# qiskit-community/aqc-research

Measured on AMD Instinct MI355X. Metric: objective+gradient evals/sec, higher is better.
Workload: dtype f64; 1 GPU; 16-qubit, 40-block cx spin ansatz, state-vector objective+gradient; n_qubits=16, num_thetas=208, gate_groups=56, batch_per_gpu=1024, columns=1, transport=none, records_gathered=1024, launcher=none

## Files before the change

### aqc_research_amd/csrc/aqc_api.cpp

```cpp
#include "aqc_ws.h"

using namespace aqc;

namespace {
thread_local std::string g_error;
}

namespace aqc {

int fail(const char* fmt, ...) {
    char buf[1024];
    va_list ap;
    va_start(ap, fmt);
    vsnprintf(buf, sizeof buf, fmt, ap);
    va_end(ap);
    g_error = buf;
    return 1;
}
int set_error(const std::string& msg) { g_error = msg; return 1; }

int check_buf(const aqc_ws* ws, int buf) {
    if (!ws) return fail("null workspace");
    if (buf < 0 || buf >= AQC_NUM_BUFS) return fail("invalid buffer id %d", buf);
    return 0;
}

int check_block_range(const aqc_ws* ws, int block_from, int block_to) {
    const int nb = ws->ctx->prog.num_blocks;
    if (block_from < 0 || nb == 0) return 0;
    if (!(block_from < block_to && block_to <= nb)) return fail("invalid block_range [%d, %d)", block_from, block_to);
    return 0;
}

int ensure_small(aqc_ws* ws, size_t n_cplx) {
    if (n_cplx <= ws->small_cap) return 0;
    if (ws->d_small) HIP_OK(hipFree(ws->d_small));
    ws->d_small = nullptr;
    HIP_OK(hipMalloc((void**)&ws->d_small, n_cplx * sizeof(double2)));
    ws->small_cap = n_cplx;
    return 0;
}

int ensure_tmp(aqc_ws* ws, size_t n_index, size_t n_cplx) {
    if (n_index > ws->tmp_index_cap) {
        if (ws->d_tmp_index) HIP_OK(hipFree(ws->d_tmp_index));
        ws->d_tmp_index = nullptr;
        HIP_OK(hipMalloc((void**)&ws->d_tmp_index, n_index * sizeof(long long)));
        ws->tmp_index_cap = n_index;
    }
    if (n_cplx > ws->tmp_small_cap) {
        if (ws->d_tmp_small) HIP_OK(hipFree(ws->d_tmp_small));
        ws->d_tmp_small = nullptr;
        HIP_OK(hipMalloc((void**)&ws->d_tmp_small, n_cplx * sizeof(double2)));
        ws->tmp_small_cap = n_cplx;
    }
    return 0;
}

int ensure_index(aqc_ws* ws, size_t n) {
    if (n <= ws->index_cap) return 0;
    if (ws->d_index) HIP_OK(hipFree(ws->d_index));
    ws->d_index = nullptr;
    HIP_OK(hipMalloc((void**)&ws->d_index, n * sizeof(long long)));
    ws->index_cap = n;
    return 0;
}

int ensure_coef(aqc_ws* ws) {
    if (ws->coef_valid) return 0;
    return fail("thetas have not been uploaded (aqc_ws_set_thetas)");
}

int copy_in(aqc_ws* ws, double2* dst, const double* src, size_t rows) {
    if (ws->pitch == ws->ncols) {
        HIP_OK(hipMemcpyAsync(dst, src, rows * ws->ncols * sizeof(double2), hipMemcpyHostToDevice, ws->stream));
    } else {
        HIP_OK(hipMemsetAsync(dst, 0, rows * ws->pitch * sizeof(double2), ws->stream));
        HIP_OK(hipMemcpy2DAsync(dst, (size_t)ws->pitch * sizeof(double2), src, (size_t)ws->ncols * sizeof(double2),
                                (size_t)ws->ncols * sizeof(double2), rows, hipMemcpyHostToDevice, ws->stream));
    }
    HIP_OK(hipStreamSynchronize(ws->stream));
    return 0;
}
int copy_out(aqc_ws* ws, double* dst, const double2* src, size_t rows) {
    if (ws->pitch == ws->ncols) {
        HIP_OK(hipMemcpyAsync(dst, src, rows * ws->ncols * sizeof(double2), hipMemcpyDeviceToHost, ws->stream));
    } else {
        HIP_OK(hipMemcpy2DAsync(dst, (size_t)ws->ncols * sizeof(double2), src, (size_t)ws->pitch * sizeof(double2),
                                (size_t)ws->ncols * sizeof(double2), rows, hipMemcpyDeviceToHost, ws->stream));
    }
    HIP_OK(hipStreamSynchronize(ws->stream));
    return 0;
}

int results_guard(aqc_ws* ws) {
    if (ws->copy_pending && !ws->capturing) {
        HIP_OK(hipStreamWaitEvent(ws->stream, ws->ev_copied, 0));
        ws->copy_pending = false;
    }
    return 0;
}


}

extern "C" {

const char* aqc_version(void) { return "aqc_hip 0.1.0 (gfx950)"; }
const char* aqc_last_error(void) { return g_error.c_str(); }

int aqc_device_count(void) {
    int ndev = 0;
    return hipGetDeviceCount(&ndev) == hipSuccess ? ndev : 0;
}

int aqc_create(int num_qubits, int entangler, const int32_t* blocks, int num_blocks, int trotter, int second_order,
               aqc_ctx** out) {
    if (!out) return fail("out pointer is null");
    *out = nullptr;
    aqc_ctx* ctx = new aqc_ctx();
    const std::string err = build_program(num_qubits, entangler, blocks, num_blocks, trotter != 0, second_order != 0, ctx->prog);
    if (!err.empty()) {
        delete ctx;
        return fail("%s", err.c_str());
    }
    *out = ctx;
    return 0;
}

int aqc_destroy(aqc_ctx* ctx) {
    if (!ctx) return 0;
    for (auto& kv : ctx->oneshot) aqc_ws_destroy(kv.second);
    delete ctx;
    return 0;
}

int aqc_num_thetas(const aqc_ctx* ctx) { return ctx ? ctx->prog.num_thetas() : -1; }
int aqc_num_gate_groups(const aqc_ctx* ctx) { return ctx ? (int)ctx->prog.groups.size() : -1; }

int aqc_plan_query(aqc_ctx* ctx, int ncols, int which, int tile_bits, int low_bits, int stage, int* num_stages,
                   int* bits_out, int* num_bits, int* ops_out, int* num_ops) {
    if (!ctx) return fail("null context");
    if (ncols < 1) return fail("ncols must be positive");
    const int col_bits = ceil_log2(ncols);
    if (tile_bits <= 0) tile_bits = which == 1 ? 12 : 13;
    if (low_bits < 0) low_bits = 3;
    Plan plan = make_plan(ctx->prog, col_bits, tile_bits, low_bits, which == 0);
    if (which == 3) {
        split_substages(ctx->prog, plan, 4, 1 << 20);
        plan = mirror_plan(plan);
    }
    const std::string err = check_plan(ctx->prog, plan);
    if (!err.empty()) return fail("planner produced an invalid plan: %s", err.c_str());
    if (num_stages) *num_stages = (int)plan.stages.size();
    if (stage >= 0) {
        if (stage >= (int)plan.stages.size()) return fail("stage index out of range");
        const Stage& st = plan.stages[stage];
        if (num_bits) *num_bits = (int)st.bits.size();
        if (num_ops) *num_ops = (int)st.ops.size();
        if (bits_out) for (size_t i = 0; i < st.bits.size(); ++i) bits_out[i] = st.bits[i];
        if (ops_out) for (size_t i = 0; i < st.ops.size(); ++i) ops_out[i] = st.ops[i];
    }
    return 0;
}

int aqc_plan_projected(aqc_ctx* ctx, int tile_bits, int low_bits, int32_t* info) {
    if (!ctx || !info) return fail("null argument");
    if (tile_bits <= 0) tile_bits = 12;
    if (low_bits < 0) low_bits = 3;
    const Program& prog = ctx->prog;
    tile_bits = std::min(std::max(tile_bits, 8), std::min(12, prog.n));
    aqc_ws tmp;
    tmp.ctx = ctx;
    tmp.ncols = 1; tmp.col_bits = 0; tmp.nbits = prog.n;
    Plan best = make_plan(prog, 0, tile_bits, low_bits, false);
    for (int lb = low_bits - 1; lb >= 2; --lb) {
        Plan cand = make_plan(prog, 0, tile_bits, lb, false);
        if (cand.stages.size() < best.stages.size()) best = cand;
    }
    lower_plan(prog, best, tmp.sweep, 4, true, true);
    tmp.sparse_enabled = true;
    tmp.inv_mirrored = tmp.sweep.v3 && tmp.sweep.plan.stages.size() >= 2;
    proj_plan(&tmp, low_bits);
    const int rc = aqc_ws_projected_info(&tmp, info);
    tmp.ctx = nullptr;
    return rc;
}

int aqc_plan_substages(aqc_ctx* ctx, int ncols, int which, int tile_bits, int low_bits, int stage, int* num_subs, int* subs_out, int max_subs) {
    if (!ctx || !num_subs) return fail("null argument");
    if (ncols < 1) return fail("ncols must be positive");
    const int col_bits = ceil_log2(ncols);
    if (tile_bits <= 0) tile_bits = 12;
    if (low_bits < 0) low_bits = 3;
    Plan plan = make_plan(ctx->prog, col_bits, tile_bits, low_bits, which == 0);
    split_substages(ctx->prog, plan, 4, 1 << 20);
    if (which == 3) plan = mirror_plan(plan);
    const std::string err = check_plan(ctx->prog, plan);
    if (!err.empty()) return fail("planner produced an invalid plan: %s", err.c_str());
    if (stage < 0 || stage >= (int)plan.stages.size()) return fail("stage index out of range");
    const Stage& st = plan.stages[stage];
    *num_subs = (int)st.subs.size();
    if (subs_out)
        for (int i = 0; i < (int)st.subs.size() && i < max_subs; ++i) {
            for (int j = 0; j < 4; ++j) subs_out[5 * i + j] = j < (int)st.subs[i].bits.size() ? st.subs[i].bits[j] : -1;
            subs_out[5 * i + 4] = (int)st.subs[i].ops.size();
        }
    return 0;
}

int aqc_ws_create(aqc_ctx* ctx, int device, int batch, int ncols, int tile_bits_apply, int tile_bits_sweep, aqc_ws** out) {
    if (!out) return fail("out pointer is null");
    *out = nullptr;
    if (!ctx) return fail("null context");
    if (batch < 1 || batch > 65535) return fail("batch must be in [1, 65535] (lanes are the y dimension of the launch grid)");
    if (ncols < 1) return fail("ncols must be >= 1");
    const Program& prog = ctx->prog;
    int ndev = 0;
    hipError_t e = hipGetDeviceCount(&ndev);
    if (e != hipSuccess || ndev <= 0)
        return fail("no HIP device available (%s): the aqc_hip path needs an AMD GPU and has no CPU fallback",
                    e == hipSuccess ? "device count is 0" : hipGetErrorString(e));
    if (device < 0 || device >= ndev) return fail("device %d out of range (%d visible)", device, ndev);
    HIP_OK(hipSetDevice(device));
    HIP_OK(init_kernels());
    HIP_OK(init_kernels2());
    HIP_OK(init_kernels3());

    aqc_ws* ws = new aqc_ws();
    ws->ctx = ctx;
    ws->device = device;
    ws->batch = batch;
    ws->ncols = ncols;
    ws->col_bits = ceil_log2(ncols);
    ws->pitch = 1 << ws->col_bits;
    ws->nbits = ws->col_bits + prog.n;
    if (ws->nbits > kMaxBits) { delete ws; return fail("2^%d elements per lane is beyond this build's limit", ws->nbits); }
    ws->lane_elems = (size_t)1 << ws->nbits;
    const int low_bits = env_int("AQC_LOW_BITS", 3);
    int ka = tile_bits_apply > 0 ? tile_bits_apply : env_int("AQC_TILE_BITS_APPLY", 0);
    int ks = tile_bits_sweep > 0 ? tile_bits_sweep : env_int("AQC_TILE_BITS_SWEEP", 0);
    const int family = env_int("AQC_KERNEL_FAMILY", env_int("AQC_KERNEL_V2", -1) >= 0 ? env_int("AQC_KERNEL_V2", -1) + 1 : 0);
    if (family < 0 || family > 3) { delete ws; return fail("AQC_KERNEL_FAMILY must be 1 (per-group), 2 (register-blocked) or 3 (matrix cores)"); }
    const bool want_v3 = (family == 3 || family == 0) && ws->nbits >= 8;
    const int force_v2 = family == 3 ? 0 : (family ? family - 1 : -1);
    const size_t big_tiles = (size_t)batch << std::max(0, ws->nbits - 12);
    const bool want_v2 = force_v2 >= 0 ? force_v2 != 0 : big_tiles >= 512;
    auto pick = [&](int kmax) {
        if (want_v3) {
            int k = std::min(12, ws->nbits);
            while (k > 10 && ((size_t)batch << (ws->nbits - k)) < 256) --k;
            const int kmin = std::max(8, prog.n + std::min(ws->col_bits, 3));
            while (ws->col_bits > 0 && k > kmin && ((size_t)batch << (ws->nbits - k)) < 256) --k;
            return k;
        }
        if (want_v2) return std::min(kmax, ws->nbits);
        int k = std::min(11, ws->nbits);
        while (k > 10 && ((size_t)batch << (ws->nbits - k)) < 512) --k;
        return k;
    };
    if (ka <= 0) ka = pick(13);
    if (ks <= 0) ks = pick(12);
    ka = std::min(std::min(ka, 13), ws->nbits);
    ks = std::min(std::min(ks, 12), ws->nbits);
    ws->threads = env_int("AQC_THREADS", 0);
    if (ws->threads <= 0) ws->threads = std::min(256, std::max(64, 1 << (std::min(ka, ks) - 2)));
    if (ws->threads < 64 || ws->threads > 512 || ws->threads % 64) { delete ws; return fail("AQC_THREADS must be a multiple of 64 in [64, 512]"); }

    auto best_plan = [&](int k, bool inverse) {
        Plan best = make_plan(prog, ws->col_bits, k, low_bits, inverse);
        for (int lb = low_bits - 1; lb >= 2; --lb) {
            Plan cand = make_plan(prog, ws->col_bits, k, lb, inverse);
            if (cand.stages.size() < best.stages.size()) best = cand;
        }
        return best;
    };
    if (want_v3) { ka = std::min(std::max(ka, 8), 12); ks = std::max(ks, 8); }
    auto cached_plan = [&](int which, int k, bool inverse, int reg_bits, bool dots, DevPlan& out) {
        const std::vector<int> key = {which, ws->col_bits, k, low_bits, reg_bits, (int)dots, (int)want_v3};
        std::lock_guard<std::mutex> lock(ctx->mu);
        auto it = ctx->plan_cache.find(key);
        if (it == ctx->plan_cache.end()) {
            DevPlan fresh;
            lower_plan(prog, best_plan(k, inverse), fresh, reg_bits, dots, want_v3);
            it = ctx->plan_cache.emplace(key, std::move(fresh)).first;
        }
        out = it->second;
    };
    cached_plan(2, ka, false, (want_v2 || want_v3) ? 4 : 0, false, ws->fwd);
    cached_plan(1, ks, false, want_v3 ? 4 : (want_v2 ? (env_int("AQC_SWEEP_REG_BITS", 4) == 3 ? 3 : 4) : 0), true, ws->sweep);
    ws->inv_mirrored = want_v3 && ka == ks && ws->sweep.v3 && ws->sweep.plan.stages.size() >= 2 && env_int("AQC_MIRROR_PLAN", 1) != 0;
    if (ws->inv_mirrored) {
        const std::vector<int> key = {3, ws->col_bits, ks, low_bits, 4, 0, 1};
        std::lock_guard<std::mutex> lock(ctx->mu);
        auto it = ctx->plan_cache.find(key);
        if (it == ctx->plan_cache.end()) {
            DevPlan fresh;
            lower_plan(prog, mirror_plan(ws->sweep.plan), fresh, 4, false, true, true);
            it = ctx->plan_cache.emplace(key, std::move(fresh)).first;
        }
        ws->inv = it->second;
    } else {
        cached_plan(0, ka, true, (want_v2 || want_v3) ? 4 : 0, false, ws->inv);
    }
    ws->sparse_enabled = env_int("AQC_SPARSE_SWEEP", 1) != 0;
    ws->sparse_min_items = env_int("AQC_SPARSE_MIN_ITEMS", 512);
    ws->lazy_z_enabled = env_int("AQC_LAZY_Z", 1) != 0;
    ws->r_only_enabled = env_int("AQC_R_ONLY_LAST", 1) != 0;
    ws->r_only_max_subs = env_int("AQC_R_ONLY_MAX_SUBS", 12);
    ws->proj_vdag_enabled = env_int("AQC_PROJECTED_VDAG", 1) != 0;
    ws->proj_fused_enabled = env_int("AQC_PROJECTED_FUSED", 1) != 0;
    ws->proj_vdag_min_elems = (long long)env_int("AQC_PROJECTED_VDAG_MIN_ELEMS", 1 << 24);
    ws->skipw_enabled = env_int("AQC_SKIP_ZERO_W", 0) != 0;
    for (DevPlan* p : {&ws->fwd, &ws->inv, &ws->sweep}) {
        const std::string err = check_plan(prog, p->plan);
        if (!err.empty()) { delete ws; return fail("planner produced an invalid plan: %s", err.c_str()); }
    }
    proj_plan(ws, low_bits);

    const int T = prog.num_thetas();
    const int G = (int)prog.groups.size();
    ws->nslots = G * kSlotsPerGroup;
    const int partial_tiles = ws->sweep.v3 ? 1 : ws->sweep.ntiles;
    std::vector<int> theta_slots(2 * (size_t)std::max(T, 1), -1), slot_ntiles((size_t)std::max(ws->nslots, 1), partial_tiles);
    auto feed = [&](int theta, int slot) {
        if (theta_slots[2 * theta] < 0) theta_slots[2 * theta] = slot; else theta_slots[2 * theta + 1] = slot;
    };
    for (int gi = 0; gi < G; ++gi) {
        const GateGroup& g = prog.groups[gi];
        if (g.type == GROUP_FRONT) {
            feed(g.theta0 + 2, gi * kSlotsPerGroup + 0);
            feed(g.theta0 + 1, gi * kSlotsPerGroup + 1);
            feed(g.theta0 + 0, gi * kSlotsPerGroup + 2);
        } else {
            for (int d = 0; d < prog.tpb; ++d) feed(g.theta0 + d, gi * kSlotsPerGroup + d);
        }
    }

    std::vector<int> slot_theta((size_t)std::max(ws->nslots, 1), -1);
    ws->grads_direct = ws->sweep.v3 && T > 0 && env_int("AQC_GRADS_DIRECT", 1) != 0;
    for (int t = 0; t < T; ++t) {
        if (theta_slots[2 * t] < 0 || theta_slots[2 * t + 1] >= 0) { ws->grads_direct = false; break; }
        slot_theta[theta_slots[2 * t]] = t;
    }
    if (env_int("AQC_VERBOSE", 0) && want_v3)
        fprintf(stderr, "aqc_hip: matrix-core kernels, tiles 2^%d (V / V^H, %d workgroups per CU) / 2^%d (sweep, %d per CU), sub-stages %zu / %zu / %zu\n",
                ws->inv.k, mfma_occupancy(ws->inv.k, false), ws->sweep.k, mfma_occupancy(ws->sweep.k, true), ws->fwd.h_subs3.size(),
                ws->inv.h_subs3.size(), ws->sweep.h_subs3.size());
#define WS_TRY(x) do { if ((x) != 0) { aqc_ws_destroy(ws); return 1; } } while (0)
#define WS_HIP(x) do { hipError_t e_ = (x); if (e_ != hipSuccess) { fail("%s failed: %s", #x, hipGetErrorString(e_)); aqc_ws_destroy(ws); return 1; } } while (0)
    WS_HIP(hipStreamCreateWithFlags(&ws->stream, hipStreamNonBlocking));
    WS_HIP(hipEventCreate(&ws->ev0)); WS_HIP(hipEventCreate(&ws->ev1));
    WS_HIP(hipEventCreate(&ws->pev0)); WS_HIP(hipEventCreate(&ws->pev1));
    WS_TRY(upload_plan(ws->fwd)); WS_TRY(upload_plan(ws->inv)); WS_TRY(upload_plan(ws->sweep));
    WS_TRY(proj_alloc(ws));
    WS_HIP(hipMalloc((void**)&ws->d_thetas_own, sizeof(double) * (size_t)batch * std::max(T, 1)));
    ws->d_thetas = ws->d_thetas_own;
    WS_HIP(hipMalloc((void**)&ws->d_coef, sizeof(double) * (size_t)batch * (prog.n + prog.num_blocks + 1) * kCoefStride));
    for (int b = 0; b < AQC_NUM_BUFS; ++b) {
        WS_HIP(hipMalloc((void**)&ws->bufs[b], sizeof(double2) * (size_t)batch * ws->lane_elems));
        WS_HIP(hipMemsetAsync(ws->bufs[b], 0, sizeof(double2) * (size_t)batch * ws->lane_elems, ws->stream));
    }
    WS_HIP(hipMalloc((void**)&ws->d_partial, sizeof(double2) * (size_t)batch * std::max(ws->nslots, 1) * partial_tiles));
    for (DevPlan* p : {&ws->fwd, &ws->inv, &ws->sweep})
        if (p->v3) WS_HIP(hipMalloc((void**)&p->d_umat, sizeof(double) * (size_t)batch * std::max<size_t>(p->h_subs3.size(), 1) * 12 * 64));
    {
        std::vector<UJob> jobs;
        DevPlan* vsw = ws->proj.ok ? &ws->proj.vsw : nullptr;
        const int nsw = ws->sweep.v3 ? (int)ws->sweep.h_subs3.size() : 0;
        ws->ujobs_mirror = ws->inv_mirrored && ws->inv.v3 && (int)ws->inv.h_subs3.size() == nsw && env_int("AQC_UBUILD_MIRROR", 1) != 0;
        for (DevPlan* p : {&ws->inv, &ws->sweep, vsw, &ws->fwd})
            if (p && p->v3)
                for (size_t i = 0; i < p->h_subs3.size(); ++i) {
                    if (p == &ws->inv && ws->ujobs_mirror) continue;
                    UJob j{p->d_subs3 + i, p->d_grps, p->d_umat, (int)i, (int)p->h_subs3.size(), p->plan.inverse ? 1 : 0, prog.entangler, nullptr, 0, 0};
                    if (p == &ws->sweep && ws->ujobs_mirror) { j.umat_mirror = ws->inv.d_umat; j.mirror_index = nsw - 1 - (int)i; j.mirror_nsubs = nsw; }
                    if (p == vsw) {
                        const int nvs = (int)vsw->h_subs3.size();
                        j.umat_mirror = ws->proj.vinv.d_umat; j.mirror_index = nvs - 1 - (int)i; j.mirror_nsubs = nvs;
                    }
                    jobs.push_back(j);
                }
        if (!jobs.empty()) {
            WS_HIP(hipMalloc((void**)&ws->d_ujobs, sizeof(UJob) * jobs.size()));
            WS_HIP(hipMemcpy(ws->d_ujobs, jobs.data(), sizeof(UJob) * jobs.size(), hipMemcpyHostToDevice));
        }
    }
    if (ws->sweep.v3)
        WS_HIP(hipMalloc((void**)&ws->sweep.d_rpart, sizeof(double2) * (size_t)batch * std::max<size_t>(ws->sweep.h_subs3.size(), 1) *
                                                        sweep3_nparts(ws->sweep.ntiles, batch, ws->sweep.k) * 256));
    WS_HIP(hipMalloc((void**)&ws->d_grads, sizeof(double2) * (size_t)batch * std::max(T, 1)));
    WS_HIP(hipMalloc((void**)&ws->d_theta_slots, sizeof(int) * theta_slots.size()));
    WS_HIP(hipMalloc((void**)&ws->d_slot_ntiles, sizeof(int) * slot_ntiles.size()));
    WS_HIP(hipMemcpy(ws->d_theta_slots, theta_slots.data(), sizeof(int) * theta_slots.size(), hipMemcpyHostToDevice));
    WS_HIP(hipMalloc((void**)&ws->d_slot_theta, sizeof(int) * slot_theta.size()));
    WS_HIP(hipMemcpy(ws->d_slot_theta, slot_theta.data(), sizeof(int) * slot_theta.size(), hipMemcpyHostToDevice));
    WS_HIP(hipMemcpy(ws->d_slot_ntiles, slot_ntiles.data(), sizeof(int) * slot_ntiles.size(), hipMemcpyHostToDevice));
    ws->pin_thetas = (size_t)batch * std::max(T, 1);
    ws->pin_grads = 2 * (size_t)batch * std::max(T, 1);
    ws->pin_small = 2 * (size_t)batch * 64;
    WS_HIP(hipHostMalloc((void**)&ws->h_pin, sizeof(double) * (ws->pin_thetas + ws->pin_grads + ws->pin_small), hipHostMallocDefault));
    ws->vdot_parts = (int)std::min<size_t>(1024, std::max<size_t>(1, ws->lane_elems / 1024));
    WS_HIP(hipMalloc((void**)&ws->d_vdot_part, sizeof(double2) * (size_t)batch * ws->vdot_parts));
    WS_HIP(hipStreamSynchronize(ws->stream));
#undef WS_TRY
#undef WS_HIP
    *out = ws;
    return 0;
}


int aqc_ws_destroy(aqc_ws* ws) {
    if (!ws) return 0;
    (void)hipSetDevice(ws->device);
    if (ws->stream) (void)hipStreamSynchronize(ws->stream);
    drop_graphs(ws);
    proj_free(ws);
    for (DevPlan* p : {&ws->fwd, &ws->inv, &ws->sweep}) {
        if (p->d_stages) (void)hipFree(p->d_stages);
        if (p->d_ops) (void)hipFree(p->d_ops);
        if (p->d_subs) (void)hipFree(p->d_subs);
        if (p->d_mops) (void)hipFree(p->d_mops);
        if (p->d_subs3) (void)hipFree(p->d_subs3);
        if (p->d_grps) (void)hipFree(p->d_grps);
        if (p->d_umat) (void)hipFree(p->d_umat);
        if (p->d_rpart) (void)hipFree(p->d_rpart);
    }
    void* ptrs[] = {ws->d_thetas_own, ws->d_theta_bank, ws->d_coef, ws->d_partial, ws->d_grads, ws->d_small, ws->d_vdot_part, ws->d_index, ws->d_tmp_index, ws->d_tmp_small,
                    ws->d_theta_slots, ws->d_slot_theta, ws->d_slot_ntiles, ws->d_basis_index, ws->d_vdot_out, ws->d_ujobs};
    for (void* p : ptrs) if (p) (void)hipFree(p);
    for (int b = 0; b < AQC_NUM_BUFS; ++b) if (ws->bufs[b]) (void)hipFree(ws->bufs[b]);
    for (int b = 0; b < AQC_NUM_BUFS; ++b) if (ws->d_combo_prev[b]) (void)hipFree(ws->d_combo_prev[b]);
    for (void* q : {(void*)ws->d_sw_items, (void*)ws->d_sw_clear, (void*)ws->d_sw_counts, (void*)ws->d_sw_lane_parts, (void*)ws->d_sw_prev_tiles,
                    (void*)ws->w2, (void*)ws->zw2, (void*)ws->d_vd_items})
        if (q) (void)hipFree(q);
    if (ws->d_sur) (void)hipFree(ws->d_sur);
    if (ws->d_sur_real) (void)hipFree(ws->d_sur_real);
    if (ws->h_sur) (void)hipHostFree(ws->h_sur);
    if (ws->d_combo_index) (void)hipFree(ws->d_combo_index);
    if (ws->d_combo_coef) (void)hipFree(ws->d_combo_coef);
    if (ws->h_pin) (void)hipHostFree(ws->h_pin);
    for (auto& m : ws->mps) if (m.d_t) (void)hipFree(m.d_t);
    if (ws->d_mps_scratch) (void)hipFree(ws->d_mps_scratch);
    for (auto& t : ws->mps_tabs) if (t.dev) (void)hipFree(t.dev);
    if (ws->d_cd_prog) (void)hipFree(ws->d_cd_prog);
    if (ws->d_cd_thetas) (void)hipFree(ws->d_cd_thetas);
    if (ws->d_cd_fobj) (void)hipFree(ws->d_cd_fobj);
    if (ws->d_mps_lam) (void)hipFree(ws->d_mps_lam);
    for (hipEvent_t ev : {ws->ev0, ws->ev1, ws->pev0, ws->pev1, ws->ev_ready, ws->ev_copied}) if (ev) (void)hipEventDestroy(ev);
    if (ws->copy_stream) { (void)hipStreamSynchronize(ws->copy_stream); (void)hipStreamDestroy(ws->copy_stream); }
    if (ws->mps_stream) { (void)hipStreamSynchronize(ws->mps_stream); (void)hipStreamDestroy(ws->mps_stream); }
    for (hipEvent_t ev : {ws->ev_mps_fork, ws->ev_mps_join}) if (ev) (void)hipEventDestroy(ev);
    if (ws->stream) (void)hipStreamDestroy(ws->stream);
    delete ws;
    return 0;
}

int aqc_ws_set_thetas(aqc_ws* ws, const double* thetas) {
    if (!ws || !thetas) return fail("null argument");
    HIP_OK(hipSetDevice(ws->device));
    const Program& prog = ws->ctx->prog;
    const int T = prog.num_thetas();
    HIP_OK(hipMemcpyAsync(ws->d_thetas_own, thetas, sizeof(double) * (size_t)ws->batch * T, hipMemcpyHostToDevice, ws->stream));
    HIP_OK(hipStreamSynchronize(ws->stream));
    return run_coef(ws, ws->d_thetas_own);
}

int aqc_ws_upload(aqc_ws* ws, int buf, const double* src) {
    if (check_buf(ws, buf) || before_write(ws, buf)) return 1;
    if (!src) return fail("null source");
    HIP_OK(hipSetDevice(ws->device));
    return copy_in(ws, ws->bufs[buf], src, (size_t)ws->batch << ws->ctx->prog.n);
}

int aqc_ws_upload_lane(aqc_ws* ws, int buf, int lane, const double* src) {
    if (check_buf(ws, buf)) return 1;
    if (!src) return fail("null source");
    if (lane < 0 || lane >= ws->batch) return fail("lane out of range");
    HIP_OK(hipSetDevice(ws->device));
    if (before_write(ws, buf, true)) return 1;
    return copy_in(ws, ws->bufs[buf] + (size_t)lane * ws->lane_elems, src, (size_t)1 << ws->ctx->prog.n);
}

int aqc_ws_broadcast(aqc_ws* ws, int buf, const double* src) {
    if (check_buf(ws, buf) || before_write(ws, buf)) return 1;
    if (!src) return fail("null source");
    HIP_OK(hipSetDevice(ws->device));
    if (copy_in(ws, ws->bufs[buf], src, (size_t)1 << ws->ctx->prog.n)) return 1;
    for (int b = 1; b < ws->batch; ++b)
        HIP_OK(hipMemcpyAsync(ws->bufs[buf] + (size_t)b * ws->lane_elems, ws->bufs[buf], ws->lane_elems * sizeof(double2),
                              hipMemcpyDeviceToDevice, ws->stream));
    return 0;
}

int aqc_ws_copy_lane(aqc_ws* dst_ws, int dst_buf, int dst_lane, aqc_ws* src_ws, int src_buf, int src_lane) {
    if (check_buf(dst_ws, dst_buf) || check_buf(src_ws, src_buf)) return 1;
    if (dst_ws->device != src_ws->device) return fail("copy_lane: the two workspaces live on different devices");
    if (dst_ws->lane_elems != src_ws->lane_elems) return fail("copy_lane: lane sizes differ");
    if (dst_lane < 0 || dst_lane >= dst_ws->batch || src_lane < 0 || src_lane >= src_ws->batch) return fail("lane out of range");
    if (before_read(src_ws, src_buf) || before_write(dst_ws, dst_buf, true)) return 1;
    HIP_OK(hipSetDevice(dst_ws->device));
    if (src_ws->stream != dst_ws->stream) HIP_OK(hipStreamSynchronize(src_ws->stream));
    HIP_OK(hipMemcpyAsync(dst_ws->bufs[dst_buf] + (size_t)dst_lane * dst_ws->lane_elems, src_ws->bufs[src_buf] + (size_t)src_lane * src_ws->lane_elems,
                          sizeof(double2) * dst_ws->lane_elems, hipMemcpyDeviceToDevice, dst_ws->stream));
    return 0;
}

int aqc_ws_download(aqc_ws* ws, int buf, double* dst) {
    if (check_buf(ws, buf)) return 1;
    if (!dst) return fail("null destination");
    HIP_OK(hipSetDevice(ws->device));
    if (before_read(ws, buf)) return 1;
    return copy_out(ws, dst, ws->bufs[buf], (size_t)ws->batch << ws->ctx->prog.n);
}

int aqc_ws_download_lane(aqc_ws* ws, int buf, int lane, double* dst) {
    if (check_buf(ws, buf)) return 1;
    if (!dst) return fail("null destination");
    if (lane < 0 || lane >= ws->batch) return fail("lane out of range");
    HIP_OK(hipSetDevice(ws->device));
    if (before_read(ws, buf)) return 1;
    return copy_out(ws, dst, ws->bufs[buf] + (size_t)lane * ws->lane_elems, (size_t)1 << ws->ctx->prog.n);
}

int aqc_ws_set_basis(aqc_ws* ws, int buf, const int64_t* index) {
    if (check_buf(ws, buf) || before_write(ws, buf)) return 1;
    if (!index) return fail("null index");
    HIP_OK(hipSetDevice(ws->device));
    const int64_t dim = (int64_t)1 << ws->ctx->prog.n;
    std::vector<long long> elem(ws->batch);
    for (int b = 0; b < ws->batch; ++b) {
        if (index[b] < 0 || index[b] >= dim) return fail("basis index out of range");
        elem[b] = (long long)index[b] << ws->col_bits;
    }
    if (!ws->d_basis_index) HIP_OK(hipMalloc((void**)&ws->d_basis_index, sizeof(long long) * ws->batch));
    HIP_OK(hipMemcpyAsync(ws->d_basis_index, elem.data(), sizeof(long long) * ws->batch, hipMemcpyHostToDevice, ws->stream));
    HIP_OK(hipStreamSynchronize(ws->stream));
    HIP_OK(hipMemsetAsync(ws->bufs[buf], 0, sizeof(double2) * (size_t)ws->batch * ws->lane_elems, ws->stream));
    {
        ProfScope ps(ws, AQC_K_MISC);
        HIP_OK(launch_scatter_one(ws->bufs[buf], ws->lane_elems, ws->batch, ws->d_basis_index, ws->stream));
    }
    std::vector<long long> supp(2 * (size_t)ws->batch, -1);
    for (int b = 0; b < ws->batch; ++b) supp[2 * (size_t)b] = elem[b];
    if (!ws->d_combo_prev[buf]) HIP_OK(hipMalloc((void**)&ws->d_combo_prev[buf], sizeof(long long) * 2 * ws->batch));
    HIP_OK(hipMemcpyAsync(ws->d_combo_prev[buf], supp.data(), sizeof(long long) * supp.size(), hipMemcpyHostToDevice, ws->stream));
    HIP_OK(hipStreamSynchronize(ws->stream));
    std::vector<double> coef(4 * (size_t)ws->batch, 0.0);
    for (int b = 0; b < ws->batch; ++b) coef[4 * (size_t)b] = 1.0;
    lhs_support_changed(ws, buf, std::move(supp), std::move(coef));
    return 0;
}

int aqc_ws_set_identity(aqc_ws* ws, int buf) {
    if (check_buf(ws, buf) || before_write(ws, buf)) return 1;
    const int dim = 1 << ws->ctx->prog.n;
    if (ws->ncols != dim) return fail("identity needs a square workspace (ncols == 2^n)");
    HIP_OK(hipSetDevice(ws->device));
    HIP_OK(hipMemsetAsync(ws->bufs[buf], 0, sizeof(double2) * (size_t)ws->batch * ws->lane_elems, ws->stream));
    ProfScope ps(ws, AQC_K_MISC);
    HIP_OK(launch_set_identity(ws->bufs[buf], ws->lane_elems, dim, ws->pitch, ws->batch, ws->stream));
    return 0;
}

int aqc_ws_set_combo(aqc_ws* ws, int buf, const int64_t* index, const double* coef) {
    if (check_buf(ws, buf)) return 1;
    if (!index || !coef) return fail("null argument");
    if (buf == AQC_BUF_W || buf == AQC_BUF_ZW || buf == AQC_BUF_Z) return fail("set_combo targets an lhs buffer (X, X2) or Y");
    HIP_OK(hipSetDevice(ws->device));
    const int64_t dim = (int64_t)1 << ws->ctx->prog.n;
    const int B = ws->batch;
    std::vector<long long> elem(2 * (size_t)B);
    for (int b = 0; b < B; ++b) {
        const int64_t i0 = index[2 * b], i1 = index[2 * b + 1];
        if (i0 < 0 || i0 >= dim || i1 >= dim) return fail("basis index out of range");
        if (i1 == i0) return fail("the two basis states of a lane must differ");
        elem[2 * b] = (long long)i0 << ws->col_bits;
        elem[2 * b + 1] = i1 < 0 ? -1 : (long long)i1 << ws->col_bits;
    }
    std::vector<double> cf(coef, coef + 4 * (size_t)B);
    if (ws->combo_valid[buf] && ws->combo_last_elem[buf] == elem && ws->combo_last_coef[buf] == cf) return 0;
    if (!ws->d_combo_index) HIP_OK(hipMalloc((void**)&ws->d_combo_index, sizeof(long long) * 2 * B));
    if (!ws->d_combo_coef) HIP_OK(hipMalloc((void**)&ws->d_combo_coef, sizeof(double2) * 2 * B));
    if (!ws->d_combo_prev[buf]) HIP_OK(hipMalloc((void**)&ws->d_combo_prev[buf], sizeof(long long) * 2 * B));
    HIP_OK(hipMemcpyAsync(ws->d_combo_index, elem.data(), sizeof(long long) * 2 * B, hipMemcpyHostToDevice, ws->stream));
    HIP_OK(hipMemcpyAsync(ws->d_combo_coef, coef, sizeof(double2) * 2 * B, hipMemcpyHostToDevice, ws->stream));
    HIP_OK(hipStreamSynchronize(ws->stream));
    if (!ws->combo_valid[buf]) {
        HIP_OK(hipMemsetAsync(ws->bufs[buf], 0, sizeof(double2) * (size_t)B * ws->lane_elems, ws->stream));
        HIP_OK(hipMemsetAsync(ws->d_combo_prev[buf], 0xff, sizeof(long long) * 2 * B, ws->stream));
    }
    ProfScope ps(ws, AQC_K_MISC);
    HIP_OK(launch_scatter_two(ws->bufs[buf], ws->lane_elems, B, ws->d_combo_index, ws->d_combo_coef, ws->d_combo_prev[buf], ws->stream));
    lhs_support_changed(ws, buf, std::move(elem), std::move(cf));
    return 0;
}

int aqc_ws_get_grads(aqc_ws* ws, double* grads) {
    if (!ws || !grads) return fail("null argument");
    HIP_OK(hipSetDevice(ws->device));
    HIP_OK(hipMemcpyAsync(grads, ws->d_grads, sizeof(double2) * (size_t)ws->batch * ws->ctx->prog.num_thetas(),
                          hipMemcpyDeviceToHost, ws->stream));
    HIP_OK(hipStreamSynchronize(ws->stream));
    return 0;
}

int aqc_ws_gather(aqc_ws* ws, int buf, const int64_t* index, int count, double* out) {
    if (check_buf(ws, buf)) return 1;
    if (!index || !out || count < 1) return fail("invalid gather arguments");
    HIP_OK(hipSetDevice(ws->device));
    if (before_read(ws, buf)) return 1;
    const int64_t dim = (int64_t)1 << ws->ctx->prog.n;
    std::vector<long long> elem(count);
    for (int i = 0; i < count; ++i) {
// ... 352 lines not shown
```

### aqc_research_amd/csrc/aqc_kernels3.hip

```cpp
#include <hip/hip_runtime.h>

#include <cstring>

#include <type_traits>

#include "aqc_device.h"
#include "aqc_launch.h"
#include "aqc_math.h"

namespace aqc {

typedef double double4_t __attribute__((ext_vector_type(4)));

__host__ __device__ __forceinline__ unsigned swz3(unsigned l) { return l ^ ((l >> 4) & 15u) ^ ((l >> 8) & 15u); }

__device__ __forceinline__ double4_t mfma(double a, double b, double4_t c) {
    return __builtin_amdgcn_mfma_f64_16x16x4f64(a, b, c, 0, 0, 0);
}

struct Acc3 { double4_t k1, k2, k3; };
__device__ __forceinline__ void u_mfma(const cplx (&v)[4], const double (&u0)[4], const double (&u1)[4], const double (&u2)[4], Acc3& t) {
    t.k1 = double4_t{0.0, 0.0, 0.0, 0.0}; t.k2 = t.k1; t.k3 = t.k1;
#pragma unroll
    for (int s = 0; s < 4; ++s) {
        t.k1 = mfma(v[s].x + v[s].y, u0[s], t.k1);
        t.k2 = mfma(v[s].x, u1[s], t.k2);
        t.k3 = mfma(v[s].y, u2[s], t.k3);
    }
}
__device__ __forceinline__ void u_combine(const Acc3& t, cplx (&o)[4]) {
#pragma unroll
    for (int r = 0; r < 4; ++r) {
        o[r].x = t.k1[r] - t.k3[r];
        o[r].y = t.k1[r] + t.k2[r];
    }
}

#ifdef AQC_TUNING
#define AQC_STAMP(slot) do { if (a.stamps && threadIdx.x == 0 && (slot) < kStampSlots) \
    a.stamps[((size_t)blockIdx.y * gridDim.x + blockIdx.x) * kStampSlots + (slot)] = __builtin_amdgcn_s_memtime(); } while (0)
#ifdef AQC_TUNING_NODBG
#define AQC_DBG_AND(x)
#define AQC_DBG_TEST(x) false
#else
#define AQC_DBG_AND(x) && (x)
#define AQC_DBG_TEST(x) (x)
#endif
#else
#define AQC_STAMP(slot) do { } while (0)
#define AQC_DBG_AND(x)
#define AQC_DBG_TEST(x) false
#endif

__host__ __device__ constexpr bool sweep_scratch_double(int k) { return k >= 12 || k <= 9; }
#ifndef AQC_SWEEP_SPREAD
#define AQC_SWEEP_SPREAD 1
#endif
#ifndef AQC_APPLY_SPREAD
#define AQC_APPLY_SPREAD 1
#endif
#ifndef AQC_EXP_APPLY_SKIP
#define AQC_EXP_APPLY_SKIP 0
#endif
constexpr int kApplySkip = AQC_EXP_APPLY_SKIP;
#ifndef AQC_EXP_SWEEP_SKIP
#define AQC_EXP_SWEEP_SKIP 0
#endif
constexpr int kSweepSkip = AQC_EXP_SWEEP_SKIP;

constexpr int kSweepSpread = AQC_SWEEP_SPREAD, kApplySpread = AQC_APPLY_SPREAD;
template <int K, bool SWEEP = false> struct TileShape {
    static constexpr int kSweepWaves12 = 4;
    static constexpr int kWaves = (SWEEP && K == 12) ? kSweepWaves12 : (K >= 10 ? 4 : (1 << (K - 8)));
    static constexpr int kGroups = 1 << (K - 8);
    static constexpr int kGpw = kGroups / kWaves;
    static constexpr int kLoads = (1 << (K - 6)) / kWaves;
};

struct SubRegs {
    double u0[4], u1[4], u2[4];
    unsigned lane12;
};

template <int GPW>
__device__ __forceinline__ void fetch_sub(SubRegs& x, const DevSub3* subs, const double* umat, int sub_index, int lane, int wave,
                                          int nwaves) {
    const DevSub3* sub = subs + sub_index;
    const double* up = umat + (size_t)sub_index * 12 * 64;
#pragma unroll
    for (int s = 0; s < 4; ++s) {
        x.u0[s] = up[(0 * 4 + s) * 64 + lane];
        x.u1[s] = up[(1 * 4 + s) * 64 + lane];
        x.u2[s] = up[(2 * 4 + s) * 64 + lane];
    }
    x.lane12 = sub->lane12[lane];
}

template <int GPW>
struct SubAddr {
    unsigned a1, a2;
    unsigned k1[GPW][4], k2[GPW][4];
};
typedef unsigned uint8v_t __attribute__((ext_vector_type(8)));
template <int GPW>
__device__ __forceinline__ void fetch_k(SubAddr<GPW>& x, const DevSub3* subs, int sub_index, int wave, int nwaves) {
#pragma unroll
    for (int j = 0; j < GPW; ++j) {
        const uint8v_t kv = *reinterpret_cast<const __attribute__((address_space(4))) uint8v_t*>(
            (const __attribute__((address_space(4))) void*)(const void*)&subs[sub_index].kk[wave + j * nwaves][0]);
#pragma unroll
        for (int s = 0; s < 4; ++s) { x.k1[j][s] = kv[s]; x.k2[j][s] = kv[4 + s]; }
    }
}
template <int GPW>
__device__ __forceinline__ void sub_addr(SubAddr<GPW>& x, const SubRegs& c, unsigned lds_base) {
    x.a1 = ((c.lane12 & 0xffffu) << 4) + lds_base;
    x.a2 = ((c.lane12 >> 16) << 4) + lds_base;
}
typedef double dbl2_t __attribute__((ext_vector_type(2)));
typedef __attribute__((address_space(3))) dbl2_t* lds_cplx_ptr;
__device__ __forceinline__ cplx lds_get(unsigned addr) {
    const dbl2_t v = *reinterpret_cast<lds_cplx_ptr>(addr);
    return make_double2(v.x, v.y);
}
__device__ __forceinline__ void lds_put(unsigned addr, cplx v) { *reinterpret_cast<lds_cplx_ptr>(addr) = dbl2_t{v.x, v.y}; }
__device__ __forceinline__ unsigned lds_address(const void* p) {
    return (unsigned)reinterpret_cast<size_t>((__attribute__((address_space(3))) const char*)p);
}

__device__ __forceinline__ const void* uniform_ptr(const void* p) {
    const unsigned long long v = (unsigned long long)p;
    const unsigned lo = __builtin_amdgcn_readfirstlane((unsigned)v), hi = __builtin_amdgcn_readfirstlane((unsigned)(v >> 32));
    return (const void*)(((unsigned long long)hi << 32) | lo);
}

template <int K, int NV>
__device__ __forceinline__ void load_tiles3(cplx* t0, cplx* t1, const cplx* s0, const cplx* s1, const DevStage& st, unsigned lo, int wave) {
    constexpr int NL = TileShape<K, NV == 2>::kLoads, NW = TileShape<K, NV == 2>::kWaves;
    cplx v0[NL], v1[NL];
#pragma unroll
    for (int i = 0; i < NL; ++i) {
        const unsigned off = lo + st.dhi[wave + i * NW];
        v0[i] = s0[off];
        if (NV == 2) v1[i] = s1[off];
    }
#pragma unroll
    for (int i = 0; i < NL; ++i) {
        const unsigned slot = swz3((unsigned)((wave + i * NW) << 6) | (threadIdx.x & 63u));
        t0[slot] = v0[i];
        if (NV == 2) t1[slot] = v1[i];
    }
}
template <int K, bool SWEEP>
__device__ __forceinline__ void store_tile3(const cplx* tile, cplx* dst, const DevStage& st, unsigned lo, int wave) {
    constexpr int NL = TileShape<K, SWEEP>::kLoads, NW = TileShape<K, SWEEP>::kWaves;
#pragma unroll
    for (int i = 0; i < NL; ++i) {
        const unsigned slot = swz3((unsigned)((wave + i * NW) << 6) | (threadIdx.x & 63u));
        dst[lo + st.dhi[wave + i * NW]] = tile[slot];
    }
}
__device__ __forceinline__ size_t tile_base3(const DevStage& st, unsigned tile) {
    size_t base = 0;
    for (int i0 = 0; i0 < st.nub; i0 += 4) {
        int ub[4];
#pragma unroll
        for (int u = 0; u < 4; ++u) ub[u] = st.ubits[i0 + u];
#pragma unroll
        for (int u = 0; u < 4; ++u)
            if (i0 + u < st.nub) base |= (size_t)((tile >> (i0 + u)) & 1u) << ub[u];
    }
    return base;
}

__device__ __forceinline__ int uniform_load(const int* p) { return __builtin_amdgcn_readfirstlane(*p); }
struct ItemAt { int bl, tile, slot; };
template <bool LIST>
__device__ __forceinline__ ItemAt item_at(const Stage3Args& a, int wi) {
    if (LIST) {
        const TileItem* it = a.items + wi;
        return ItemAt{uniform_load(&it->lane), uniform_load(&it->tile), uniform_load(&it->slot)};
    }
    const int bl = wi / a.ntiles;
    return ItemAt{bl, wi - bl * a.ntiles, 0};
}
template <int K, bool LIST = false>
__global__ __launch_bounds__(TileShape<K>::kWaves * 64, 2) void apply_mfma_kernel(const Stage3Args a) {
    using TS = TileShape<K>;
    extern __shared__ __attribute__((aligned(16))) char smem[];
    const DevStage& st = a.stage;
    cplx* tw = reinterpret_cast<cplx*>(smem);
    const unsigned lds_base = lds_address(smem);
    if (lds_base & ((16u << K) - 1)) __builtin_trap();
    const int lane = threadIdx.x & 63;
    const int wave = __builtin_amdgcn_readfirstlane((int)(threadIdx.x >> 6));
    constexpr int NL = TS::kLoads, NW = TS::kWaves;
    constexpr bool kPersist = K >= 12;
    const int nwork = LIST ? uniform_load(a.nitems) : a.ntiles * a.batch;
    const unsigned lo = st.dlo[lane];
    const unsigned lo16 = lo << 4;
    SubRegs cur, nxt;
    SubAddr<TS::kGpw> ad;
    dbl2_t pw[NL];
    int wi = blockIdx.x + ((kPersist || LIST) ? 0 : (int)blockIdx.y * a.ntiles);
    if (LIST && wi >= nwork) return;
    ItemAt it = item_at<LIST>(a, wi);
    {
        const int bl = it.bl;
        if (st.nsubs > 0) {
            fetch_sub<TS::kGpw>(cur, a.subs, a.umat + (size_t)bl * a.nsubs_total * 12 * 64, st.sub_begin, lane, wave, NW);
            fetch_k<TS::kGpw>(ad, a.subs, st.sub_begin, wave, NW);
        }
        AQC_STAMP(0);
        if (!(kApplySkip & 64)) load_tiles3<K, 1>(tw, nullptr, a.in0 + (size_t)bl * a.lane_stride + tile_base3(st, it.tile), nullptr, st, lo, wave);
    }
    __builtin_amdgcn_s_waitcnt(0x0F70);
    AQC_STAMP(1);
    for (;;) {
    const int bl = it.bl;
    const size_t lane_off = (size_t)bl * a.lane_stride + tile_base3(st, it.tile);
    const double* umat = a.umat + (size_t)bl * a.nsubs_total * 12 * 64;
    const int nwi = wi + (int)gridDim.x;
    const bool more = kPersist && st.nsubs > 0 && nwi < nwork;
    const ItemAt nit = more ? item_at<LIST>(a, nwi) : ItemAt{0, 0, 0};
    const int nbl = nit.bl;
    const size_t next_off = more ? (size_t)nbl * a.lane_stride + tile_base3(st, nit.tile) : 0;
    for (int si = 0; si < st.nsubs; ++si) {
        AQC_STAMP(4 + si);
        if (!(kApplySkip & 512)) __syncthreads();
        if (si + 1 < st.nsubs) fetch_sub<TS::kGpw>(nxt, a.subs, umat, st.sub_begin + si + 1, lane, wave, NW);
        else if (more) fetch_sub<TS::kGpw>(nxt, a.subs, a.umat + (size_t)nbl * a.nsubs_total * 12 * 64, st.sub_begin, lane, wave, NW);
        if (kPersist && more && !(kApplySkip & 64)) {
#pragma unroll
            for (int c = 0; c < 4; ++c) {
                if (si == (c < st.nsubs ? c : st.nsubs - 1)) {
#pragma unroll
                    for (int i = c * (NL / 4); i < (c + 1) * (NL / 4); ++i) {
                        const size_t ub = next_off + st.dhi[wave + i * NW];
                        asm volatile("s_nop 4\n\tglobal_load_dwordx4 %0, %1, %2" : "=a"(pw[i]) : "v"(lo16), "s"(uniform_ptr(a.in0 + ub)) : "memory");
                    }
                }
            }
        }
        sub_addr(ad, cur, lds_base);
        cplx v[2][4];
        Acc3 acc;
#pragma unroll
        for (int s = 0; s < 4; ++s) v[0][s] = lds_get(ad.a1 ^ ad.k1[0][s]);
#pragma unroll
        for (int j = 0; j <= TS::kGpw; ++j) {
            if (j + 1 < TS::kGpw && !(kApplySkip & 2)) {
#pragma unroll
                for (int s = 0; s < 4; ++s) v[(j + 1) & 1][s] = lds_get((kApplySkip & 32) ? ad.a1 : (ad.a1 ^ ad.k1[j + 1][s]));
            }
            __builtin_amdgcn_sched_barrier(0);
            double sv[4];
            cplx o[4];
            if (j < TS::kGpw) {
#pragma unroll
                for (int s = 0; s < 4; ++s) sv[s] = (kApplySkip & (16 | 128)) ? v[j & 1][s].x : v[j & 1][s].x + v[j & 1][s].y;
            }
            if (j > 0) {
                if (kApplySkip & (16 | 256)) {
#pragma unroll
                    for (int r = 0; r < 4; ++r) o[r] = make_double2(acc.k1[r], acc.k2[r]);
                } else u_combine(acc, o);
            }
            unsigned wa[4];
            if (j < TS::kGpw) {
#pragma unroll
                for (int s = 0; s < 4; ++s) asm volatile("" : "+v"(sv[s]));
            }
            if (j > 0) {
#pragma unroll
                for (int r = 0; r < 4; ++r) { wa[r] = (kApplySkip & 32) ? ad.a2 : (ad.a2 ^ ad.k2[j - 1][r]); asm volatile("" : "+v"(wa[r])); }
            }
            __builtin_amdgcn_sched_barrier(0);
            if (j < TS::kGpw) {
                acc.k1 = double4_t{0.0, 0.0, 0.0, 0.0}; acc.k2 = acc.k1; acc.k3 = acc.k1;
#pragma unroll
                for (int s = 0; s < 4; ++s) {
                    if (kApplySkip & 8) continue;
                    acc.k1 = mfma(sv[s], cur.u0[s], acc.k1);
                    acc.k2 = mfma(v[j & 1][s].x, cur.u1[s], acc.k2);
                    acc.k3 = mfma(v[j & 1][s].y, cur.u2[s], acc.k3);
                }
            }
            if (j > 0 && !(kApplySkip & 1)) {
#pragma unroll
                for (int r = 0; r < 4; ++r) lds_put(wa[r], o[r]);
                if (j < TS::kGpw) {
#pragma unroll
                    for (int i = 0; i < 4; ++i) {
                        __builtin_amdgcn_sched_group_barrier(0x008, kApplySpread, 0);
                        __builtin_amdgcn_sched_group_barrier(0x200, 1, 0);
                    }
                }
            }
            __builtin_amdgcn_sched_barrier(0);
        }
        if (si + 1 < st.nsubs || more) {
            cur = nxt;
            fetch_k<TS::kGpw>(ad, a.subs, si + 1 < st.nsubs ? st.sub_begin + si + 1 : st.sub_begin, wave, NW);
        }
    }
    AQC_STAMP(4 + st.nsubs);
    __syncthreads();
    AQC_STAMP(2);
    if (!(kApplySkip & 64)) store_tile3<K, false>(tw, a.out0 + lane_off, st, lo, wave);
    AQC_STAMP(3);
    if (!more) break;
    __syncthreads();
    __builtin_amdgcn_s_waitcnt(0x0F70);
#pragma unroll
    for (int i = 0; i < NL; ++i) {
        const unsigned slot = swz3((unsigned)((wave + i * NW) << 6) | (threadIdx.x & 63u));
        asm volatile("ds_write_b128 %0, %1" : : "v"(lds_base + (slot << 4)), "a"(pw[i]) : "memory");
    }
    __builtin_amdgcn_s_waitcnt(0xC07F);
    wi = nwi;
    it = nit;
    }
}

template <int N>
__device__ __forceinline__ void wait_prefetched(dbl2_t (&pw)[N], dbl2_t (&pz)[N]) {
    asm volatile("s_waitcnt vmcnt(0)" : : : "memory");
#pragma unroll
    for (int i = 0; i < N; ++i) asm volatile("" : "+a"(pw[i]), "+a"(pz[i]));
}
__device__ __forceinline__ unsigned tile_offset3(const DevStage& st, unsigned local) { return st.dlo[local & 63u] | st.dhi[local >> 6]; }
template <int K> struct SweepShape : TileShape<K, true> {};
__device__ __forceinline__ unsigned elem_bit(const DevStage& st, long long e, unsigned local_pos) {
    const unsigned m = local_pos < 6 ? st.dlo[1u << local_pos] : st.dhi[1u << (local_pos - 6)];
    return ((unsigned long long)e & m) ? 1u : 0u;
}
template <int GPW, int NW>
__device__ __forceinline__ void skip_masks(const DevStage& st, unsigned info, long long e0, long long e1, int wave, unsigned& nzmask, unsigned& kneed) {
    nzmask = 0; kneed = 0;
    const unsigned gfresh = info & 15u, kfresh = (info >> 6) & 3u;
#pragma unroll
    for (int k = 0; k < 2; ++k) {
        const long long e = k ? e1 : e0;
        if (e < 0) continue;
        unsigned gb = 0;
#pragma unroll
        for (int i = 0; i < 4; ++i)
            if (gfresh >> i & 1) gb |= elem_bit(st, e, (info >> (8 + 4 * i)) & 15u) << i;
        unsigned kb = 0;
        if (kfresh & 1) kb |= elem_bit(st, e, (info >> 24) & 15u);
        if (kfresh & 2) kb |= elem_bit(st, e, (info >> 28) & 15u) << 1;
#pragma unroll
        for (int j = 0; j < GPW; ++j)
            if ((((unsigned)(wave + j * NW) ^ gb) & gfresh) == 0) nzmask |= 1u << j;
#pragma unroll
        for (unsigned s2 = 0; s2 < 4; ++s2)
            if (((s2 ^ kb) & kfresh) == 0) kneed |= 1u << s2;
    }
}
template <int K, bool LIST = false, bool SKIPW = false, bool RLAST = false>
__global__ __launch_bounds__(SweepShape<K>::kWaves * 64, K >= 12 ? 1 : 2) void sweep_mfma_kernel(const Stage3Args a) {
    using TS = TileShape<K, true>;
    constexpr int kSlots = TS::kWaves > 4 ? 4 : TS::kWaves;
    constexpr unsigned tsize = 1u << K;
    extern __shared__ __attribute__((aligned(16))) char smem[];
    const DevStage& st = a.stage;
    cplx* tw = reinterpret_cast<cplx*>(smem);
    cplx* tz = tw + tsize;
    cplx* scratch = tz + tsize;
    constexpr bool kDouble = sweep_scratch_double(K);
    const unsigned lds_base = lds_address(smem);
    if (lds_base & ((32u << K) - 1)) __builtin_trap();
    const int lane = threadIdx.x & 63;
    const int wave = __builtin_amdgcn_readfirstlane((int)(threadIdx.x >> 6));
    constexpr bool kPersist = K >= 12;
    constexpr int NL = TS::kLoads, NW = TS::kWaves;
    const int nwork = LIST ? uniform_load(a.nitems) : a.ntiles * a.batch;
    const unsigned lo = st.dlo[lane];
    SubRegs cur, nxt;
    SubAddr<TS::kGpw> ad;
    dbl2_t pw[NL], pz[NL];
    unsigned parity = 0;
    AQC_STAMP(0);
    const int chunk = kPersist ? (LIST ? (nwork + (int)gridDim.x - 1) / (int)gridDim.x : a.chunk) : 0;
    const int wi_first = kPersist ? (int)blockIdx.x * chunk : (int)blockIdx.x;
    const int wi_end = kPersist ? (wi_first + chunk < nwork ? wi_first + chunk : nwork) : wi_first + 1;
    int wi = wi_first;
    if (wi >= nwork) return;
    const unsigned e16 = threadIdx.x << 4;
    dbl2_t racc;
    static_assert(!kPersist || NL == 4 * TS::kGpw, "the prefetch registers are the first sub-stage's operands");
    const bool reg_first = kPersist && st.nsubs > 0;
    unsigned flo16 = 0;
    ItemAt it = item_at<LIST>(a, wi);
    size_t item_off = (size_t)it.bl * a.lane_stride + tile_base3(st, it.tile);
    {
        const size_t off0 = item_off;
        if (st.nsubs > 0) {
            fetch_sub<TS::kGpw>(cur, a.subs, a.umat + (size_t)it.bl * a.nsubs_total * 12 * 64, st.sub_begin, lane, wave, NW);
            fetch_k<TS::kGpw>(ad, a.subs, st.sub_begin, wave, NW);
        }
        if (reg_first) {
            flo16 = tile_offset3(st, swz3(cur.lane12 & 0xffffu)) << 4;
#pragma unroll
            for (int i = 0; i < ((kSweepSkip & 64) ? 0 : NL); ++i) {
                const size_t ub = off0 + a.first_hi[wave + (i / 4) * NW][i % 4];
                asm volatile("s_nop 4\n\tglobal_load_dwordx4 %0, %1, %2" : "=a"(pw[i]) : "v"(flo16), "s"(uniform_ptr(a.in0 + ub)) : "memory");
                asm volatile("s_nop 4\n\tglobal_load_dwordx4 %0, %1, %2" : "=a"(pz[i]) : "v"(flo16), "s"(uniform_ptr(a.in1 + ub)) : "memory");
            }
        } else {
            load_tiles3<K, 2>(tw, tz, a.in0 + off0, a.in1 + off0, st, lo, wave);
        }
    }
    __builtin_amdgcn_s_waitcnt(0x0F70);
    if (reg_first) wait_prefetched<NL>(pw, pz);
    __syncthreads();
    AQC_STAMP(1);
    for (;;) {
    const int bl = it.bl, tile = it.tile;
    const size_t lane_off = item_off;
    long long se0 = -1, se1 = -1;
    if (SKIPW) {
        const unsigned long long toff = (unsigned long long)tile_base3(st, tile);
        const long long c0 = a.supp[2 * (size_t)bl], c1 = a.supp[2 * (size_t)bl + 1];
        const unsigned lo0 = __builtin_amdgcn_readfirstlane((unsigned)c0), hi0 = __builtin_amdgcn_readfirstlane((unsigned)(c0 >> 32));
        const unsigned lo1 = __builtin_amdgcn_readfirstlane((unsigned)c1), hi1 = __builtin_amdgcn_readfirstlane((unsigned)(c1 >> 32));
        const long long u0 = (long long)(((unsigned long long)hi0 << 32) | lo0), u1 = (long long)(((unsigned long long)hi1 << 32) | lo1);
        if (u0 >= 0 && (((unsigned long long)u0 ^ toff) & st.fresh_nonlocal) == 0) se0 = u0;
        if (u1 >= 0 && (((unsigned long long)u1 ^ toff) & st.fresh_nonlocal) == 0) se1 = u1;
    }
    const double* umat = a.umat + (size_t)bl * a.nsubs_total * 12 * 64;
    const int part = LIST ? it.slot : (kPersist ? (int)blockIdx.x - (bl * a.ntiles) / chunk : tile);
    const bool seg_first = LIST || !kPersist || wi == wi_first || tile == 0;
    cplx* rpart = a.rpart + (((size_t)bl * a.nsubs_total + st.sub_begin) * a.nparts + part) * 256;
    const int nwi = wi + 1;
    const bool more = reg_first && nwi < wi_end;
    const ItemAt nit = more ? item_at<LIST>(a, nwi) : ItemAt{0, 0, 0};
    const int nbl = nit.bl;
    const size_t next_off = more ? (size_t)nbl * a.lane_stride + tile_base3(st, nit.tile) : 0;
    constexpr unsigned ZOFF = tsize * 16;
    cplx vw[2][4], vz[2][4];
    constexpr bool kEarly = K >= 11;
    if (reg_first) {
        sub_addr(ad, cur, lds_base);
#pragma unroll
        for (int s = 0; s < 4; ++s) { vw[0][s] = make_double2(pw[s].x, pw[s].y); vz[0][s] = make_double2(pz[s].x, pz[s].y); }
    } else if (kEarly && st.nsubs > 0) {
        sub_addr(ad, cur, lds_base);
#pragma unroll
        for (int s = 0; s < 4; ++s) { vw[0][s] = lds_get(ad.a1 ^ ad.k1[0][s]); vz[0][s] = lds_get((ad.a1 | ZOFF) ^ ad.k1[0][s]); }
    }
    auto prefetch = [&](int c) __attribute__((always_inline)) {
#pragma unroll
        for (int i = 0; i < ((kSweepSkip & 64) ? 0 : NL); ++i)
            if (i / (NL / 4) == c) {
                const size_t ub = next_off + a.first_hi[wave + (i / 4) * NW][i % 4];
                asm volatile("s_nop 4\n\tglobal_load_dwordx4 %0, %1, %2" : "=a"(pw[i]) : "v"(flo16), "s"(uniform_ptr(a.in0 + ub)) : "memory");
                asm volatile("s_nop 4\n\tglobal_load_dwordx4 %0, %1, %2" : "=a"(pz[i]) : "v"(flo16), "s"(uniform_ptr(a.in1 + ub)) : "memory");
            }
    };
    const int nmain = RLAST && a.r_only_last && st.nsubs >= 1 && !(kPersist && st.nsubs == 1) ? st.nsubs - 1 : st.nsubs;
    if (!RLAST) {
        for (int si = 0; si < st.nsubs; ++si) {
#define AQC_SS_FROM_REGS (reg_first && si == 0)
#define AQC_SS_RONLY false
#include "aqc_sweep_substage.inc"
#undef AQC_SS_FROM_REGS
#undef AQC_SS_RONLY
        }
    } else {
        if (nmain > 0) {
            const int si = 0;
#define AQC_SS_FROM_REGS reg_first
#define AQC_SS_RONLY false
#include "aqc_sweep_substage.inc"
#undef AQC_SS_FROM_REGS
#undef AQC_SS_RONLY
        }
        for (int si = 1; si < nmain; ++si) {
#define AQC_SS_FROM_REGS false
#define AQC_SS_RONLY false
#include "aqc_sweep_substage.inc"
#undef AQC_SS_FROM_REGS
#undef AQC_SS_RONLY
        }
        if (nmain < st.nsubs) {
            const int si = nmain;
#define AQC_SS_FROM_REGS false
#define AQC_SS_RONLY true
#include "aqc_sweep_substage.inc"
#undef AQC_SS_FROM_REGS
#undef AQC_SS_RONLY
        }
    }
    AQC_STAMP(kStampSlots - 2);
    if (more) wait_prefetched<NL>(pw, pz);
    if (!(kSweepSkip & 64)) {
        if (a.store_out & 1) store_tile3<K, true>(tw, a.out0 + lane_off, st, lo, wave);
        if (a.store_out & 2) store_tile3<K, true>(tz, a.out1 + lane_off, st, lo, wave);
    }
    AQC_STAMP(kStampSlots - 1);
    if (!more) break;
    AQC_STAMP(kStampSlots - 6);
    __syncthreads();
    AQC_STAMP(kStampSlots - 5);
    wi = nwi;
    it = nit;
    item_off = next_off;
    }
    AQC_STAMP(kStampSlots - 4);
}

constexpr int kGrpChunk = 16;
struct Gm {
    cplx c[4], t[4];
    double ec, es;
    double rc[4], rs[4];
    int type, pc, pt, flags, slot0, jblock, o0, o1;
};
__device__ __forceinline__ void m2_mul(const cplx (&a)[4], const cplx (&b)[4], cplx (&o)[4]) {
#pragma unroll
    for (int i = 0; i < 2; ++i)
#pragma unroll
        for (int j = 0; j < 2; ++j) {
            const cplx x = a[2 * i], y = b[j], u = a[2 * i + 1], v = b[2 + j];
            o[2 * i + j] = make_double2(x.x * y.x - x.y * y.y + u.x * v.x - u.y * v.y, x.x * y.y + x.y * y.x + u.x * v.y + u.y * v.x);
        }
}
__device__ __forceinline__ void m2_ry(double c, double s, cplx (&o)[4]) {
    o[0] = make_double2(c, 0.0); o[1] = make_double2(-s, 0.0); o[2] = make_double2(s, 0.0); o[3] = make_double2(c, 0.0);
}
__device__ __forceinline__ void m2_rz(double c, double s, cplx (&o)[4]) {
    o[0] = make_double2(c, -s); o[1] = make_double2(0.0, 0.0); o[2] = make_double2(0.0, 0.0); o[3] = make_double2(c, s);
}
__device__ __forceinline__ void m2_rx(double c, double s, cplx (&o)[4]) {
    o[0] = make_double2(c, 0.0); o[1] = make_double2(0.0, -s); o[2] = make_double2(0.0, -s); o[3] = make_double2(c, 0.0);
}
template <bool DAG, bool TR>
__device__ __forceinline__ void m2_apply(const cplx (&m)[4], cplx& a0, cplx& a1) {
    const cplx m00 = m[0], m01 = (DAG || TR) ? m[2] : m[1], m10 = (DAG || TR) ? m[1] : m[2], m11 = m[3];
    const double sg = DAG ? -1.0 : 1.0;
    const cplx x = a0, y = a1;
    a0 = make_double2(m00.x * x.x - sg * m00.y * x.y + m01.x * y.x - sg * m01.y * y.y, m00.x * x.y + sg * m00.y * x.x + m01.x * y.y + sg * m01.y * y.x);
    a1 = make_double2(m10.x * x.x - sg * m10.y * x.y + m11.x * y.x - sg * m11.y * y.y, m10.x * x.y + sg * m10.y * x.x + m11.x * y.y + sg * m11.y * y.x);
}
__device__ __forceinline__ void stage_groups(Gm* gm, const DevGrp* grps, int begin, int count, const double* th, int ent, int lane) {
    {
        const int gi = lane >> 2, k = lane & 3;
        if (gi < count) {
            const DevGrp d = grps[begin + gi];
            double c = 1.0, s = 0.0;
            if (k < (d.type == 0 ? 3 : 4)) sincos(0.5 * th[d.theta0 + k], &s, &c);
            gm[gi].rc[k] = c; gm[gi].rs[k] = s;
            if (k == 0) {
                double ec = 1.0, es = 0.0;
                if (ent == 2 && d.type != 0) sincos(th[d.theta0 + 4], &es, &ec);
                gm[gi].ec = ec; gm[gi].es = es;
            }
        }
    }
    __builtin_amdgcn_fence(__ATOMIC_SEQ_CST, "wavefront");
    __builtin_amdgcn_wave_barrier();
    if (lane >= count) return;
    const DevGrp d = grps[begin + lane];
    Gm g;
    g.type = d.type; g.pc = d.pc; g.pt = d.pt; g.flags = d.flags; g.slot0 = d.slot0; g.jblock = d.jblock;
    const int mask = 0xF & ~(1 << d.pc) & ~(1 << d.pt);
    g.o0 = __ffs(mask) - 1; g.o1 = __ffs(mask & (mask - 1)) - 1;
    g.ec = gm[lane].ec; g.es = gm[lane].es;
#pragma unroll
    for (int k = 0; k < 4; ++k) { g.rc[k] = gm[lane].rc[k]; g.rs[k] = gm[lane].rs[k]; }
    cplx a[4], b[4], m[4];
    if (d.type == 0) {
        m2_rz(g.rc[0], g.rs[0], a); m2_ry(g.rc[1], g.rs[1], b); m2_mul(a, b, m);
        m2_rz(g.rc[2], g.rs[2], b); m2_mul(m, b, g.c);
        g.t[0] = make_double2(1.0, 0.0); g.t[1] = make_double2(0.0, 0.0); g.t[2] = g.t[1]; g.t[3] = g.t[0];
    } else {
        m2_rz(g.rc[1], g.rs[1], a); m2_ry(g.rc[0], g.rs[0], b); m2_mul(a, b, g.c);
        if (d.flags & 1) { m2_rz(kR, -kR, b); m2_mul(g.c, b, m); g.c[0] = m[0]; g.c[1] = m[1]; g.c[2] = m[2]; g.c[3] = m[3]; }
        if (ent == 0) m2_rx(g.rc[3], g.rs[3], a); else m2_rz(g.rc[3], g.rs[3], a);
        m2_ry(g.rc[2], g.rs[2], b); m2_mul(a, b, g.t);
        if (d.flags & 2) { m2_rz(kR, kR, a); m2_mul(a, g.t, m); g.t[0] = m[0]; g.t[1] = m[1]; g.t[2] = m[2]; g.t[3] = m[3]; }
    }
    gm[lane] = g;
}
__device__ __forceinline__ int grp_index(const Gm& g, int l, int rest) {
    return ((l >> 1) << g.pc) | ((l & 1) << g.pt) | ((rest & 1) << g.o0) | ((rest >> 1) << g.o1);
}
template <int MODE>
__device__ __forceinline__ void grp_apply(const Gm& g, int ent, cplx (&x)[4]) {
    auto entangle = [&](double es) {
        if (g.type == 0) return;
        if (ent == 0) { const cplx t = x[2]; x[2] = x[3]; x[3] = t; }
        else if (ent == 1) x[3] = make_double2(-x[3].x, -x[3].y);
        else x[3] = cmul(x[3], g.ec, es);
    };
    if (MODE == 0) {
        entangle(g.es);
        m2_apply<false, false>(g.t, x[0], x[1]); m2_apply<false, false>(g.t, x[2], x[3]);
        m2_apply<false, false>(g.c, x[0], x[2]); m2_apply<false, false>(g.c, x[1], x[3]);
    } else {
        m2_apply<MODE == 1, MODE == 2>(g.c, x[0], x[2]); m2_apply<MODE == 1, MODE == 2>(g.c, x[1], x[3]);
        m2_apply<MODE == 1, MODE == 2>(g.t, x[0], x[1]); m2_apply<MODE == 1, MODE == 2>(g.t, x[2], x[3]);
        entangle(MODE == 1 ? -g.es : g.es);
    }
}

__global__ __launch_bounds__(64) void ubuild_kernel(const UJob* jobs, const double* thetas, int T, double* thetas_copy) {
    __shared__ cplx u[256];
    __shared__ Gm gm[kGrpChunk];
    const int lane = threadIdx.x, b = blockIdx.y;
    const UJob job = jobs[blockIdx.x];
    const DevSub3 sub = *job.sub;
    const double* th = thetas + (size_t)b * T;
    if (thetas_copy && blockIdx.x == 0)
        for (int i = lane; i < T; i += 64) thetas_copy[(size_t)b * T + i] = th[i];
#pragma unroll
    for (int m = 0; m < 4; ++m) {
        const int e = lane + 64 * m;
        u[e] = make_double2((e >> 4) == (e & 15) ? 1.0 : 0.0, 0.0);
    }
    const int col = lane & 15, rest = lane >> 4;
    for (int base = 0; base < sub.ngrp; base += kGrpChunk) {
        const int count = min(kGrpChunk, sub.ngrp - base);
        __syncthreads();
        stage_groups(gm, job.grps, sub.grp_begin + base, count, th, job.entangler, lane);
        __syncthreads();
        for (int i = 0; i < count; ++i) {
            const Gm& g = gm[i];
            cplx x[4];
            int idx[4];
#pragma unroll
            for (int l = 0; l < 4; ++l) { idx[l] = grp_index(g, l, rest) * 16 + col; x[l] = u[idx[l]]; }
            if (job.inverse) grp_apply<1>(g, job.entangler, x); else grp_apply<0>(g, job.entangler, x);
#pragma unroll
            for (int l = 0; l < 4; ++l) u[idx[l]] = x[l];
            __syncthreads();
        }
    }
    __syncthreads();
    double* out = job.umat + ((size_t)b * job.nsubs + job.index) * 12 * 64;
#pragma unroll
    for (int s = 0; s < 4; ++s) {
        const cplx v = u[(lane & 15) * 16 + 4 * s + (lane >> 4)];
        out[(0 * 4 + s) * 64 + lane] = v.x;
        out[(1 * 4 + s) * 64 + lane] = v.y - v.x;
        out[(2 * 4 + s) * 64 + lane] = v.x + v.y;
    }
    if (job.umat_mirror) {
        double* om = job.umat_mirror + ((size_t)b * job.mirror_nsubs + job.mirror_index) * 12 * 64;
#pragma unroll
        for (int s = 0; s < 4; ++s) {
            const cplx t = u[(4 * s + (lane >> 4)) * 16 + (lane & 15)];
            const double re = t.x, im = -t.y;
            om[(0 * 4 + s) * 64 + lane] = re;
            om[(1 * 4 + s) * 64 + lane] = im - re;
            om[(2 * 4 + s) * 64 + lane] = re + im;
        }
    }
}

template <int LB>
__device__ __forceinline__ void rho_unapply(cplx (&rho)[16], int kind, double c, double s) {
    constexpr int st = LB == 0 ? 1 : 2, other = LB == 0 ? 2 : 1;
#pragma unroll
    for (int q = 0; q < 2; ++q)
#pragma unroll
        for (int b = 0; b < 4; ++b) {
            const int a0 = q * other;
            if (kind == MOP_RY) ry2(rho[a0 * 4 + b], rho[(a0 + st) * 4 + b], c, -s);
            else if (kind == MOP_RZ) rz2(rho[a0 * 4 + b], rho[(a0 + st) * 4 + b], c, -s);
            else rx2(rho[a0 * 4 + b], rho[(a0 + st) * 4 + b], c, -s);
        }
#pragma unroll
    for (int q = 0; q < 2; ++q)
#pragma unroll
        for (int a = 0; a < 4; ++a) {
            const int b0 = q * other;
            if (kind == MOP_RY) ry2(rho[a * 4 + b0], rho[a * 4 + b0 + st], c, -s);
            else if (kind == MOP_RZ) rz2(rho[a * 4 + b0], rho[a * 4 + b0 + st], c, s);
            else rx2(rho[a * 4 + b0], rho[a * 4 + b0 + st], c, s);
        }
}
template <int LB>
__device__ __forceinline__ cplx rho_dot(const cplx (&rho)[16], int kind) {
    constexpr int st = LB == 0 ? 1 : 2, other = LB == 0 ? 2 : 1;
    double re = 0.0, im = 0.0;
#pragma unroll
    for (int q = 0; q < 2; ++q) {
        const int i0 = q * other, i1 = i0 + st;
        if (kind == MOP_RY) { re += rho[i1 * 4 + i0].x - rho[i0 * 4 + i1].x; im += rho[i1 * 4 + i0].y - rho[i0 * 4 + i1].y; }
        else if (kind == MOP_RZ) { re += rho[i0 * 4 + i0].x - rho[i1 * 4 + i1].x; im += rho[i0 * 4 + i0].y - rho[i1 * 4 + i1].y; }
        else { re += rho[i0 * 4 + i1].x + rho[i1 * 4 + i0].x; im += rho[i0 * 4 + i1].y + rho[i1 * 4 + i0].y; }
    }
    return kind == MOP_RY ? make_double2(0.5 * re, 0.5 * im) : make_double2(-0.5 * im, 0.5 * re);
}

#ifdef AQC_TUNING
__device__ unsigned long long g_rgrad_stamps[32 * 8];
#define RG_STAMP(slot) do { if (blockIdx.y == 0 && blockIdx.x < 32 && threadIdx.x == 0) g_rgrad_stamps[blockIdx.x * 8 + (slot)] = __builtin_amdgcn_s_memtime(); } while (0)
#else
#define RG_STAMP(slot) do { } while (0)
#endif
template <int WAVES>
__global__ __launch_bounds__(64 * WAVES) void rgrad_kernel(const DevSub3* subs, const DevGrp* grps, int ent, const double* thetas, int T,
                                                           const cplx* rpart, int ntiles, int nsubs_total, cplx* partial, int nslots,
                                                           int from, int to, int front, const int* slot_theta, cplx* grads, cplx* mirror,
                                                           const GatherJob gj, int tiles_per_lane, int chunk, int sparse_subs,
                                                           const int* lane_parts, int conj_sub, const double* umat, int nsubs_run,
                                                           const RgradSecond second) {
    if ((int)blockIdx.x == nsubs_run + second.count) {
        const cplx* src = static_cast<const cplx*>(gj.buf) + (size_t)blockIdx.y * gj.lane_stride;
        for (int i = threadIdx.x; i < gj.count; i += 64 * WAVES) {
            const cplx v = src[(size_t)gj.elem[i]];
            static_cast<cplx*>(gj.out)[(size_t)blockIdx.y * gj.count + i] = v;
            if (gj.mirror) static_cast<cplx*>(gj.mirror)[(size_t)blockIdx.y * gj.count + i] = v;
        }
        return;
    }
    __shared__ cplx R[16 * 17];
    __shared__ Gm gm[kGrpChunk];
    __shared__ cplx rho_s[kGrpChunk][16];
    __shared__ cplx psum[WAVES > 1 ? WAVES - 1 : 1][WAVES > 1 ? 256 : 1];
    const int lane = threadIdx.x & 63, wave = threadIdx.x >> 6, b = blockIdx.y;
    int si = blockIdx.x;
    if (si >= nsubs_run) {
        si -= nsubs_run;
        subs = second.subs; grps = second.grps; rpart = second.rpart; ntiles = second.nparts; nsubs_total = second.nsubs_total;
        tiles_per_lane = second.nparts; chunk = 0; sparse_subs = second.nsubs_total; lane_parts = second.lane_parts; conj_sub = -1; umat = second.umat;
    }
    RG_STAMP(0);
    const DevSub3 sub = subs[si];
    const double* th = thetas + (size_t)b * T;
    const int nparts_stride = ntiles;
    if (chunk > 0) ntiles = ((b + 1) * tiles_per_lane - 1) / chunk - (b * tiles_per_lane) / chunk + 1;
    if (si < sparse_subs) ntiles = lane_parts[b];
    const cplx* rp = rpart + ((size_t)b * nsubs_total + si) * nparts_stride * 256;
    {
        cplx acc[4] = {make_double2(0.0, 0.0), make_double2(0.0, 0.0), make_double2(0.0, 0.0), make_double2(0.0, 0.0)};
        constexpr int TB = 8;
        for (int t0 = wave; t0 < ntiles; t0 += TB * WAVES) {
            cplx v[TB][4];
#pragma unroll
            for (int u = 0; u < TB; ++u)
#pragma unroll
                for (int r = 0; r < 4; ++r)
                    v[u][r] = t0 + u * WAVES < ntiles ? rp[(size_t)(t0 + u * WAVES) * 256 + 64 * r + lane] : make_double2(0.0, 0.0);
            if (WAVES > 1 && t0 == wave && wave == 0 && sub.ngrp > 0)
                stage_groups(gm, grps, sub.grp_begin + max(0, sub.ngrp - kGrpChunk), min(sub.ngrp, kGrpChunk), th, ent, lane);
#pragma unroll
            for (int u = 0; u < TB; ++u)
#pragma unroll
                for (int r = 0; r < 4; ++r) { acc[r].x += v[u][r].x; acc[r].y += v[u][r].y; }
        }
        if (WAVES > 1) {
            if (wave > 0) {
#pragma unroll
                for (int r = 0; r < 4; ++r) psum[wave - 1][64 * r + lane] = acc[r];
            }
            __syncthreads();
            if (wave > 0) return;
#pragma unroll
            for (int w = 0; w < WAVES - 1; ++w)
#pragma unroll
                for (int r = 0; r < 4; ++r) { const cplx p = psum[w][64 * r + lane]; acc[r].x += p.x; acc[r].y += p.y; }
        }
#pragma unroll
        for (int r = 0; r < 4; ++r)
            R[(4 * r + (lane >> 4)) * 17 + (lane & 15)] = acc[r];
    }
    if (si == conj_sub) {
        cplx* const Us = &rho_s[0][0];
        const double* up = umat + ((size_t)b * nsubs_total + si) * 12 * 64;
        __syncthreads();
#pragma unroll
        for (int s2 = 0; s2 < 4; ++s2) {
            const double re = up[(0 * 4 + s2) * 64 + lane], im = up[(1 * 4 + s2) * 64 + lane] + re;
            Us[(lane & 15) * 16 + 4 * s2 + (lane >> 4)] = make_double2(re, im);
        }
        __syncthreads();
        const int i0 = lane & 15, j0 = lane >> 4;
        cplx acc[4];
#pragma unroll
        for (int m = 0; m < 4; ++m) {
            const int j = j0 + 4 * m;
            double re = 0.0, im = 0.0;
            for (int k = 0; k < 16; ++k) {
                const cplx u = Us[j * 16 + k], r = R[k * 17 + i0];
                re += u.x * r.x - u.y * r.y; im += u.x * r.y + u.y * r.x;
            }
            acc[m] = make_double2(re, im);
        }
        __syncthreads();
#pragma unroll
        for (int m = 0; m < 4; ++m) R[(j0 + 4 * m) * 17 + i0] = acc[m];
        __syncthreads();
#pragma unroll
        for (int m = 0; m < 4; ++m) {
            const int j = j0 + 4 * m;
            double re = 0.0, im = 0.0;
            for (int k = 0; k < 16; ++k) {
                const cplx t = R[j * 17 + k], u = Us[i0 * 16 + k];
                re += t.x * u.x + t.y * u.y; im += t.y * u.x - t.x * u.y;
            }
            acc[m] = make_double2(re, im);
        }
        __syncthreads();
#pragma unroll
        for (int m = 0; m < 4; ++m) R[(j0 + 4 * m) * 17 + i0] = acc[m];
        __syncthreads();
    }
    RG_STAMP(1);
    cplx* out = partial + (size_t)b * nslots;
    auto put = [&](int slot, cplx v) {
        out[slot] = v;
        if (slot_theta) {
            const int t = slot_theta[slot];
            if (t >= 0) {
                grads[(size_t)b * T + t] = v;
                if (mirror) mirror[(size_t)b * T + t] = v;
            }
        }
    };
    const int lo = lane & 15, hi = lane >> 4;
    for (int top = sub.ngrp; top > 0; top -= kGrpChunk) {
        const int base = max(0, top - kGrpChunk), count = top - base;
        __syncthreads();
        if (WAVES == 1 || top != sub.ngrp) stage_groups(gm, grps, sub.grp_begin + base, count, th, ent, lane);
        __syncthreads();
        RG_STAMP(2);
        for (int i = count - 1; i >= 0; --i) {
            const Gm& g = gm[i];
            {
                const int a = lane >> 4, bb = (lane >> 2) & 3, o = lane & 3;
                cplx v = R[grp_index(g, a, o) * 17 + grp_index(g, bb, o)];
                v.x += dpp_mov<0xB1, 0xf>(v.x); v.y += dpp_mov<0xB1, 0xf>(v.y);
                v.x += dpp_mov<0x4E, 0xf>(v.x); v.y += dpp_mov<0x4E, 0xf>(v.y);
                if (o == 0) rho_s[i][a * 4 + bb] = v;
            }
            cplx x[4];
            int idx[4];
#pragma unroll
            for (int l = 0; l < 4; ++l) { idx[l] = grp_index(g, l, hi) * 17 + lo; x[l] = R[idx[l]]; }
            grp_apply<1>(g, ent, x);
#pragma unroll
            for (int l = 0; l < 4; ++l) R[idx[l]] = x[l];
            __syncthreads();
#pragma unroll
            for (int l = 0; l < 4; ++l) { idx[l] = lo * 17 + grp_index(g, l, hi); x[l] = R[idx[l]]; }
            grp_apply<2>(g, ent, x);
#pragma unroll
            for (int l = 0; l < 4; ++l) R[idx[l]] = x[l];
            __syncthreads();
        }
        RG_STAMP(3);
        if (lane < count) {
            const Gm& g = gm[lane];
            const bool on = g.jblock < 0 ? (front != 0) : (g.jblock >= from && g.jblock < to);
            if (on && g.slot0 >= 0) {
                cplx rho[16];
#pragma unroll
                for (int e = 0; e < 16; ++e) rho[e] = rho_s[lane][e];
                if (g.type == 0) {
                    put(g.slot0 + 2, rho_dot<1>(rho, MOP_RZ));
                    rho_unapply<1>(rho, MOP_RZ, g.rc[0], g.rs[0]);
                    put(g.slot0 + 1, rho_dot<1>(rho, MOP_RY));
                    rho_unapply<1>(rho, MOP_RY, g.rc[1], g.rs[1]);
                    put(g.slot0 + 0, rho_dot<1>(rho, MOP_RZ));
                } else {
                    const int ks = ent == 0 ? MOP_RX : MOP_RZ;
                    if (g.flags & 2) rho_unapply<0>(rho, MOP_RZ, kR, kR);
                    put(g.slot0 + 3, rho_dot<0>(rho, ks));
                    rho_unapply<0>(rho, ks, g.rc[3], g.rs[3]);
                    put(g.slot0 + 2, rho_dot<0>(rho, MOP_RY));
                    put(g.slot0 + 1, rho_dot<1>(rho, MOP_RZ));
                    rho_unapply<1>(rho, MOP_RZ, g.rc[1], g.rs[1]);
                    put(g.slot0 + 0, rho_dot<1>(rho, MOP_RY));
                    if (ent == 2) {
                        rho_unapply<0>(rho, MOP_RY, g.rc[2], g.rs[2]);
                        rho_unapply<1>(rho, MOP_RY, g.rc[0], g.rs[0]);
                        put(g.slot0 + 4, make_double2(rho[15].y, -rho[15].x));
                    }
                }
            } else if (slot_theta && g.slot0 >= 0) {
                for (int k = 0; k < 5; ++k) put(g.slot0 + k, make_double2(0.0, 0.0));
            }
        }
        RG_STAMP(4);
    }
}
#ifdef AQC_TUNING
void rgrad_print_stamps(int nsubs) {
    unsigned long long h[32 * 8];
    if (hipMemcpyFromSymbol(h, HIP_SYMBOL(g_rgrad_stamps), sizeof h) != hipSuccess) return;
    double a = 0, b = 0, c = 0, d = 0;
    const int n = nsubs < 32 ? nsubs : 32;
    for (int i = 0; i < n; ++i) { a += h[i * 8 + 1] - h[i * 8]; b += h[i * 8 + 2] - h[i * 8 + 1]; c += h[i * 8 + 3] - h[i * 8 + 2]; d += h[i * 8 + 4] - h[i * 8 + 3]; }
    fprintf(stderr, "aqc_hip stamps: gradient walk (lane 0, %d sub-stages): tile sum %.0f + group decode %.0f + R walk %.0f + rho walk %.0f cycles\n", n, a / n, b / n, c / n, d / n);
}
#endif

void stage3_first_offsets(Stage3Args& a, const DevSub3& first_sub) {
    for (int g = 0; g < 16; ++g)
        for (int s = 0; s < 4; ++s) {
            const unsigned local = swz3(first_sub.kk[g][s] >> 4);
            a.first_hi[g][s] = a.stage.dlo[local & 63u] | a.stage.dhi[local >> 6];
        }
}

int mfma_threads(int k, bool sweep) { return (sweep && k == 12) ? 64 * SweepShape<12>::kWaves : 64 * std::min(4, 1 << std::max(0, k - 8)); }
size_t apply3_lds_bytes(int k) { return (size_t)16 << k; }
size_t sweep3_lds_bytes(int k) {
    return ((size_t)32 << k) + (size_t)(sweep_scratch_double(k) ? 2 : 1) * std::min(4, mfma_threads(k, true) / 64) * 256 * sizeof(cplx);
}

template <typename F>
static hipError_t big_lds(F kernel) {
    return hipFuncSetAttribute(reinterpret_cast<const void*>(kernel), hipFuncAttributeMaxDynamicSharedMemorySize, 160 * 1024);
}
hipError_t init_kernels3() {
    hipError_t e;
#define AQC_TRY(x) if ((e = (x)) != hipSuccess) return e
    AQC_TRY(big_lds(apply_mfma_kernel<8>)); AQC_TRY(big_lds(apply_mfma_kernel<9>)); AQC_TRY(big_lds(apply_mfma_kernel<10>));
    AQC_TRY(big_lds(apply_mfma_kernel<11>)); AQC_TRY(big_lds(apply_mfma_kernel<12>));
    AQC_TRY(big_lds(sweep_mfma_kernel<8>)); AQC_TRY(big_lds(sweep_mfma_kernel<9>)); AQC_TRY(big_lds(sweep_mfma_kernel<10>));
    AQC_TRY(big_lds(sweep_mfma_kernel<11>)); AQC_TRY(big_lds(sweep_mfma_kernel<12>));
    AQC_TRY(big_lds((apply_mfma_kernel<8, true>))); AQC_TRY(big_lds((apply_mfma_kernel<9, true>))); AQC_TRY(big_lds((apply_mfma_kernel<10, true>)));
    AQC_TRY(big_lds((apply_mfma_kernel<11, true>))); AQC_TRY(big_lds((apply_mfma_kernel<12, true>)));
    AQC_TRY(big_lds((sweep_mfma_kernel<8, true>))); AQC_TRY(big_lds((sweep_mfma_kernel<9, true>))); AQC_TRY(big_lds((sweep_mfma_kernel<10, true>)));
    AQC_TRY(big_lds((sweep_mfma_kernel<11, true>))); AQC_TRY(big_lds((sweep_mfma_kernel<12, true>)));
    AQC_TRY(big_lds((sweep_mfma_kernel<8, false, true>))); AQC_TRY(big_lds((sweep_mfma_kernel<9, false, true>)));
    AQC_TRY(big_lds((sweep_mfma_kernel<10, false, true>))); AQC_TRY(big_lds((sweep_mfma_kernel<11, false, true>)));
    AQC_TRY(big_lds((sweep_mfma_kernel<12, false, true>)));
    AQC_TRY(big_lds((sweep_mfma_kernel<8, false, false, true>))); AQC_TRY(big_lds((sweep_mfma_kernel<9, false, false, true>)));
    AQC_TRY(big_lds((sweep_mfma_kernel<10, false, false, true>))); AQC_TRY(big_lds((sweep_mfma_kernel<11, false, false, true>)));
    AQC_TRY(big_lds((sweep_mfma_kernel<12, false, false, true>)));
    AQC_TRY(big_lds((sweep_mfma_kernel<8, true, false, true>))); AQC_TRY(big_lds((sweep_mfma_kernel<9, true, false, true>)));
    AQC_TRY(big_lds((sweep_mfma_kernel<10, true, false, true>))); AQC_TRY(big_lds((sweep_mfma_kernel<11, true, false, true>)));
    AQC_TRY(big_lds((sweep_mfma_kernel<12, true, false, true>)));
#undef AQC_TRY
    return hipSuccess;
}
int mfma_occupancy(int k, bool sweep) {
    int n = 0;
    hipError_t e = hipErrorInvalidValue;
    const int t = mfma_threads(k, sweep);
    const size_t l = sweep ? sweep3_lds_bytes(k) : apply3_lds_bytes(k);
#define AQC_OCC(KK) case KK: e = sweep ? hipOccupancyMaxActiveBlocksPerMultiprocessor(&n, sweep_mfma_kernel<KK>, t, l) \
                                      : hipOccupancyMaxActiveBlocksPerMultiprocessor(&n, apply_mfma_kernel<KK>, t, l); break
    switch (k) { AQC_OCC(8); AQC_OCC(9); AQC_OCC(10); AQC_OCC(11); AQC_OCC(12); default: break; }
#undef AQC_OCC
    return e == hipSuccess ? n : -1;
}
static long persistent_sweep_grid() {
    static int cus[64] = {0};
    int dev = 0;
    if (hipGetDevice(&dev) != hipSuccess || dev < 0 || dev >= 64) return 256;
    if (cus[dev] == 0) {
        int n = 0;
        cus[dev] = (hipDeviceGetAttribute(&n, hipDeviceAttributeMultiprocessorCount, dev) == hipSuccess && n > 0) ? n : 256;
    }
    if (const char* e = getenv("AQC_SWEEP_GRID")) { const long v = atol(e); if (v > 0) return v; }
    return cus[dev];
}
hipError_t launch_apply3(int ntiles, int batch, int k, hipStream_t s, const Stage3Args& a) {
    if (a.ntiles != ntiles || a.batch != batch) return hipErrorInvalidValue;
    for (int l = 0; l < 64; ++l)
        if (k >= 12 && a.stage.dlo[l] >= (1u << 28)) return hipErrorInvalidValue;
    const bool list = a.items != nullptr;
    if (list && (!a.nitems || a.max_items < 1)) return hipErrorInvalidValue;
    const long nwork = list ? (long)a.max_items : (long)ntiles * batch;
    static const long persist = []() { const char* e = getenv("AQC_APPLY_PERSIST"); return e ? atol(e) : 2L; }();
    const dim3 grid = (k >= 12 && persist > 0 && a.stage.nsubs > 0) ? dim3((unsigned)std::min<long>(nwork, persist * persistent_sweep_grid()))
                                                                     : ((k >= 12 || list) ? dim3((unsigned)nwork) : dim3(ntiles, batch));
    if (list && k >= 12 && !(persist > 0 && a.stage.nsubs > 0)) return hipErrorInvalidValue;
    const int t = mfma_threads(k, false);
    const size_t l = apply3_lds_bytes(k);
#define AQC_LAUNCH(KK) case KK: if (list) apply_mfma_kernel<KK, true><<<grid, t, l, s>>>(a); else apply_mfma_kernel<KK, false><<<grid, t, l, s>>>(a); break
    switch (k) {
        AQC_LAUNCH(8); AQC_LAUNCH(9); AQC_LAUNCH(10); AQC_LAUNCH(11); AQC_LAUNCH(12);
        default: return hipErrorInvalidValue;
    }
#undef AQC_LAUNCH
    return hipGetLastError();
}
int sweep3_chunk(int ntiles, int batch, int k) {
    if (k < 12) return 0;
    const long nwork = (long)ntiles * batch, g = std::min<long>(nwork, persistent_sweep_grid());
    return (int)((nwork + g - 1) / g);
}
int sweep3_nparts(int ntiles, int batch, int k) {
    const int chunk = sweep3_chunk(ntiles, batch, k);
    return chunk > 0 ? std::min(ntiles, (ntiles + chunk - 1) / chunk + 1) : ntiles;
}
hipError_t launch_sweep3(int ntiles, int batch, int k, hipStream_t s, const Stage3Args& a) {
    if (a.ntiles != ntiles || a.batch != batch) return hipErrorInvalidValue;
    const bool list = a.items != nullptr;
    if (list && (!a.nitems || a.max_items < 1)) return hipErrorInvalidValue;
    if (a.nparts < 1 || (!list && (a.nparts != sweep3_nparts(ntiles, batch, k) || a.chunk != sweep3_chunk(ntiles, batch, k)))) return hipErrorInvalidValue;
    if (k >= 12 && a.stage.nsubs <= 0) return hipErrorInvalidValue;
    for (int l = 0; l < 64; ++l)
        if (k >= 12 && a.stage.dlo[l] >= (1u << 28)) return hipErrorInvalidValue;
    const long nwork = list ? (long)a.max_items : (long)ntiles * batch;
    const dim3 grid((unsigned)(k >= 12 ? (list ? std::min<long>(nwork, persistent_sweep_grid()) : (nwork + a.chunk - 1) / a.chunk) : nwork));
    const int t = mfma_threads(k, true);
    const size_t l = sweep3_lds_bytes(k);
    const bool skipw = !list && a.supp != nullptr;
    const bool rlast = !skipw && a.r_only_last != 0;
#define AQC_LAUNCH(KK) case KK: if (list && rlast) sweep_mfma_kernel<KK, true, false, true><<<grid, t, l, s>>>(a); \
                                else if (list) sweep_mfma_kernel<KK, true, false><<<grid, t, l, s>>>(a); \
                                else if (skipw) sweep_mfma_kernel<KK, false, true><<<grid, t, l, s>>>(a); \
                                else if (rlast) sweep_mfma_kernel<KK, false, false, true><<<grid, t, l, s>>>(a); \
                                else sweep_mfma_kernel<KK, false, false><<<grid, t, l, s>>>(a); break
    switch (k) {
        AQC_LAUNCH(8); AQC_LAUNCH(9); AQC_LAUNCH(10); AQC_LAUNCH(11); AQC_LAUNCH(12);
        default: return hipErrorInvalidValue;
    }
#undef AQC_LAUNCH
    return hipGetLastError();
}

__device__ __forceinline__ int tile_of_elem(const DevStage& st, long long e) {
    int t = 0;
    for (int i = 0; i < st.nub; ++i) t |= (int)((e >> st.ubits[i]) & 1) << i;
    return t;
}
__device__ __forceinline__ int lane_tiles(const DevStage& st, const long long* supp, int per_lane, const long long* extra, int nextra, int b,
                                          int (&tiles)[kMaxTileCands]) {
    int n = 0;
    auto add = [&](long long e) {
        if (e < 0) return;
        const int t = tile_of_elem(st, e);
        for (int i = 0; i < n; ++i)
            if (tiles[i] == t) return;
        tiles[n++] = t;
    };
    for (int k = 0; supp && k < per_lane; ++k) add(supp[(size_t)b * per_lane + k]);
    for (int k = 0; extra && k < nextra; ++k) add(extra[k]);
    return n;
}
__global__ __launch_bounds__(1024) void tile_items_kernel(const DevStage st, const long long* supp, int per_lane, const long long* extra, int nextra,
                                                          int batch, TileItem* items, int* nitems, int* lane_parts, int* prev_tiles,
                                                          TileItem* clear_items, int* nclear) {
    __shared__ int scan_a[1024], scan_b[1024];
    const int tid = threadIdx.x, per = (batch + 1023) / 1024;
    const int b0 = tid * per, b1 = min(batch, b0 + per);
    int tiles[kMaxTileCands];
    int mine = 0, mine_clear = 0;
    for (int b = b0; b < b1; ++b) {
        const int n = lane_tiles(st, supp, per_lane, extra, nextra, b, tiles);
        mine += n;
        if (prev_tiles)
            for (int k = 0; k < 2; ++k) {
                const int pt = prev_tiles[2 * b + k];
                bool stale = pt >= 0;
                for (int i = 0; i < n; ++i) stale = stale && tiles[i] != pt;
                mine_clear += stale ? 1 : 0;
            }
    }
    scan_a[tid] = mine; scan_b[tid] = mine_clear;
    __syncthreads();
    for (int d = 1; d < 1024; d <<= 1) {
        const int va = tid >= d ? scan_a[tid - d] : 0, vb = tid >= d ? scan_b[tid - d] : 0;
        __syncthreads();
        scan_a[tid] += va; scan_b[tid] += vb;
        __syncthreads();
    }
    int at = scan_a[tid] - mine, at_clear = scan_b[tid] - mine_clear;
    if (tid == 1023) { *nitems = scan_a[tid]; if (nclear) *nclear = scan_b[tid]; }
    for (int b = b0; b < b1; ++b) {
        const int n = lane_tiles(st, supp, per_lane, extra, nextra, b, tiles);
        if (lane_parts) lane_parts[b] = n;
        if (prev_tiles) {
            for (int k = 0; k < 2; ++k) {
                const int pt = prev_tiles[2 * b + k];
                bool stale = pt >= 0;
                for (int i = 0; i < n; ++i) stale = stale && tiles[i] != pt;
                if (stale) clear_items[at_clear++] = TileItem{b, pt, 0, 0};
            }
            prev_tiles[2 * b] = n > 0 ? tiles[0] : -1;
            prev_tiles[2 * b + 1] = n > 1 ? tiles[1] : -1;
        }
        for (int i = 0; i < n; ++i) items[at++] = TileItem{b, tiles[i], i, 0};
    }
}
hipError_t launch_tile_items(const DevStage& stage, const long long* supp, int per_lane, const long long* extra, int nextra, int batch,
                             TileItem* items, int* nitems, int* lane_parts, int* prev_tiles, TileItem* clear_items, int* nclear, hipStream_t s) {
    if ((supp ? per_lane : 0) + (extra ? nextra : 0) > kMaxTileCands || batch < 1) return hipErrorInvalidValue;
    if (prev_tiles && ((supp ? per_lane : 0) > 2 || (extra && nextra > 0) || !clear_items || !nclear)) return hipErrorInvalidValue;
    tile_items_kernel<<<1, 1024, 0, s>>>(stage, supp, per_lane, extra, nextra, batch, items, nitems, lane_parts, prev_tiles, clear_items, nclear);
    return hipGetLastError();
}
__global__ __launch_bounds__(256) void clear_tiles_kernel(const DevStage st, cplx* buf, size_t lane_stride, const TileItem* clear_items, const int* nclear) {
    if ((int)blockIdx.x >= *nclear) return;
    const TileItem it = clear_items[blockIdx.x];
    cplx* dst = buf + (size_t)it.lane * lane_stride + tile_base3(st, (unsigned)it.tile);
    for (unsigned l = threadIdx.x; l < (1u << st.k); l += 256) dst[tile_offset3(st, l)] = make_double2(0.0, 0.0);
}
hipError_t launch_clear_tiles(const DevStage& stage, void* buf, size_t lane_stride, const TileItem* clear_items, const int* nclear, int max_items,
                              hipStream_t s) {
    if (max_items < 1) return hipSuccess;
    clear_tiles_kernel<<<max_items, 256, 0, s>>>(stage, static_cast<cplx*>(buf), lane_stride, clear_items, nclear);
    return hipGetLastError();
}
hipError_t launch_ubuild(const UJob* jobs, int njobs, const double* thetas, int T, int batch, hipStream_t s, double* thetas_copy) {
    if (njobs < 1) return hipSuccess;
    ubuild_kernel<<<dim3(njobs, batch), 64, 0, s>>>(jobs, thetas, T, thetas_copy);
    return hipGetLastError();
}
hipError_t launch_rgrad(const DevSub3* subs, const DevGrp* grps, int entangler, const double* thetas, int T, const void* rpart,
                        int ntiles, int nsubs_total, void* partial, int nslots, int from, int to, int front, int batch, hipStream_t s,
                        const int* slot_theta, void* grads, void* mirror, GatherJob gather, int nparts, int chunk, int sparse_subs,
                        const int* lane_parts, int conj_sub, const double* umat, int nsubs_run, const RgradSecond* second_plan) {
    if (nsubs_total < 1) return hipSuccess;
    if (nsubs_run < 0 || nsubs_run > nsubs_total) nsubs_run = nsubs_total;
    RgradSecond second;
    memset(&second, 0, sizeof second);
    if (second_plan) second = *second_plan;
    const int extra = (gather.count > 0 && gather.buf ? 1 : 0) + second.count;
    if (nsubs_run + extra < 1) return hipSuccess;
    const int tiles_per_lane = ntiles;
    if (nparts <= 0) nparts = ntiles;
    ntiles = nparts;
    if (nparts >= 32 && second.count == 0)
        rgrad_kernel<4><<<dim3(nsubs_run + extra, batch), 256, 0, s>>>(subs, grps, entangler, thetas, T, static_cast<const cplx*>(rpart), ntiles,
                                                                  nsubs_total, static_cast<cplx*>(partial), nslots, from, to, front, slot_theta,
                                                                  static_cast<cplx*>(grads), static_cast<cplx*>(mirror), gather, tiles_per_lane, chunk, sparse_subs, lane_parts, conj_sub, umat, nsubs_run, second);
    else
        rgrad_kernel<1><<<dim3(nsubs_run + extra, batch), 64, 0, s>>>(subs, grps, entangler, thetas, T, static_cast<const cplx*>(rpart), ntiles,
                                                                 nsubs_total, static_cast<cplx*>(partial), nslots, from, to, front, slot_theta,
                                                                 static_cast<cplx*>(grads), static_cast<cplx*>(mirror), gather, tiles_per_lane, chunk, sparse_subs, lane_parts, conj_sub, umat, nsubs_run, second);
    return hipGetLastError();
}

}
```

### aqc_research_amd/csrc/aqc_launch.h

```cpp
#pragma once
#include <string>
#include <hip/hip_runtime.h>

#include <algorithm>
#include <cstddef>

#include "aqc_device.h"
#include "aqc_mps_walk.h"

namespace aqc {

struct StageArgs {
    const DevStage* stage;
    const DevOp* ops;
    const DevSub* subs;
    const DevMop* mops;
    const double* coef;
    int ncoef;
    const double2* in0;
    const double2* in1;
    double2* out0;
    double2* out1;
    size_t lane_stride;
    double2* partial;
    int nslots, ntiles_max;
    int from, to, front;
    int final_stage;
    int debug;
};

size_t apply_lds_bytes(int k);
size_t sweep_lds_bytes(int k, int threads);
hipError_t init_kernels();
hipError_t launch_apply(int ent, bool inverse, int ntiles, int batch, int threads, int k, hipStream_t s, const StageArgs& a);
hipError_t launch_sweep(int ent, int ntiles, int batch, int threads, int k, hipStream_t s, const StageArgs& a);
hipError_t launch_coef(const double* thetas, double* coef, int n, int nblocks, int tpb, int tail, int batch, hipStream_t s);
hipError_t launch_finalize(const void* partial, const int* theta_slots, const int* slot_ntiles, void* grads, int T,
                           int nslots, int ntiles_max, int n, int tpb, int from, int to, int front, int batch,
                           hipStream_t s, void* mirror = nullptr);
hipError_t launch_scatter_one(void* buf, size_t lane_stride, int batch, const long long* elem, hipStream_t s);
hipError_t launch_scatter_two(void* buf, size_t lane_stride, int batch, const long long* elem, const void* coef, long long* prev, hipStream_t s);
hipError_t launch_set_identity(void* buf, size_t lane_stride, int dim, int pitch, int batch, hipStream_t s);
hipError_t launch_gather(const void* buf, size_t lane_stride, const long long* elem, int count, int batch, void* out,
                         hipStream_t s, void* mirror = nullptr);
hipError_t launch_vdot(const void* a, const void* b, size_t lane_stride, size_t count, int batch, void* part, int nparts,
                       void* out, hipStream_t s);

hipError_t init_kernels2();
hipError_t launch_apply2(int ent, int ntiles, int batch, int k, hipStream_t s, const StageArgs& a);
hipError_t launch_sweep2(int ent, int ntiles, int batch, int k, int reg_bits, hipStream_t s, const StageArgs& a);

struct TileItem { int lane, tile, slot, pad; };
struct Stage3Args {
    DevStage stage;
    const DevSub3* subs;
    const double* umat;
    int nsubs_total;
    const double2* in0;
    const double2* in1;
    double2* out0;
    double2* out1;
    size_t lane_stride;
    double2* rpart;
    int ntiles;
    int batch;
    int chunk, nparts;
    int store_out;
    int r_only_last;
    const long long* supp;
    const TileItem* items;
    const int* nitems;
    int max_items;
    unsigned first_hi[16][4];
    int debug;
    unsigned long long* stamps;
};
constexpr int kStampSlots = 40;
void stage3_first_offsets(Stage3Args& a, const DevSub3& first_sub);
hipError_t init_kernels3();
int mfma_threads(int k, bool sweep);
int mfma_occupancy(int k, bool sweep);
hipError_t launch_apply3(int ntiles, int batch, int k, hipStream_t s, const Stage3Args& a);
hipError_t launch_sweep3(int ntiles, int batch, int k, hipStream_t s, const Stage3Args& a);
void rgrad_print_stamps(int nsubs);
int sweep3_chunk(int ntiles, int batch, int k);
int sweep3_nparts(int ntiles, int batch, int k);
struct ProjMap { const unsigned* tab; int shift; };
struct ProjArgs {
    const double2* y;
    const double2* s;
    double2* out;
    int s_virtual, out_virtual;
    int staged;
    int keep_bits, k_bits, cb;
    ProjMap y_keep, y_k, s_k, s_c, o_keep, o_c;
    size_t lane_stride;
    const TileItem* items;
    const int* nitems;
    const int* lane_parts;
    int nub0, ubits0[32];
    unsigned ff_mask, cb_mask, tf_mask;
    int nvp;
    const unsigned* off_t;
    const unsigned* off_cb;
    const unsigned* it_of_c;
    const unsigned* off_us;
    int us_bits;
    size_t part_stride;
    double2* cpart;
    int cpart_shares;
    int t, ntiles_v;
    double2* vm;
    TileItem* vitems;
    int* vcount;
    int* vlane_parts;
    int batch;
};
hipError_t launch_project_init(const ProjArgs& a, hipStream_t s);
hipError_t launch_project_fused(const ProjArgs& a, const void* mend, void* ctile, void* yout, hipStream_t s);
hipError_t launch_project_amps(const ProjArgs& a, const long long* gather, int ngather, const long long* supp, void* small, const void* vy, const void* z,
                               hipStream_t s);
hipError_t launch_project(const ProjArgs& a, hipStream_t s);
struct UJob {
    const DevSub3* sub;
    const DevGrp* grps;
    double* umat;
    int index, nsubs;
    int inverse, entangler;
    double* umat_mirror;
    int mirror_index, mirror_nsubs;
};
hipError_t launch_ubuild(const UJob* jobs, int njobs, const double* thetas, int T, int batch, hipStream_t s, double* thetas_copy = nullptr);
struct GatherJob {
    const void* buf; size_t lane_stride; const long long* elem; int count; void* out; void* mirror;
};
struct RgradSecond {
    const DevSub3* subs;
    const DevGrp* grps;
    const double2* rpart;
    const int* lane_parts;
    const double* umat;
    int nparts, nsubs_total, count;
};
hipError_t launch_rgrad(const DevSub3* subs, const DevGrp* grps, int entangler, const double* thetas, int T, const void* rpart,
                        int ntiles, int nsubs_total, void* partial, int nslots, int from, int to, int front, int batch, hipStream_t s,
                        const int* slot_theta = nullptr, void* grads = nullptr, void* mirror = nullptr,
                        GatherJob gather = GatherJob{nullptr, 0, nullptr, 0, nullptr, nullptr},
                        int nparts = 0, int chunk = 0,
                        int sparse_subs = 0, const int* lane_parts = nullptr,
                        int conj_sub = -1, const double* umat = nullptr,
                        int nsubs_run = -1,
                        const RgradSecond* second_plan = nullptr);
constexpr int kMaxTileCands = 72;
hipError_t launch_tile_items(const DevStage& stage, const long long* supp, int per_lane, const long long* extra, int nextra, int batch,
                             TileItem* items, int* nitems, int* lane_parts, int* prev_tiles, TileItem* clear_items, int* nclear, hipStream_t s);
hipError_t launch_clear_tiles(const DevStage& stage, void* buf, size_t lane_stride, const TileItem* clear_items, const int* nclear, int max_items,
                              hipStream_t s);

struct LbState {
    int B, T, S, memory;
    double *x, *g, *f;
    double *d, *slope, *step;
    double *x_new;
    double *Smem, *Ymem, *rho;
    int *active, *done;
    long long* nit;
    double *weight, *fidelity;
    int* max_no;
    double2 *cur_hs, *cur_g0;
    double2 *acc_hs, *acc_g0;
};
hipError_t lb_prepare(const LbState& st, const void* hs, int update, double* f_out, void* raw_hs, void* x2, size_t lane_stride,
                      const long long* index, long long* prev, hipStream_t s);
hipError_t lb_take(const LbState& st, const void* grads, double* g_out, void* raw_g, hipStream_t s);
hipError_t lb_probe(const LbState& st, const void* hs, int* flags, hipStream_t s);
hipError_t lb_commit0(const LbState& st, const void* hs, const void* raw_g, double* f_out, double* g_out, hipStream_t s);
hipError_t lb_active(const LbState& st, double gtol, double fid_thr, int* flags, hipStream_t s);
hipError_t lb_direction(const LbState& st, int count, hipStream_t s);
hipError_t lb_trial(const LbState& st, double* thetas, hipStream_t s);
hipError_t lb_armijo(const LbState& st, double c1, const double* thetas, const double* ft, const void* raw_hs_t, const void* raw_g0_t,
                     int* flags, hipStream_t s);
hipError_t lb_copy_raw(const LbState& st, hipStream_t s);
hipError_t lb_history(const LbState& st, int count, double ftol, const double* f_acc, const double* g_acc, hipStream_t s);

hipError_t launch_mps_scale(void* g, const double* lam, int rows, int cols, hipStream_t s);
hipError_t launch_zgemm(bool conj_t, bool accum, int M, int N, int K, const void* A, int lda, const void* B, int ldb,
                        void* C, int ldc, hipStream_t s);
hipError_t launch_zgemm_bh(bool conj_t, bool accum, int M, int N, int K, const void* A, int lda, const void* B, int ldb,
                           void* C, int ldc, hipStream_t s);
hipError_t launch_mps_env_dot(const void* e, const void* rc, size_t count, void* out, hipStream_t s);
hipError_t launch_zgemm_batched(bool conj_t, bool accum, int M, int N, int K, const void* A, int lda, const void* B, int ldb,
                                void* C, int ldc, size_t stride_a, size_t stride_b, size_t stride_c, int nbatch, hipStream_t s);
hipError_t launch_zgemm_tables(int M, int N, int K, const void* const* a_tab, int lda, const void* const* b_tab, int ldb, void* const* c_tab, int ldc,
                               size_t stride_a, size_t stride_b, size_t stride_c, int outer, int inner, hipStream_t s, int b_transposed = 0);
hipError_t launch_mps_product(const void* const* t_tab, void* const* out_tab, int n, int count, hipStream_t s);
struct MpsSites {
    int n;
    size_t total;
    size_t offset[65];
    int lam_offset[64];
    int cols[64];
};
hipError_t launch_mps_scale_all(void* t, const double* lam, const MpsSites& sites, hipStream_t s);

int cd_num_parts(size_t npairs);
hipError_t launch_cd_dot(const void* w, const void* z, size_t npairs, int hbit, int kind, void* part, hipStream_t s);
hipError_t launch_cd_update(void* w, void* z, size_t npairs, int hbit, int kind, const void* part, int nparts,
                            const double* theta_in, double* theta_out, int tindex, double dim, hipStream_t s);
hipError_t launch_cd_entangle(void* w, void* z, size_t ngroups, int cbit, int tbit, int ent, hipStream_t s);
struct CdSegHost { int32_t ha, hb, ent, nrot, kind[4], on_b[4], tindex[4]; };
size_t cd_persistent_lds_bytes(int nbits, int T);
hipError_t launch_cd_persistent(const void* prog, int nsegs, int nbits, int col_bits, const void* target, size_t lane_stride, double* thetas,
                                int T, double* fobj, int nsweeps, int max_steps, int batch, hipStream_t s);


hipError_t launch_gate1q(const void* src, void* dst, int n, size_t ncols, int q, const double* g, hipStream_t s);
hipError_t launch_gate2q(const void* src, void* dst, int n, size_t ncols, int qc, int qt, const double* g, hipStream_t s);
int gate_dot_parts(int n, size_t ncols, int kind);
hipError_t launch_gate_dot(const void* w, const void* z, int n, size_t ncols, int kind, int q0, int q1, void* partial, void* out,
                           hipStream_t s);


int set_error(const std::string& msg);

hipError_t launch_svd_identity(void* V, int cols, hipStream_t s);
hipError_t launch_jacobi_round(void* W, int rows, void* V, int cols, const void* pairs, int npairs, double tol, const double* fro2, int* rotations,
                               hipStream_t s);
hipError_t launch_svd_fro2(const void* W, size_t n, double* out, hipStream_t s);
hipError_t launch_svd_load(const void* a, int m, int n, int mode, void* work, hipStream_t s);
hipError_t launch_svd_assemble(const void* W, const void* V, const int* ord, const double* sigma, int m, int n, int k, int mode, void* u, void* vh,
                               double* s_sorted, hipStream_t s);
bool svd_fits_small(int rows, int cols);
hipError_t launch_jacobi_small(void* W, int rows, void* V, int cols, double tol, int max_sweeps, int* sweeps_out, double* sigma_out,
                               hipStream_t s);
bool svd_fits_block(int rows, int cols);
int svd_block_size();
hipError_t launch_jacobi_block(void* W, int rows, void* V, int cols, const void* bpairs, int rounds, int per_round, double tol, int max_sweeps,
                               const double* fro2, int* rot, unsigned* bar, int* status, hipStream_t s);
hipError_t launch_svd_norms(const void* W, int rows, int cols, double* sigma, hipStream_t s);
hipError_t launch_mps_theta(const void* theta0, const double* lam_left, int chil, int chir, const double* g16, int mode, void* work, hipStream_t s);
constexpr int kLaneCap = 32;
constexpr int kLaneSite = 2 * kLaneCap * kLaneCap;
constexpr int kLaneEnv = kLaneCap * kLaneCap;
constexpr int kLaneNoConv = 1, kLaneOverflow = 2, kLaneZero = 4, kLaneLdsShort = 8;
struct LaneMps { void* T; double* lam; int* dims; double* discarded; int n, pad; };
hipError_t launch_lanes_gate1(const LaneMps& a, const LaneMps* b, const LaneOp1* ops, int nops, const LaneOp1& one, const double* thetas, int T, int lanes,
                              int bond_hint, hipStream_t s);
hipError_t launch_lanes_gate2(const LaneMps& m, const LaneMps* m2, const LaneOp2* ops, int nops, const LaneOp2& one, const double* thetas, int T,
                              double trunc_thr, int max_bond, int* status, int* peak, int lanes, int bond_hint, hipStream_t s,
                              unsigned long long* jstats = nullptr);
hipError_t launch_lanes_env_left(const LaneMps& w, const LaneMps& z, int p, const void* in, size_t in_stride, void* out, size_t out_stride,
                                 const double* gh8, int lanes, hipStream_t s);
hipError_t launch_lanes_env_right(const LaneMps& w, const LaneMps& z, int p, const void* in, size_t in_stride, void* out, size_t out_stride, int lanes,
                                  hipStream_t s);
hipError_t launch_lanes_env_dot(const LaneMps& w, const LaneMps& z, int hi, const void* e, size_t e_stride, const void* rc, size_t rc_stride, void* vals,
                                int nvals, int slot, int lanes, hipStream_t s);
struct LaneSteps { LaneGate1 g[3]; double gh[3][8]; int count, pad; };
hipError_t launch_lanes_grad_step(const LaneMps& w, const LaneMps& z, int q, const LaneSteps& steps, const double* thetas, int T, const void* env_l,
                                  size_t l_stride, const void* env_r, size_t r_stride, void* scratch, void* vals, int nvals, int slot, int lanes, hipStream_t s);
hipError_t launch_lanes_basis(const LaneMps& m, const unsigned char* bits , int lanes, hipStream_t s);
hipError_t launch_lanes_bank_dot(const LaneMps& bank, int count, const LaneMps& vh, int lanes, void* vals, int nvals, int slot0, int* status,
                                 int bond_hint, hipStream_t s);
hipError_t launch_lanes_env_init(void* env_l, size_t l_stride, void* env_r_last, size_t r_stride, int lanes, hipStream_t s);
bool mps_env_fits_small(int xa, int ua, int yb, int vb);
hipError_t launch_mps_env_left(const void* in, const void* A, const void* B, int xa, int ua, int yb, int vb, const double* gh8, void* out, hipStream_t s);
hipError_t launch_mps_env_right(const void* rc, const void* A, const void* B, int xa, int ua, int yb, int vb, void* out, hipStream_t s);
hipError_t launch_mps_theta_fused(const void* tq, const void* tq1, const double* lam_left, int chil, int chim, int chir, const double* g16, int mode,
                                  void* work, hipStream_t s);
hipError_t launch_mps_split(const void* W, const void* V, const int* ord, const double* sigma, const double* lam_left, int chil, int chir,
                            int k, int mode, double rescale, void* tq, void* tq1, const double* lam_new, double* lam_dst, hipStream_t s);
hipError_t launch_mps_colscale(void* t, const double* lam, size_t rows, int cols, int mul, hipStream_t s);

}
```

### aqc_research_amd/csrc/aqc_ws.h

```cpp
#pragma once
#include <hip/hip_runtime_api.h>

#include <cmath>
#include <cstdarg>
#include <cstdio>
#include <cstdlib>
#include <cstring>
#include <functional>
#include <map>
#include <mutex>
#include <string>
#include <vector>

#include "../../include/aqc_hip.h"
#include "aqc_device.h"
#include "aqc_launch.h"
#include "aqc_plan.h"

namespace aqc {

int fail(const char* fmt, ...) __attribute__((format(printf, 1, 2)));

#define HIP_OK(expr)                                                                              \
    do {                                                                                          \
        hipError_t e_ = (expr);                                                                   \
        if (e_ != hipSuccess) return ::aqc::fail("%s failed: %s (%s:%d)", #expr, hipGetErrorString(e_), __FILE__, __LINE__); \
    } while (0)

inline int env_int(const char* name, int dflt) {
    const char* v = getenv(name);
    return (v && *v) ? atoi(v) : dflt;
}

inline int ceil_log2(int v) {
    int b = 0;
    while ((1 << b) < v) ++b;
    return b;
}

struct DevPlan {
    Plan plan;
    std::vector<DevStage> h_stages;
    std::vector<DevOp> h_ops;
    std::vector<DevSub> h_subs;
    std::vector<DevMop> h_mops;
    DevStage* d_stages = nullptr;
    DevOp* d_ops = nullptr;
    DevSub* d_subs = nullptr;
    DevMop* d_mops = nullptr;
    int k = 0, ntiles = 0, reg_bits = 0;
    bool v2 = false;
    bool v3 = false;
    std::vector<DevSub3> h_subs3;
    std::vector<DevGrp> h_grps;
    DevSub3* d_subs3 = nullptr;
    DevGrp* d_grps = nullptr;
    double* d_umat = nullptr;
    double2* d_rpart = nullptr;
    bool u_valid = false;
    int family() const { return v3 ? 3 : (v2 ? 2 : 1); }
};

struct ListKey {
    static constexpr int kUnknown = -2, kGatherOnly = -1;
    int buf = kUnknown;
    unsigned long long supp = 0, gather = 0;
    bool operator==(const ListKey& o) const { return buf != kUnknown && buf == o.buf && supp == o.supp && gather == o.gather; }
};

struct ProjRoute {
    bool ok = false;
    int t = 0, cb = 0, us = 0, nv = 0, nvp = 0, kv = 0, ntiles_v = 0;
    int first_subs = 0;
    Program vprog;
    std::vector<int> rest;
    DevPlan vsw;
    DevPlan vinv;
    double2* vm = nullptr;
    double2* vy = nullptr;
    double2* vme = nullptr;
    double2* cpart = nullptr;
    int cpart_shares = 0;
    int vy_copies = 1;
    unsigned l0_mask = 0;
    unsigned* d_tab = nullptr;
    std::vector<unsigned> h_tab;
    unsigned ff_mask = 0, cb_mask = 0, tf_mask = 0;
    TileItem* d_items = nullptr;
    int* d_count = nullptr;
    int* d_lane_parts = nullptr;
    ListKey init_key;
};

void lower_plan(const Program& prog, const Plan& plan, DevPlan& out, int reg_bits, bool with_dots, bool mfma = false, bool presplit = false, int beam_width = 64);
int upload_plan(DevPlan& p);
Plan mirror_plan(const Plan& plan);

}

using aqc::DevPlan; using aqc::Program; using aqc::UJob;

struct aqc_ctx {
    Program prog;
    std::mutex mu;
    std::map<std::vector<int>, DevPlan> plan_cache;
    std::map<int, aqc_ws*> oneshot;
};

struct aqc_ws {
    aqc_ctx* ctx = nullptr;
    int device = 0, batch = 1, ncols = 1, pitch = 1, col_bits = 0, nbits = 0, threads = 256;
    size_t lane_elems = 0;
    hipStream_t stream = nullptr;
    DevPlan fwd, inv, sweep;
    double* d_thetas = nullptr;
    double* d_thetas_own = nullptr;
    double* d_theta_bank = nullptr;
    int bank_sets = 0, gather_count = 0;
    double* d_coef = nullptr;
    double2* bufs[AQC_NUM_BUFS] = {nullptr, nullptr, nullptr, nullptr, nullptr, nullptr};
    double* h_pin = nullptr;
    size_t pin_thetas = 0, pin_grads = 0, pin_small = 0;
    double2* d_partial = nullptr;
    double2* d_grads = nullptr;
    double* mirror_grads = nullptr;
    double* mirror_small = nullptr;
    double2* d_small = nullptr;
    double2* d_vdot_part = nullptr;
    double2* d_vdot_out = nullptr;
    long long* d_index = nullptr;
    long long* d_tmp_index = nullptr;
    double2* d_tmp_small = nullptr;
    size_t tmp_index_cap = 0, tmp_small_cap = 0;
    long long* d_basis_index = nullptr;
    long long* d_combo_prev[AQC_NUM_BUFS] = {nullptr, nullptr, nullptr, nullptr, nullptr, nullptr};
    bool combo_valid[AQC_NUM_BUFS] = {false, false, false, false, false, false};
    std::vector<long long> combo_last_elem[AQC_NUM_BUFS];
    std::vector<double> combo_last_coef[AQC_NUM_BUFS];
    void* d_sur = nullptr;
    void* h_sur = nullptr;
    int sur_states = 0;
    double* d_sur_real = nullptr;
    size_t sur_real_cap = 0;
    long long* d_combo_index = nullptr;
    double2* d_combo_coef = nullptr;
    size_t small_cap = 0, index_cap = 0;
    int* d_theta_slots = nullptr;
    int* d_slot_theta = nullptr;
    bool grads_direct = false;
    int* d_slot_ntiles = nullptr;
    int nslots = 0, vdot_parts = 0;
    bool coef_valid = false;
    bool need_coef = false;
    std::map<std::vector<long long>, hipGraphExec_t> graphs;
    bool capturing = false;
    UJob* d_ujobs = nullptr;
    bool ujobs_mirror = false;
    struct MpsSlot {
        std::vector<int> dims;
        std::vector<size_t> offset;
        double2* d_t = nullptr;
        size_t cap = 0;
    } mps[AQC_MPS_SLOTS];
    double* d_mps_lam = nullptr;
    size_t mps_lam_cap = 0;
    double2* d_mps_scratch = nullptr;
    size_t mps_scratch_cap = 0;
    struct MpsTabs { std::vector<const void*> host; const void** dev = nullptr; size_t cap = 0; unsigned long long tick = 0; };
    void* d_cd_prog = nullptr;
    int cd_nsteps = 0;
    double* d_cd_thetas = nullptr;
    double* d_cd_fobj = nullptr;
    size_t cd_fobj_cap = 0;
    MpsTabs mps_tabs[32];
    unsigned long long mps_tabs_tick = 0;
    hipEvent_t ev0 = nullptr, ev1 = nullptr, pev0 = nullptr, pev1 = nullptr;
    hipStream_t copy_stream = nullptr;
    hipEvent_t ev_ready = nullptr, ev_copied = nullptr;
    hipStream_t mps_stream = nullptr;
    hipEvent_t ev_mps_fork = nullptr, ev_mps_join = nullptr;
    bool copy_pending = false;
    const double* theta_host = nullptr;
    bool gather_rides = false;
    bool inv_mirrored = false;
    bool ckpt_valid = false;
    bool w_clean = true;
    bool sparse_enabled = true;
    bool r_only_enabled = true;
    int r_only_max_subs = 12;
    bool skipw_enabled = false;
    long sparse_min_items = 512;
    unsigned long long supp_version[AQC_NUM_BUFS] = {0, 0, 0, 0, 0, 0};
    aqc::TileItem* d_sw_items = nullptr;
    aqc::TileItem* d_sw_clear = nullptr;
    int* d_sw_counts = nullptr;
    int* d_sw_lane_parts = nullptr;
    int* d_sw_prev_tiles = nullptr;
    int sw_lists_built = 0;
    aqc::ListKey sw_items_key;
    double2* w2 = nullptr;
    double2* zw2 = nullptr;
    bool lazy_z_enabled = true;
    bool z_full = true;
    aqc::TileItem* d_vd_items = nullptr;
    size_t vd_items_cap = 0;
    unsigned long long gather_gen = 0;
    aqc::ListKey vd_key;
    aqc::ListKey z_key;
    aqc::ProjRoute proj;
    bool proj_vdag_enabled = true;
    long long proj_vdag_min_elems = 1ll << 24;
    bool proj_fused_enabled = true;
    bool proj_y0_ready = false;
    bool z_from_y = false;
    std::vector<long long> h_gather;
    aqc::ListKey projb_key;
    bool projb_ok = false;
    bool profile = false;
    int64_t prof_count[AQC_NUM_KINDS] = {};
    double prof_ms[AQC_NUM_KINDS] = {};
    std::vector<std::pair<int, float>> prof_log;
};

namespace aqc {

struct ProfScope {
    aqc_ws* ws;
    int kind;
    ProfScope(aqc_ws* w, int k) : ws(w), kind(k) {
        if (ws->profile) (void)hipEventRecord(ws->pev0, ws->stream);
    }
    ~ProfScope() {
        if (!ws->profile) return;
        float ms = 0.f;
        if (hipEventRecord(ws->pev1, ws->stream) == hipSuccess && hipEventSynchronize(ws->pev1) == hipSuccess &&
            hipEventElapsedTime(&ms, ws->pev0, ws->pev1) == hipSuccess) {
            ws->prof_count[kind] += 1;
            ws->prof_ms[kind] += ms;
            if (ws->prof_log.size() < 100000) ws->prof_log.emplace_back(kind, ms);
        }
    }
};

int check_buf(const aqc_ws* ws, int buf);
int check_block_range(const aqc_ws* ws, int block_from, int block_to);
int ensure_small(aqc_ws* ws, size_t n_cplx);
int ensure_tmp(aqc_ws* ws, size_t n_index, size_t n_cplx);
int ensure_index(aqc_ws* ws, size_t n);
int ensure_coef(aqc_ws* ws);
int copy_in(aqc_ws* ws, double2* dst, const double* src, size_t rows);
int copy_out(aqc_ws* ws, double* dst, const double2* src, size_t rows);
int results_guard(aqc_ws* ws);
int before_read(aqc_ws* ws, int buf);
int before_gather(aqc_ws* ws, int buf);
int before_write(aqc_ws* ws, int buf, bool some_lanes = false);
void lhs_support_changed(aqc_ws* ws, int buf, std::vector<long long> elem = {}, std::vector<double> coef = {});
int run_coef(aqc_ws* ws, double* d_thetas);
void thetas_changed(aqc_ws* ws, double* d_thetas);
ListKey key_of(const aqc_ws* ws, int lhs_buf, bool gather);
bool built_for(const aqc_ws* ws, const ListKey& slot, const ListKey& key);
void record_key(const aqc_ws* ws, ListKey& slot, const ListKey& key);
void replay_state_after(aqc_ws* ws);
int run_graph(aqc_ws* ws, const std::vector<long long>& key, const std::function<int()>& enqueue, const std::function<void()>& state_after);
bool vdag_route_restricted(const aqc_ws* ws, int x_buf);
int run_vdag_restricted(aqc_ws* ws, int x_buf, bool support_in_gather_set = false);
void vdag_restricted_state_after(aqc_ws* ws, int x_buf);
void vdag_projected_state_after(aqc_ws* ws, int x_buf);
int grad_from_impl(aqc_ws* ws, int x_buf, int block_from, int block_to, int front_layer, bool support_in_gather_set);
bool sweep_route_sparse(const aqc_ws* ws, int x_buf, bool will_vdag);
bool sweep_skips_zero_w(const aqc_ws* ws, int x_buf);
int sweep_r_only_sub(const aqc_ws* ws);
int sweep_sparse_prepare(aqc_ws* ws);
void apply_state_after(aqc_ws* ws, bool inverse, int src_buf, int dst_buf);
void sweep_state_after(aqc_ws* ws, bool sparse);
int ensure_umat(aqc_ws* ws, DevPlan& p);
int run_apply(aqc_ws* ws, bool inverse, int src_buf, int dst_buf);
void drop_graphs(aqc_ws* ws);
void proj_plan(aqc_ws* ws, int low_bits);
int proj_alloc(aqc_ws* ws);
void proj_free(aqc_ws* ws);
bool sweep_route_projected(const aqc_ws* ws, bool sparse);
int run_projected_stages(aqc_ws* ws);
aqc::RgradSecond projected_rgrad_plan(aqc_ws* ws);
bool vdag_route_projected(aqc_ws* ws, int x_buf);
int run_vdag_projected(aqc_ws* ws, int x_buf);
int proj_fix_amplitudes(aqc_ws* ws, int x_buf);
int ensure_sweep_items(aqc_ws* ws, int x_buf);

}
```

### aqc_research_amd/csrc/aqc_ws_project.cpp

```cpp
#include "aqc_ws.h"

#include <algorithm>

using namespace aqc;

namespace aqc {

namespace {
int popc(uint64_t v) { return __builtin_popcountll(v); }
unsigned deposit_bits(unsigned v, const std::vector<int>& bits) {
    unsigned o = 0;
    for (size_t j = 0; j < bits.size(); ++j)
        if (v >> j & 1) o |= 1u << bits[j];
    return o;
}
}

void proj_plan(aqc_ws* ws, int low_bits) {
    ProjRoute& pr = ws->proj;
    pr.ok = false;
    const Program& prog = ws->ctx->prog;
    const DevPlan& p = ws->sweep;
    if (env_int("AQC_PROJECTED", 1) == 0 || !ws->sparse_enabled || !ws->inv_mirrored || !p.v3 || ws->col_bits != 0 || ws->ncols != 1 ||
        p.plan.stages.size() < 2 || prog.n > 30)
        return;
    const int n = prog.n;
    uint64_t L0 = 0, T = 0;
    for (int b : p.plan.stages[0].bits) L0 |= 1ull << b;
    pr.rest.clear();
    for (size_t s = 1; s < p.plan.stages.size(); ++s)
        for (int gi : p.plan.stages[s].ops) {
            const GateGroup& g = prog.groups[gi];
            pr.rest.push_back(gi);
            T |= 1ull << g.q0;
            if (g.q1 >= 0) T |= 1ull << g.q1;
        }
    if (pr.rest.empty()) return;
    const uint64_t all = (1ull << n) - 1, F = all & ~L0, Cb = T & L0, Us = L0 & ~T;
    pr.t = popc(T); pr.cb = popc(Cb); pr.us = popc(Us);
    pr.nv = pr.t + pr.cb;
    if ((Us & 15) != 15 || pr.t < 4 || pr.cb > 6 || pr.nv + 2 > n || pr.nv > 20) return;
    pr.nvp = std::max(pr.nv, 8);
    pr.kv = std::min(pr.nvp, p.k);
    pr.ntiles_v = 1 << (pr.nvp - pr.kv);
    pr.first_subs = p.h_stages[0].nsubs;
    std::vector<int> tbits, cbits, usbits;
    std::vector<int> vq(n, -1);
    for (int b = 0; b < n; ++b) {
        if (T >> b & 1) { vq[b] = (int)tbits.size(); tbits.push_back(b); }
        if (Cb >> b & 1) cbits.push_back(b);
        if (Us >> b & 1) usbits.push_back(b);
    }
    pr.vprog = prog;
    for (int gi : pr.rest) {
        GateGroup& g = pr.vprog.groups[gi];
        g.q0 = vq[g.q0];
        if (g.q1 >= 0) g.q1 = vq[g.q1];
    }
    Plan best;
    for (int lb = std::max(low_bits, 2); lb >= 2; --lb) {
        Plan cand = make_plan(pr.vprog, 0, pr.kv, lb, false, &pr.rest, pr.nvp);
        if (best.stages.empty() || cand.stages.size() < best.stages.size()) best = cand;
    }
    lower_plan(pr.vprog, best, pr.vsw, 4, true, true, false, env_int("AQC_PROJECTED_BEAM", 8));
    if (!pr.vsw.v3 || !check_plan(pr.vprog, pr.vsw.plan, &pr.rest).empty()) return;
    lower_plan(pr.vprog, mirror_plan(pr.vsw.plan), pr.vinv, 4, false, true, true);
    if (!pr.vinv.v3 || pr.vinv.h_subs3.size() != pr.vsw.h_subs3.size()) return;
    for (DevPlan* q : {&pr.vsw, &pr.vinv})
        for (DevStage& ds : q->h_stages) {
            if (ds.nub >= 32) return;
            ds.ubits[ds.nub++] = pr.nvp;
            ds.ntiles *= 2;
        }
    pr.l0_mask = (unsigned)L0;
    pr.ff_mask = (unsigned)(F & ~T);
    pr.cb_mask = (unsigned)Cb;
    pr.tf_mask = (unsigned)(T & F);
    pr.h_tab.clear();
    for (unsigned i = 0; i < (1u << pr.t); ++i) pr.h_tab.push_back(deposit_bits(i, tbits));
    for (unsigned k = 0; k < (1u << pr.us); ++k) pr.h_tab.push_back(deposit_bits(k, usbits));
    for (unsigned c = 0; c < (1u << pr.cb); ++c) pr.h_tab.push_back(deposit_bits(c, cbits));
    for (unsigned c = 0; c < (1u << pr.cb); ++c) {
        const unsigned addr = deposit_bits(c, cbits);
        unsigned it = 0;
        for (size_t j = 0; j < tbits.size(); ++j)
            if (addr >> tbits[j] & 1) it |= 1u << j;
        pr.h_tab.push_back(it);
    }
    pr.ok = true;
    if (env_int("AQC_VERBOSE", 0))
        fprintf(stderr, "aqc_hip: projected route: the sweep's stages after the first run on %d virtual qubits (%d touched, %d shared with the first "
                "stage) instead of %d: %zu stage(s) of 2^%d tiles, %zu sub-stages\n", pr.nv, pr.t, pr.cb, n, pr.vsw.h_stages.size(), pr.kv,
                pr.vsw.h_subs3.size());
}

int proj_alloc(aqc_ws* ws) {
    ProjRoute& pr = ws->proj;
    if (!pr.ok) return 0;
    const size_t B = (size_t)ws->batch;
    if (upload_plan(pr.vsw) || upload_plan(pr.vinv)) return 1;
    const size_t nsubs = std::max<size_t>(pr.vsw.h_subs3.size(), 1);
    HIP_OK(hipMalloc((void**)&pr.vsw.d_umat, sizeof(double) * B * nsubs * 12 * 64));
    HIP_OK(hipMalloc((void**)&pr.vinv.d_umat, sizeof(double) * B * nsubs * 12 * 64));
    HIP_OK(hipMalloc((void**)&pr.vsw.d_rpart, sizeof(double2) * B * nsubs * (2 * (size_t)pr.ntiles_v) * 256));
    const size_t vbytes = sizeof(double2) * B * (2ull << pr.nvp);
    HIP_OK(hipMalloc((void**)&pr.vm, vbytes));
    pr.vy_copies = pr.us > 8 && pr.us <= 10 && pr.cb <= 4 ? 1 << (pr.us - 8) : 1;
    HIP_OK(hipMalloc((void**)&pr.vy, vbytes * pr.vy_copies));
    HIP_OK(hipMemsetAsync(pr.vm, 0, vbytes, ws->stream));
    HIP_OK(hipMemsetAsync(pr.vy, 0, vbytes * pr.vy_copies, ws->stream));
    pr.cpart_shares = 0;
    const long want_wgs = env_int("AQC_PROJECTED_FUSED_WGS", 512);
    if (pr.us <= 10 && pr.cb <= 4 && (long)B < want_wgs) {
        int shares = 1;
        const int cap = env_int("AQC_PROJECTED_FUSED_MAX_SHARES", 64);
        while ((long)B * pr.vy_copies * shares < want_wgs && 2 * shares <= (1 << (pr.t - 4)) && 2 * shares <= cap) shares *= 2;
        if (shares > 1) {
            HIP_OK(hipMalloc((void**)&pr.cpart, sizeof(double2) * (size_t)shares * 2 * B * (16ull << pr.us)));
            pr.cpart_shares = shares;
        }
    }
    HIP_OK(hipMalloc((void**)&pr.vme, vbytes));
    HIP_OK(hipMemsetAsync(pr.vme, 0, vbytes, ws->stream));
    HIP_OK(hipMalloc((void**)&pr.d_tab, sizeof(unsigned) * pr.h_tab.size()));
    HIP_OK(hipMemcpy(pr.d_tab, pr.h_tab.data(), sizeof(unsigned) * pr.h_tab.size(), hipMemcpyHostToDevice));
    HIP_OK(hipMalloc((void**)&pr.d_items, sizeof(TileItem) * 2 * B * pr.ntiles_v));
    HIP_OK(hipMalloc((void**)&pr.d_count, sizeof(int)));
    HIP_OK(hipMemsetAsync(pr.d_count, 0, sizeof(int), ws->stream));
    HIP_OK(hipMalloc((void**)&pr.d_lane_parts, sizeof(int) * B));
    HIP_OK(hipMemsetAsync(pr.d_lane_parts, 0, sizeof(int) * B, ws->stream));
    return 0;
}

void proj_free(aqc_ws* ws) {
    ProjRoute& pr = ws->proj;
    for (DevPlan* vp : {&pr.vsw, &pr.vinv}) {
        DevPlan& v = *vp;
        for (void* q : {(void*)v.d_stages, (void*)v.d_ops, (void*)v.d_subs, (void*)v.d_mops, (void*)v.d_subs3, (void*)v.d_grps, (void*)v.d_umat, (void*)v.d_rpart})
            if (q) (void)hipFree(q);
        v.d_stages = nullptr; v.d_ops = nullptr; v.d_subs = nullptr; v.d_mops = nullptr; v.d_subs3 = nullptr; v.d_grps = nullptr;
        v.d_umat = nullptr; v.d_rpart = nullptr;
    }
    for (void* q : {(void*)pr.vm, (void*)pr.vy, (void*)pr.vme, (void*)pr.cpart, (void*)pr.d_tab, (void*)pr.d_items, (void*)pr.d_count, (void*)pr.d_lane_parts})
        if (q) (void)hipFree(q);
    pr.vm = pr.vy = pr.vme = nullptr; pr.cpart = nullptr; pr.d_tab = nullptr; pr.d_items = nullptr; pr.d_count = nullptr; pr.d_lane_parts = nullptr;
    pr.ok = false;
}

bool sweep_route_projected(const aqc_ws* ws, bool sparse) { return sparse && ws->proj.ok; }

static ProjArgs proj_args(aqc_ws* ws);
static int ensure_pattern(aqc_ws* ws, const ProjArgs& a) {
    ProjRoute& pr = ws->proj;
    if (pr.vsw.h_stages.size() == 1 && built_for(ws, pr.init_key, ws->sw_items_key)) return 0;
    ProfScope ps(ws, AQC_K_MISC);
    HIP_OK(launch_project_init(a, ws->stream));
    record_key(ws, pr.init_key, ws->sw_items_key);
    return 0;
}

static ProjArgs proj_args(aqc_ws* ws) {
    ProjRoute& pr = ws->proj;
    ProjArgs a;
    memset(&a, 0, sizeof a);
    a.lane_stride = ws->lane_elems;
    a.items = ws->d_sw_items;
    a.nitems = ws->d_sw_counts;
    a.lane_parts = ws->d_sw_lane_parts;
    const DevStage& s0 = ws->sweep.h_stages[0];
    a.nub0 = s0.nub;
    for (int i = 0; i < s0.nub; ++i) a.ubits0[i] = s0.ubits[i];
    a.ff_mask = pr.ff_mask; a.cb_mask = pr.cb_mask; a.tf_mask = pr.tf_mask;
    a.nvp = pr.nvp;
    a.off_t = pr.d_tab;
    a.off_cb = pr.d_tab + (1u << pr.t) + (1u << pr.us);
    a.it_of_c = a.off_cb + (1u << pr.cb);
    a.off_us = pr.d_tab + (1u << pr.t);
    a.us_bits = pr.us;
    a.t = pr.t; a.cb = pr.cb; a.ntiles_v = pr.ntiles_v;
    a.vm = pr.vm;
    a.vitems = pr.d_items; a.vcount = pr.d_count; a.vlane_parts = pr.d_lane_parts;
    a.batch = ws->batch;
    return a;
}

int run_projected_stages(aqc_ws* ws) {
    ProjRoute& pr = ws->proj;
    DevPlan& v = pr.vsw;
    if (!ws->proj_y0_ready) {
        ProjArgs a = proj_args(ws);
        if (ensure_pattern(ws, a)) return 1;
        a.y = ws->bufs[AQC_BUF_ZW];
        a.s = ws->bufs[AQC_BUF_W];
        a.out = pr.vy;
        a.s_virtual = 0; a.out_virtual = 1;
        a.staged = 1;
        a.keep_bits = pr.t; a.k_bits = pr.us;
        const unsigned* off_us = pr.d_tab + (1u << pr.t);
        a.y_keep = ProjMap{pr.d_tab, 0};
        a.y_k = ProjMap{off_us, 0};
        a.s_k = ProjMap{off_us, 0};
        a.s_c = ProjMap{a.off_cb, 0};
        a.o_keep = ProjMap{nullptr, 0};
        a.o_c = ProjMap{nullptr, pr.t};
        ProfScope ps(ws, AQC_K_PROJECT);
        HIP_OK(launch_project(a, ws->stream));
    }
    const size_t m = v.h_stages.size();
    const int ntiles = 2 * pr.ntiles_v;
    for (size_t s = 0; s < m; ++s) {
        Stage3Args a;
        memset(&a, 0, sizeof a);
        a.stage = v.h_stages[s];
        a.subs = v.d_subs3;
        a.umat = v.d_umat;
        a.nsubs_total = (int)v.h_subs3.size();
        a.lane_stride = 2ull << pr.nvp;
        a.ntiles = ntiles;
        a.batch = ws->batch;
        a.in0 = pr.vm; a.in1 = pr.vy; a.out0 = pr.vm; a.out1 = pr.vy;
        a.store_out = s + 1 < m ? 3 : 0;
        a.items = pr.d_items; a.nitems = pr.d_count; a.max_items = 2 * ws->batch * pr.ntiles_v;
        a.rpart = v.d_rpart;
        a.nparts = ntiles;
        a.chunk = 0;
        if (a.stage.nsubs > 0) stage3_first_offsets(a, v.h_subs3[a.stage.sub_begin]);
        ProfScope ps(ws, AQC_K_SWEEP_VIRTUAL);
        HIP_OK(launch_sweep3(ntiles, ws->batch, pr.kv, ws->stream, a));
    }
    return 0;
}

RgradSecond projected_rgrad_plan(aqc_ws* ws) {
    ProjRoute& pr = ws->proj;
    DevPlan& v = pr.vsw;
    RgradSecond r;
    memset(&r, 0, sizeof r);
    r.subs = v.d_subs3; r.grps = v.d_grps; r.rpart = v.d_rpart; r.lane_parts = pr.d_lane_parts; r.umat = v.d_umat;
    r.nparts = 2 * pr.ntiles_v;
    r.nsubs_total = r.count = (int)v.h_subs3.size();
    return r;
}

bool vdag_route_projected(aqc_ws* ws, int x_buf) {
    ProjRoute& pr = ws->proj;
    if (!pr.ok || !ws->proj_vdag_enabled || ws->capturing || (long long)ws->lane_elems * ws->batch < ws->proj_vdag_min_elems) return false;
    const ListKey key = key_of(ws, x_buf, true);
    if (ws->projb_key == key) return ws->projb_ok;
    ws->projb_key = key;
    ws->projb_ok = false;
    const std::vector<long long>& el = ws->combo_last_elem[x_buf];
    const std::vector<double>& cf = ws->combo_last_coef[x_buf];
    const size_t B = (size_t)ws->batch;
    if (el.size() != 2 * B || cf.size() != 4 * B || (ws->gather_count > 0 && ws->h_gather.size() != (size_t)ws->gather_count)) return false;
    const unsigned fmask = ~pr.l0_mask & (unsigned)((1ull << ws->ctx->prog.n) - 1);
    for (size_t b = 0; b < B; ++b) {
        if (el[2 * b] < 0 || el[2 * b + 1] >= 0 || cf[4 * b] != 1.0 || cf[4 * b + 1] != 0.0) return false;
        const unsigned e = (unsigned)el[2 * b];
        for (long long gl : ws->h_gather) {
            const unsigned d = e ^ (unsigned)gl;
            if ((d & fmask) == 0) continue;
            if ((d & pr.l0_mask) != 0 || (d & pr.ff_mask) != 0) return false;
        }
    }
    ws->projb_ok = true;
    return true;
}

static int virtual_apply(aqc_ws* ws, DevPlan& v, const double2* src, double2* dst) {
    ProjRoute& pr = ws->proj;
    const size_t m = v.h_stages.size();
    const int ntiles = 2 * pr.ntiles_v;
    for (size_t s = 0; s < m; ++s) {
        Stage3Args a;
        memset(&a, 0, sizeof a);
        a.stage = v.h_stages[s];
        a.subs = v.d_subs3;
        a.umat = v.d_umat;
        a.nsubs_total = (int)v.h_subs3.size();
        a.lane_stride = 2ull << pr.nvp;
        a.ntiles = ntiles;
        a.batch = ws->batch;
        a.in0 = s == 0 ? src : dst;
        a.out0 = dst;
        a.items = pr.d_items; a.nitems = pr.d_count; a.max_items = 2 * ws->batch * pr.ntiles_v;
        ProfScope ps(ws, AQC_K_APPLY_VIRTUAL);
        HIP_OK(launch_apply3(ntiles, ws->batch, pr.kv, ws->stream, a));
    }
    return 0;
}

int run_vdag_projected(aqc_ws* ws, int x_buf) {
    ProjRoute& pr = ws->proj;
    DevPlan& p = ws->sweep;
    if (ensure_umat(ws, ws->inv)) return 1;
    if (!ws->d_sw_items || !ws->w_clean) return fail("objective by projection without the sparse route's preparation");
    if (ensure_sweep_items(ws, x_buf)) return 1;
    {
        Stage3Args a;
        memset(&a, 0, sizeof a);
        a.stage = p.h_stages[0];
        a.subs = p.d_subs3;
        a.umat = p.d_umat;
        a.nsubs_total = (int)p.h_subs3.size();
        a.lane_stride = ws->lane_elems;
        a.ntiles = p.ntiles;
        a.batch = ws->batch;
        a.in0 = ws->bufs[x_buf];
        a.out0 = ws->bufs[AQC_BUF_W];
        a.items = ws->d_sw_items; a.nitems = ws->d_sw_counts; a.max_items = 2 * ws->batch;
        ProfScope ps(ws, AQC_K_APPLY_LIST);
        HIP_OK(launch_apply3(p.ntiles, ws->batch, p.k, ws->stream, a));
    }
    ProjArgs a = proj_args(ws);
    if (ensure_pattern(ws, a)) return 1;
    if (virtual_apply(ws, pr.vsw, pr.vm, pr.vme)) return 1;
    const unsigned* off_us = pr.d_tab + (1u << pr.t);
    if (ws->proj_fused_enabled && pr.us <= 10 && pr.cb <= 4 && (pr.us <= 8 || pr.vy_copies == 1 << (pr.us - 8))) {
        ProjArgs q = a;
        q.part_stride = (size_t)ws->batch * (2ull << pr.nvp);
        q.cpart = pr.cpart; q.cpart_shares = pr.cpart_shares;
        q.y = ws->bufs[AQC_BUF_Y]; q.s = ws->bufs[AQC_BUF_W];
        ProfScope ps(ws, AQC_K_PROJECT);
        HIP_OK(launch_project_fused(q, pr.vme, ws->bufs[AQC_BUF_ZW], pr.vy, ws->stream));
    } else {
    {
        ProjArgs q = a;
        q.y = ws->bufs[AQC_BUF_Y]; q.s = ws->bufs[AQC_BUF_W]; q.out = pr.vy;
        q.s_virtual = 0; q.out_virtual = 1; q.staged = 1;
        q.keep_bits = pr.t; q.k_bits = pr.us;
        q.y_keep = ProjMap{pr.d_tab, 0}; q.y_k = ProjMap{off_us, 0};
        q.s_k = ProjMap{off_us, 0}; q.s_c = ProjMap{a.off_cb, 0};
        q.o_keep = ProjMap{nullptr, 0}; q.o_c = ProjMap{nullptr, pr.t};
        ProfScope ps(ws, AQC_K_PROJECT);
        HIP_OK(launch_project(q, ws->stream));
    }
    {
        ProjArgs q = a;
        q.y = ws->bufs[AQC_BUF_Y]; q.s = pr.vme; q.out = ws->bufs[AQC_BUF_ZW];
        q.s_virtual = 1; q.out_virtual = 0; q.staged = 0;
        q.keep_bits = pr.us; q.k_bits = pr.t;
        q.y_keep = ProjMap{off_us, 0}; q.y_k = ProjMap{pr.d_tab, 0};
        q.s_k = ProjMap{nullptr, 0}; q.s_c = ProjMap{nullptr, pr.t};
        q.o_keep = ProjMap{off_us, 0}; q.o_c = ProjMap{a.off_cb, 0};
        ProfScope ps(ws, AQC_K_PROJECT);
        HIP_OK(launch_project(q, ws->stream));
    }
    }
    if (virtual_apply(ws, pr.vinv, pr.vy, pr.vy)) return 1;
    {
        DevPlan& iv = ws->inv;
        Stage3Args s3;
        memset(&s3, 0, sizeof s3);
        s3.stage = iv.h_stages.back();
        s3.subs = iv.d_subs3;
        s3.umat = iv.d_umat;
        s3.nsubs_total = (int)iv.h_subs3.size();
        s3.lane_stride = ws->lane_elems;
        s3.ntiles = iv.ntiles;
        s3.batch = ws->batch;
        s3.in0 = ws->bufs[AQC_BUF_ZW];
        s3.out0 = ws->bufs[AQC_BUF_Z];
        s3.items = ws->d_sw_items; s3.nitems = ws->d_sw_counts; s3.max_items = 2 * ws->batch;
        ProfScope ps(ws, AQC_K_APPLY_LIST);
        HIP_OK(launch_apply3(iv.ntiles, ws->batch, iv.k, ws->stream, s3));
    }
    vdag_projected_state_after(ws, x_buf);
    return 0;
}

int proj_fix_amplitudes(aqc_ws* ws, int x_buf) {
    ProjRoute& pr = ws->proj;
    if (results_guard(ws)) return 1;
    ProfScope ps(ws, AQC_K_MISC);
    ProjArgs a = proj_args(ws);
    HIP_OK(launch_project_amps(a, ws->d_index, ws->gather_count, ws->d_combo_prev[x_buf], ws->d_small, pr.vy, ws->bufs[AQC_BUF_Z], ws->stream));
    return 0;
}

}
```

### aqc_research_amd/csrc/aqc_ws_sweep.cpp

```cpp
#include "aqc_ws.h"

#include <algorithm>

using namespace aqc;

namespace aqc {


void thetas_changed(aqc_ws* ws, double* d_thetas) {
    ws->d_thetas = d_thetas;
    ws->coef_valid = true;
    ws->fwd.u_valid = ws->inv.u_valid = ws->sweep.u_valid = false;
    ws->ckpt_valid = false;
    ws->z_from_y = false;
    ws->proj_y0_ready = false;
}

static void umat_state_after(aqc_ws* ws, const DevPlan& p) {
    if (!p.v3) return;
    if (&p == &ws->fwd) ws->fwd.u_valid = true;
    else ws->inv.u_valid = ws->sweep.u_valid = true;
}

static int ensure_z_full(aqc_ws* ws, bool reader);
// ... 127 lines not shown
    fprintf(stderr, "aqc_hip stamps: stage %zu workgroup lifetimes (s_memtime ticks): min %llu max %llu; starts spread over %llu, ends over %llu; "
            "first start -> last end %llu\n", s, wg_min, wg_max, last_start - first_start, last_end - first_end, last_end - first_start);
    return 0;
}
#endif

Stage3Args stage3_args(aqc_ws* ws, const DevPlan& p, size_t s) {
    Stage3Args a;
    memset(&a, 0, sizeof a);
    a.stage = p.h_stages[s];
    a.subs = p.d_subs3;
    a.umat = p.d_umat;
    a.nsubs_total = (int)p.h_subs3.size();
    a.lane_stride = ws->lane_elems;
    a.ntiles = p.ntiles;
    a.batch = ws->batch;
    return a;
}

}

static bool keeps_checkpoint(const aqc_ws* ws, bool inverse, int src_buf, int dst_buf) {
    return inverse && ws->inv_mirrored && ws->inv.v3 && dst_buf == AQC_BUF_Z && src_buf != AQC_BUF_ZW && ws->inv.h_stages.size() >= 2;
}
void apply_state_after(aqc_ws* ws, bool inverse, int src_buf, int dst_buf) {
    umat_state_after(ws, inverse ? ws->inv : ws->fwd);
    touch_buf(ws, dst_buf);
    if (keeps_checkpoint(ws, inverse, src_buf, dst_buf)) { touch_buf(ws, AQC_BUF_ZW); ws->ckpt_valid = true; }
}

int run_apply(aqc_ws* ws, bool inverse, int src_buf, int dst_buf) {
    DevPlan& p = inverse ? ws->inv : ws->fwd;
    const Program& prog = ws->ctx->prog;
    if (before_read(ws, src_buf) || before_write(ws, dst_buf)) return 1;
    if (p.v3) {
        if (ensure_umat(ws, p)) return 1;
        const bool keep = keeps_checkpoint(ws, inverse, src_buf, dst_buf);
        const size_t m = p.h_stages.size();
        for (size_t s = 0; s < m; ++s) {
            Stage3Args a = stage3_args(ws, p, s);
            const int mid = keep ? AQC_BUF_ZW : dst_buf;
            a.in0 = s == 0 ? ws->bufs[src_buf] : ws->bufs[mid];
            a.out0 = s + 1 == m ? ws->bufs[dst_buf] : ws->bufs[mid];
#ifdef AQC_TUNING
            const size_t nwg = (size_t)p.ntiles * ws->batch;
            if (stamps_begin(ws, a, nwg)) return 1;
#endif
            {
                ProfScope ps(ws, AQC_K_APPLY);
                HIP_OK(launch_apply3(p.ntiles, ws->batch, p.k, ws->stream, a));
            }
#ifdef AQC_TUNING
            if (stamps_apply(ws, a, s, nwg)) return 1;
#endif
        }
        apply_state_after(ws, inverse, src_buf, dst_buf);
        return 0;
    }
    for (size_t s = 0; s < p.h_stages.size(); ++s) {
        StageArgs a;
        memset(&a, 0, sizeof a);
        a.stage = p.d_stages + s;
        a.ops = p.d_ops;
        a.subs = p.d_subs;
        a.mops = p.d_mops;
        a.coef = ws->d_coef;
        a.ncoef = prog.n + prog.num_blocks + 1;
        a.in0 = s == 0 ? ws->bufs[src_buf] : ws->bufs[dst_buf];
        a.out0 = ws->bufs[dst_buf];
        a.lane_stride = ws->lane_elems;
        a.final_stage = (s + 1 == p.h_stages.size()) ? 1 : 0;
        ProfScope ps(ws, AQC_K_APPLY);
        if (p.v2) HIP_OK(launch_apply2(prog.entangler, p.ntiles, ws->batch, p.k, ws->stream, a));
        else HIP_OK(launch_apply(prog.entangler, inverse, p.ntiles, ws->batch, ws->threads, p.k, ws->stream, a));
    }
    apply_state_after(ws, inverse, src_buf, dst_buf);
    return 0;
}

bool vdag_route_restricted(const aqc_ws* ws, int x_buf) {
    return ws->lazy_z_enabled && sweep_route_sparse(ws, x_buf, true) && 2 + ws->gather_count <= kMaxTileCands;
}
static Stage3Args last_vdag_stage(aqc_ws* ws) {
    DevPlan& p = ws->inv;
    Stage3Args a = stage3_args(ws, p, p.h_stages.size() - 1);
    a.in0 = ws->bufs[AQC_BUF_ZW];
    a.out0 = ws->bufs[AQC_BUF_Z];
    return a;
}
int run_vdag_restricted(aqc_ws* ws, int x_buf, bool support_in_gather_set) {
    DevPlan& p = ws->inv;
    if (ensure_umat(ws, p)) return 1;
    const size_t m = p.h_stages.size();
    const size_t per_lane = 2 + (size_t)ws->gather_count;
    if (!ws->d_vd_items || ws->vd_items_cap < per_lane * ws->batch) return fail("objective V^H inside a captured graph without its preparation");
    for (size_t s = 0; s + 1 < m; ++s) {
        Stage3Args a = stage3_args(ws, p, s);
        a.in0 = s == 0 ? ws->bufs[AQC_BUF_Y] : ws->bufs[AQC_BUF_ZW];
        a.out0 = ws->bufs[AQC_BUF_ZW];
        ProfScope ps(ws, AQC_K_APPLY);
        HIP_OK(launch_apply3(p.ntiles, ws->batch, p.k, ws->stream, a));
    }
    const bool gather_only = support_in_gather_set && ws->gather_count > 0;
    const ListKey key = key_of(ws, gather_only ? ListKey::kGatherOnly : x_buf, true);
    if (!built_for(ws, ws->vd_key, key)) {
        ProfScope ps(ws, AQC_K_MISC);
        HIP_OK(launch_tile_items(p.h_stages[m - 1], gather_only ? nullptr : ws->d_combo_prev[x_buf], 2, ws->gather_count > 0 ? ws->d_index : nullptr,
                                 ws->gather_count, ws->batch, ws->d_vd_items, ws->d_sw_counts + 2, nullptr, nullptr, nullptr, nullptr, ws->stream));
        record_key(ws, ws->vd_key, key);
    }
    Stage3Args a = last_vdag_stage(ws);
    a.items = ws->d_vd_items;
    a.nitems = ws->d_sw_counts + 2;
    a.max_items = (int)(per_lane * ws->batch);
    ws->sw_lists_built |= 2;
    {
        ProfScope ps(ws, AQC_K_APPLY_LIST);
        HIP_OK(launch_apply3(p.ntiles, ws->batch, p.k, ws->stream, a));
    }
    vdag_restricted_state_after(ws, x_buf);
    return 0;
}
void vdag_restricted_state_after(aqc_ws* ws, int x_buf) {
    apply_state_after(ws, true, AQC_BUF_Y, AQC_BUF_Z);
    ws->z_full = false;
    ws->z_key = key_of(ws, x_buf, true);
}
void vdag_projected_state_after(aqc_ws* ws, int x_buf) {
    vdag_restricted_state_after(ws, x_buf);
    ws->z_key.gather = 0;
    ws->ckpt_valid = false;
    ws->z_from_y = true;
    ws->proj_y0_ready = true;
}
static int ensure_z_full(aqc_ws* ws, bool reader) {
    if (ws->z_full) return 0;
    if (ws->capturing) return fail("BUF_Z is partial inside a captured graph");
    if (ws->ckpt_valid && ws->inv.u_valid) {
        Stage3Args a = last_vdag_stage(ws);
        ProfScope ps(ws, AQC_K_APPLY);
        HIP_OK(launch_apply3(ws->inv.ntiles, ws->batch, ws->inv.k, ws->stream, a));
        ws->z_full = true;
        return 0;
    }
    if (!reader) return 0;
    if (ws->z_from_y && ws->inv.u_valid) {
        ws->z_full = true;
        return run_apply(ws, true, AQC_BUF_Y, AQC_BUF_Z);
    }
    return fail("BUF_Z holds V^H y only on the tiles the last one-call evaluation read, and the thetas (or ZW) have changed since: "
                "run aqc_ws_apply(inverse) for the whole vector");
}

void drop_graphs(aqc_ws* ws) {
    for (auto& kv : ws->graphs) (void)hipGraphExecDestroy(kv.second);
    ws->graphs.clear();
}

int run_graph(aqc_ws* ws, const std::vector<long long>& key, const std::function<int()>& enqueue, const std::function<void()>& state_after) {
    auto it = ws->graphs.find(key);
    if (it == ws->graphs.end()) {
        hipGraph_t graph = nullptr;
        hipGraphExec_t exec = nullptr;
        HIP_OK(hipStreamSynchronize(ws->stream));
        HIP_OK(hipStreamBeginCapture(ws->stream, hipStreamCaptureModeThreadLocal));
        ws->capturing = true;
        const int rc = enqueue();
        ws->capturing = false;
        const hipError_t e = hipStreamEndCapture(ws->stream, &graph);
        if (rc != 0) { if (graph) (void)hipGraphDestroy(graph); return 1; }
        if (e != hipSuccess || !graph) return fail("hipStreamEndCapture failed: %s", hipGetErrorString(e));
        const hipError_t ei = hipGraphInstantiate(&exec, graph, nullptr, nullptr, 0);
        (void)hipGraphDestroy(graph);
        if (ei != hipSuccess) return fail("hipGraphInstantiate failed: %s", hipGetErrorString(ei));
        if (ws->graphs.size() >= 16) drop_graphs(ws);
        it = ws->graphs.emplace(key, exec).first;
    }
    state_after();
    replay_state_after(ws);
    HIP_OK(hipGraphLaunch(it->second, ws->stream));
    return 0;
}

bool sweep_route_sparse(const aqc_ws* ws, int x_buf, bool will_vdag) {
    const DevPlan& p = ws->sweep;
    if (!ws->sparse_enabled || !p.v3 || !ws->inv_mirrored || p.h_stages.size() < 2) return false;
    if (!ws->combo_valid[x_buf] || !ws->d_combo_prev[x_buf]) return false;
    if (!(will_vdag ? keeps_checkpoint(ws, true, AQC_BUF_Y, AQC_BUF_Z) : (ws->ckpt_valid || ws->proj_y0_ready))) return false;
    return (long)p.ntiles * ws->batch >= ws->sparse_min_items;
}
int sweep_r_only_sub(const aqc_ws* ws) {
    const DevPlan& p = ws->sweep;
    if (!p.v3 || !ws->r_only_enabled || p.h_stages.empty()) return -1;
    const DevStage& last = p.h_stages.back();
    if (last.nsubs < 1 || last.nsubs > ws->r_only_max_subs || (p.k >= 12 && last.nsubs == 1)) return -1;
    return last.sub_begin + last.nsubs - 1;
}
bool sweep_skips_zero_w(const aqc_ws* ws, int x_buf) {
    return ws->skipw_enabled && ws->sweep.v3 && ws->combo_valid[x_buf] && ws->d_combo_prev[x_buf] != nullptr;
}
int sweep_sparse_prepare(aqc_ws* ws) {
    const DevPlan& p = ws->sweep;
    const int B = ws->batch;
    if (!ws->d_sw_items) {
        HIP_OK(hipMalloc((void**)&ws->d_sw_items, sizeof(TileItem) * 2 * B));
        HIP_OK(hipMalloc((void**)&ws->d_sw_clear, sizeof(TileItem) * 2 * B));
        HIP_OK(hipMalloc((void**)&ws->d_sw_counts, sizeof(int) * 4));
        HIP_OK(hipMemsetAsync(ws->d_sw_counts, 0, sizeof(int) * 4, ws->stream));
        HIP_OK(hipMalloc((void**)&ws->d_sw_lane_parts, sizeof(int) * B));
        HIP_OK(hipMalloc((void**)&ws->d_sw_prev_tiles, sizeof(int) * 2 * B));
        ws->w_clean = false;
    }
    if (p.h_stages.size() >= 3 && !ws->w2 && !ws->proj.ok) {
        HIP_OK(hipMalloc((void**)&ws->w2, sizeof(double2) * (size_t)B * ws->lane_elems));
        HIP_OK(hipMalloc((void**)&ws->zw2, sizeof(double2) * (size_t)B * ws->lane_elems));
    }
    const size_t vd_need = (2 + (size_t)ws->gather_count) * B;
    if (ws->lazy_z_enabled && ws->vd_items_cap < vd_need) {
        HIP_OK(hipStreamSynchronize(ws->stream));
        if (ws->d_vd_items) HIP_OK(hipFree(ws->d_vd_items));
        ws->d_vd_items = nullptr; ws->vd_items_cap = 0;
        HIP_OK(hipMalloc((void**)&ws->d_vd_items, sizeof(TileItem) * vd_need));
        ws->vd_items_cap = vd_need;
        ws->vd_key = ListKey{};
    }
    if (!ws->w_clean) {
        HIP_OK(hipMemsetAsync(ws->bufs[AQC_BUF_W], 0, sizeof(double2) * (size_t)B * ws->lane_elems, ws->stream));
        HIP_OK(hipMemsetAsync(ws->d_sw_prev_tiles, 0xff, sizeof(int) * 2 * B, ws->stream));
        ws->w_clean = true;
        ws->sw_items_key = ListKey{};
    }
    return 0;
}
void sweep_state_after(aqc_ws* ws, bool sparse) {
    umat_state_after(ws, ws->sweep);
    ws->proj_y0_ready = false;
    if (!sparse) {
        ws->w_clean = false;
        ws->ckpt_valid = false;
    }
}

}

extern "C" {

int aqc_ws_apply(aqc_ws* ws, int inverse, int src_buf, int dst_buf) {
    if (check_buf(ws, src_buf) || check_buf(ws, dst_buf)) return 1;
    if (ensure_coef(ws)) return 1;
    HIP_OK(hipSetDevice(ws->device));
    return run_apply(ws, inverse != 0, src_buf, dst_buf);
}

int aqc_ws_sweep_r_only_sub(aqc_ws* ws) { return ws ? sweep_r_only_sub(ws) : -1; }

int aqc_ws_grad(aqc_ws* ws, int block_from, int block_to, int front_layer) {
    return aqc_ws_grad_from(ws, AQC_BUF_X, block_from, block_to, front_layer);
}

int aqc_ws_grad_from(aqc_ws* ws, int x_buf, int block_from, int block_to, int front_layer) {
    return grad_from_impl(ws, x_buf, block_from, block_to, front_layer, false);
}

}

namespace aqc {

int ensure_sweep_items(aqc_ws* ws, int x_buf) {
    const DevPlan& p = ws->sweep;
    const ListKey key = key_of(ws, x_buf, false);
    if (!built_for(ws, ws->sw_items_key, key)) {
        ProfScope ps(ws, AQC_K_MISC);
        HIP_OK(launch_tile_items(p.h_stages[0], ws->d_combo_prev[x_buf], 2, nullptr, 0, ws->batch, ws->d_sw_items, ws->d_sw_counts,
                                 ws->d_sw_lane_parts, ws->d_sw_prev_tiles, ws->d_sw_clear, ws->d_sw_counts + 1, ws->stream));
        HIP_OK(launch_clear_tiles(p.h_stages[0], ws->bufs[AQC_BUF_W], ws->lane_elems, ws->d_sw_clear, ws->d_sw_counts + 1, 2 * ws->batch, ws->stream));
        record_key(ws, ws->sw_items_key, key);
        ws->sw_lists_built |= 1;
    }
    return 0;
}

int grad_from_impl(aqc_ws* ws, int x_buf, int block_from, int block_to, int front_layer, bool support_in_gather_set) {
    if (check_buf(ws, x_buf)) return 1;
    if (results_guard(ws)) return 1;
    if (x_buf == AQC_BUF_W || x_buf == AQC_BUF_ZW || x_buf == AQC_BUF_Z) return fail("lhs buffer must not be Z, W or ZW");
    if (ensure_coef(ws)) return 1;
    const Program& prog = ws->ctx->prog;
    if (block_from < 0) { block_from = 0; block_to = prog.num_blocks; }
    if (prog.num_blocks > 0 && !(0 <= block_from && block_from < block_to && block_to <= prog.num_blocks))
        return fail("invalid block_range [%d, %d)", block_from, block_to);
    HIP_OK(hipSetDevice(ws->device));
    DevPlan& p = ws->sweep;
    if (p.v3) {
        if (ensure_umat(ws, p)) return 1;
        const int nsubs = (int)p.h_subs3.size();
        const size_t m = p.h_stages.size();
        const bool sparse = sweep_route_sparse(ws, x_buf, false);
        const bool skipw = sweep_skips_zero_w(ws, x_buf);
        const bool projected = sweep_route_projected(ws, sparse);
        int r_only_sub = skipw || projected ? -1 : sweep_r_only_sub(ws);
        const bool first_stage_r_only = projected && ws->proj_y0_ready && ws->r_only_enabled && p.h_stages[0].nsubs >= 2 &&
                                        p.h_stages[0].nsubs <= ws->r_only_max_subs;
        if (first_stage_r_only) r_only_sub = p.h_stages[0].sub_begin + p.h_stages[0].nsubs - 1;
        if (!ws->z_full && !(sparse && ((support_in_gather_set && ws->z_key.gather == ws->gather_gen) ||
                                        (ws->z_key.buf == x_buf && ws->z_key.supp == ws->supp_version[x_buf]))) && ensure_z_full(ws, true))
            return 1;
        if (sparse) {
            if (!ws->capturing && sweep_sparse_prepare(ws)) return 1;
            if (!ws->d_sw_items || !ws->w_clean || (m >= 3 && !ws->w2 && !projected)) return fail("sparse sweep inside a captured graph without its preparation");
            if (ensure_sweep_items(ws, x_buf)) return 1;
        }
        for (size_t s = 0; s < (projected ? 1 : m); ++s) {
            Stage3Args a = stage3_args(ws, p, s);
            if (sparse) {
                double2* w2 = m >= 3 ? ws->w2 : nullptr;
                double2* z2 = m >= 3 ? ws->zw2 : nullptr;
                a.in0 = s == 0 ? ws->bufs[x_buf] : (s == 1 ? ws->bufs[AQC_BUF_W] : w2);
                a.in1 = s == 0 ? ws->bufs[AQC_BUF_Z] : (s == 1 ? ws->bufs[AQC_BUF_ZW] : z2);
                a.out0 = s == 0 ? ws->bufs[AQC_BUF_W] : w2;
                a.out1 = s == 0 ? nullptr : z2;
                a.store_out = s + 1 < m ? (s == 0 ? 1 : 3) : 0;
                if (s == 0) { a.items = ws->d_sw_items; a.nitems = ws->d_sw_counts; a.max_items = 2 * ws->batch; }
                if (s == 0 && first_stage_r_only) { a.r_only_last = 1; a.store_out = 0; }
            } else {
                a.in0 = s == 0 ? ws->bufs[x_buf] : ws->bufs[AQC_BUF_W];
                a.in1 = s == 0 ? ws->bufs[AQC_BUF_Z] : ws->bufs[AQC_BUF_ZW];
                a.out0 = ws->bufs[AQC_BUF_W];
                a.out1 = ws->bufs[AQC_BUF_ZW];
                a.store_out = s + 1 < m ? 3 : 0;
            }
            if (skipw && !a.items) a.supp = ws->d_combo_prev[x_buf];
            if (s + 1 == m && r_only_sub >= 0) a.r_only_last = 1;
            a.rpart = p.d_rpart;
            a.chunk = sweep3_chunk(p.ntiles, ws->batch, p.k);
            a.nparts = sweep3_nparts(p.ntiles, ws->batch, p.k);
            if (a.stage.nsubs > 0) stage3_first_offsets(a, p.h_subs3[a.stage.sub_begin]);
#ifdef AQC_TUNING
            const size_t nwg = (size_t)p.ntiles * ws->batch;
            a.debug = env_int("AQC_DEBUG_SKIP", 0);
            if (stamps_begin(ws, a, nwg)) return 1;
#endif
            {
                ProfScope ps(ws, a.items ? AQC_K_SWEEP_LIST : AQC_K_SWEEP);
                HIP_OK(launch_sweep3(p.ntiles, ws->batch, p.k, ws->stream, a));
            }
#ifdef AQC_TUNING
            if (stamps_sweep(ws, a, s, nwg)) return 1;
#endif
        }
        if (projected && run_projected_stages(ws)) return 1;
        sweep_state_after(ws, sparse);
        ProfScope ps(ws, AQC_K_FINALIZE);
        RgradSecond vwalk;
        if (projected) vwalk = projected_rgrad_plan(ws);
        HIP_OK(launch_rgrad(p.d_subs3, p.d_grps, prog.entangler, ws->d_thetas, prog.num_thetas(), p.d_rpart, p.ntiles, nsubs, ws->d_partial,
                            ws->nslots, block_from, block_to, front_layer ? 1 : 0, ws->batch, ws->stream,
                            ws->grads_direct ? ws->d_slot_theta : nullptr, ws->d_grads, ws->mirror_grads,
                            ws->gather_rides ? GatherJob{ws->bufs[AQC_BUF_Z], ws->lane_elems, ws->d_index, ws->gather_count, ws->d_small, ws->mirror_small}
                                             : GatherJob{nullptr, 0, nullptr, 0, nullptr, nullptr},
                            sweep3_nparts(p.ntiles, ws->batch, p.k), sweep3_chunk(p.ntiles, ws->batch, p.k),
                            sparse ? p.h_stages[0].nsubs : 0, sparse ? ws->d_sw_lane_parts : nullptr, r_only_sub, p.d_umat,
                            projected ? p.h_stages[0].nsubs : -1, projected ? &vwalk : nullptr));
#ifdef AQC_TUNING
        if (env_int("AQC_STAMPS", 0) != 0) { HIP_OK(hipStreamSynchronize(ws->stream)); rgrad_print_stamps(nsubs); }
#endif
        if (!ws->grads_direct)
            HIP_OK(launch_finalize(ws->d_partial, ws->d_theta_slots, ws->d_slot_ntiles, ws->d_grads, prog.num_thetas(), ws->nslots,
                                   1, prog.n, prog.tpb, block_from, block_to, front_layer ? 1 : 0, ws->batch, ws->stream, ws->mirror_grads));
        return 0;
    }
    if (before_read(ws, AQC_BUF_Z)) return 1;
    for (size_t s = 0; s < p.h_stages.size(); ++s) {
        StageArgs a;
        memset(&a, 0, sizeof a);
        a.stage = p.d_stages + s;
        a.ops = p.d_ops;
        a.subs = p.d_subs;
        a.mops = p.d_mops;
        a.coef = ws->d_coef;
        a.ncoef = prog.n + prog.num_blocks + 1;
        a.in0 = s == 0 ? ws->bufs[x_buf] : ws->bufs[AQC_BUF_W];
        a.in1 = s == 0 ? ws->bufs[AQC_BUF_Z] : ws->bufs[AQC_BUF_ZW];
        a.out0 = ws->bufs[AQC_BUF_W];
        a.out1 = ws->bufs[AQC_BUF_ZW];
        a.lane_stride = ws->lane_elems;
        a.partial = ws->d_partial;
        a.nslots = ws->nslots;
        a.ntiles_max = p.ntiles;
#ifdef AQC_TUNING
        a.debug = env_int("AQC_DEBUG_SKIP", 0);
#endif
        a.from = block_from;
        a.to = block_to;
        a.front = front_layer ? 1 : 0;
        ProfScope ps(ws, AQC_K_SWEEP);
        if (p.v2) HIP_OK(launch_sweep2(prog.entangler, p.ntiles, ws->batch, p.k, p.reg_bits, ws->stream, a));
        else HIP_OK(launch_sweep(prog.entangler, p.ntiles, ws->batch, ws->threads, p.k, ws->stream, a));
    }
    sweep_state_after(ws, false);
    ProfScope ps(ws, AQC_K_FINALIZE);
    HIP_OK(launch_finalize(ws->d_partial, ws->d_theta_slots, ws->d_slot_ntiles, ws->d_grads, prog.num_thetas(), ws->nslots,
                           p.ntiles, prog.n, prog.tpb, block_from, block_to, front_layer ? 1 : 0, ws->batch, ws->stream, ws->mirror_grads));
    return 0;
}

}

extern "C" {

int aqc_ws_objective_launch(aqc_ws* ws, int x_buf, int block_from, int block_to, int front_layer) {
    if (check_buf(ws, x_buf)) return 1;
    if (x_buf == AQC_BUF_W || x_buf == AQC_BUF_ZW || x_buf == AQC_BUF_Z || x_buf == AQC_BUF_Y) return fail("lhs buffer must be X or X2");
    if (check_block_range(ws, block_from, block_to)) return 1;
    if (ensure_coef(ws)) return 1;
    HIP_OK(hipSetDevice(ws->device));
    const bool sparse = sweep_route_sparse(ws, x_buf, true);
    if (sparse && sweep_sparse_prepare(ws)) return 1;
    const bool lazy = sparse && vdag_route_restricted(ws, x_buf);
    const bool by_projection = lazy && vdag_route_projected(ws, x_buf);
    if (by_projection) { if (run_vdag_projected(ws, x_buf)) return 1; }
    else if (lazy) { if (run_vdag_restricted(ws, x_buf)) return 1; }
    else if (run_apply(ws, true, AQC_BUF_Y, AQC_BUF_Z)) return 1;
    if (ws->gather_count > 0 && (by_projection ? proj_fix_amplitudes(ws, x_buf) : aqc_ws_gather_launch(ws, AQC_BUF_Z))) return 1;
    return grad_from_impl(ws, x_buf, block_from, block_to, front_layer, false);
}

int aqc_ws_eval(aqc_ws* ws, const double* thetas, int do_vdag, double* gathered, int x_buf, int block_from, int block_to,
                int front_layer, double* grads) {
    if (!ws) return fail("null workspace");
    HIP_OK(hipSetDevice(ws->device));
    if (ws->copy_pending) {
        HIP_OK(hipStreamSynchronize(ws->copy_stream));
        ws->copy_pending = false;
    }
    const Program& prog = ws->ctx->prog;
    const size_t nth = (size_t)ws->batch * prog.num_thetas();
    double* pin_th = ws->h_pin;
    double* pin_gr = ws->h_pin + ws->pin_thetas;
    double* pin_sm = pin_gr + ws->pin_grads;
    size_t nsm = 0;
    if (gathered) {
        if (ws->gather_count < 1) return fail("aqc_ws_gather_setup has not been called");
        nsm = (size_t)ws->batch * ws->gather_count;
        if (2 * nsm > ws->pin_small) return fail("too many gathered amplitudes for the staging buffer");
    }
    if (check_buf(ws, x_buf)) return 1;
    if (grads && check_block_range(ws, block_from, block_to)) return 1;
    if (!thetas && (do_vdag || grads) && ensure_coef(ws)) return 1;
    const bool zero_copy = sizeof(double2) * (nth + nsm) <= 65536;
    struct MirrorScope {
        aqc_ws* w;
        MirrorScope(aqc_ws* w_, double* g, double* s) : w(w_) { w->mirror_grads = g; w->mirror_small = s; }
        ~MirrorScope() {
            w->mirror_grads = nullptr; w->mirror_small = nullptr; w->theta_host = nullptr; w->gather_rides = false;
        }
    } mirror_scope(ws, zero_copy ? pin_gr : nullptr, zero_copy ? pin_sm : nullptr);
    const bool sparse = grads && (do_vdag ? sweep_route_sparse(ws, x_buf, true) : (!thetas && sweep_route_sparse(ws, x_buf, false)));
    if (sparse && sweep_sparse_prepare(ws)) return 1;
    const bool lazy = sparse && do_vdag && vdag_route_restricted(ws, x_buf);
    const bool by_projection = lazy && grads && !(gathered && zero_copy && ws->sweep.v3) && vdag_route_projected(ws, x_buf);
    if (!do_vdag && (gathered || grads) && before_read(ws, AQC_BUF_Z)) return 1;
    auto enqueue = [&]() -> int {
        if (thetas) {
            const bool direct_thetas = zero_copy && (do_vdag || grads) && ws->fwd.v3 && ws->inv.v3 && ws->sweep.v3 && !ws->need_coef &&
                                       (do_vdag ? ws->inv.v3 : true);
            if (!direct_thetas) HIP_OK(hipMemcpyAsync(ws->d_thetas_own, pin_th, sizeof(double) * nth, hipMemcpyHostToDevice, ws->stream));
            if (run_coef(ws, ws->d_thetas_own)) return 1;
            ws->theta_host = direct_thetas ? pin_th : nullptr;
        }
        if (do_vdag && (by_projection ? run_vdag_projected(ws, x_buf) : (lazy ? run_vdag_restricted(ws, x_buf) : run_apply(ws, true, AQC_BUF_Y, AQC_BUF_Z)))) return 1;
        const bool ride = gathered && grads && zero_copy && ws->sweep.v3;
        if (gathered && !ride) {
            if (by_projection ? proj_fix_amplitudes(ws, x_buf) : aqc_ws_gather_launch(ws, AQC_BUF_Z)) return 1;
            if (!zero_copy) HIP_OK(hipMemcpyAsync(pin_sm, ws->d_small, sizeof(double2) * nsm, hipMemcpyDeviceToHost, ws->stream));
        }
        ws->gather_rides = ride;
        if (grads) {
            if (aqc_ws_grad_from(ws, x_buf, block_from, block_to, front_layer)) return 1;
            if (!zero_copy) HIP_OK(hipMemcpyAsync(pin_gr, ws->d_grads, sizeof(double2) * nth, hipMemcpyDeviceToHost, ws->stream));
        }
        ws->gather_rides = false;
        ws->theta_host = nullptr;
        return 0;
    };
    if (thetas) memcpy(pin_th, thetas, sizeof(double) * nth);
    static const bool graphs_on = env_int("AQC_GRAPH", 1) != 0;
    if (thetas && graphs_on && !ws->profile) {
        const std::vector<long long> key = {do_vdag, gathered ? 1 : 0, grads ? 1 : 0, x_buf, block_from, block_to, front_layer,
                                            (long long)ws->gather_count, (long long)(size_t)ws->d_small, (long long)(size_t)ws->h_pin,
                                            (sparse ? 1 : 0) + (lazy ? 2 : 0) + (grads && sweep_skips_zero_w(ws, x_buf) ? 4 : 0) + (by_projection ? 8 : 0),
                                            (long long)(size_t)ws->d_combo_prev[x_buf],
                                            (long long)(size_t)ws->d_vd_items};
        auto state_after = [&]() {
            thetas_changed(ws, ws->d_thetas_own);
            if (do_vdag) {
                if (by_projection) vdag_projected_state_after(ws, x_buf);
                else if (lazy) vdag_restricted_state_after(ws, x_buf);
                else apply_state_after(ws, true, AQC_BUF_Y, AQC_BUF_Z);
            }
            if (grads) sweep_state_after(ws, sparse);
        };
        if (run_graph(ws, key, enqueue, state_after)) return 1;
    } else if (enqueue()) {
        return 1;
    }
    HIP_OK(hipStreamSynchronize(ws->stream));
    if (gathered) memcpy(gathered, pin_sm, sizeof(double2) * nsm);
    if (grads) memcpy(grads, pin_gr, sizeof(double2) * nth);
    return 0;
}

}
```

Before: 1.103 million evals/s.

## Pair independent apply and sweep launches into single two-list persistent kernels

Adds pair kernels that run two independent tile-list stages, a real-space apply or sweep and the projected virtual-space one, in a single launch. For persistent (K>=12) workgroups each workgroup moves from the first list to the second and prefetches the second list's first item while finishing the first. It reads both argument blocks straight from the kernarg segment. This cuts launch count and the tail idle time between back-to-back small kernels on the projected objective path. It adds complexity, macro-redirected arguments and a layout assumption about kernel-argument packing.

```diff
diff --git a/aqc_research_amd/csrc/aqc_api.cpp b/aqc_research_amd/csrc/aqc_api.cpp
--- a/aqc_research_amd/csrc/aqc_api.cpp
+++ b/aqc_research_amd/csrc/aqc_api.cpp
@@ -310,6 +310,7 @@
     ws->r_only_max_subs = env_int("AQC_R_ONLY_MAX_SUBS", 12);
     ws->proj_vdag_enabled = env_int("AQC_PROJECTED_VDAG", 1) != 0;
     ws->proj_fused_enabled = env_int("AQC_PROJECTED_FUSED", 1) != 0;
+    ws->proj_pairs_enabled = env_int("AQC_PROJECTED_PAIRS", 1) != 0;
     ws->proj_vdag_min_elems = (long long)env_int("AQC_PROJECTED_VDAG_MIN_ELEMS", 1 << 24);
     ws->skipw_enabled = env_int("AQC_SKIP_ZERO_W", 0) != 0;
     for (DevPlan* p : {&ws->fwd, &ws->inv, &ws->sweep}) {
diff --git a/aqc_research_amd/csrc/aqc_kernels3.hip b/aqc_research_amd/csrc/aqc_kernels3.hip
--- a/aqc_research_amd/csrc/aqc_kernels3.hip
+++ b/aqc_research_amd/csrc/aqc_kernels3.hip
@@ -184,11 +184,14 @@
     const int bl = wi / a.ntiles;
     return ItemAt{bl, wi - bl * a.ntiles, 0};
 }
-template <int K, bool LIST = false>
-__global__ __launch_bounds__(TileShape<K>::kWaves * 64, 2) void apply_mfma_kernel(const Stage3Args a) {
+template <int K, bool LIST, bool PAIR = false>
+__device__ __forceinline__ void apply_mfma_body(const Stage3Args& a0, const Stage3Args& b0, const int wg, const int nwg) {
     using TS = TileShape<K>;
+    static_assert(!PAIR || (LIST && K >= 12), "the pair form walks two lists with persistent workgroups");
     extern __shared__ __attribute__((aligned(16))) char smem[];
-    const DevStage& st = a.stage;
+    const Stage3Args* ca = &a0;
+#define a (*ca)
+#define st (ca->stage)
     cplx* tw = reinterpret_cast<cplx*>(smem);
     const unsigned lds_base = lds_address(smem);
     if (lds_base & ((16u << K) - 1)) __builtin_trap();
@@ -196,13 +199,16 @@
     const int wave = __builtin_amdgcn_readfirstlane((int)(threadIdx.x >> 6));
     constexpr int NL = TS::kLoads, NW = TS::kWaves;
     constexpr bool kPersist = K >= 12;
-    const int nwork = LIST ? uniform_load(a.nitems) : a.ntiles * a.batch;
-    const unsigned lo = st.dlo[lane];
-    const unsigned lo16 = lo << 4;
+    int nwork = LIST ? uniform_load(a.nitems) : a.ntiles * a.batch;
+    bool second = false;
+    if (PAIR && wg >= nwork) { ca = &b0; second = true; nwork = uniform_load(b0.nitems); }
+    unsigned lo = st.dlo[lane];
+    unsigned lo16 = lo << 4;
+    (void)lo16;
     SubRegs cur, nxt;
     SubAddr<TS::kGpw> ad;
     dbl2_t pw[NL];
-    int wi = blockIdx.x + ((kPersist || LIST) ? 0 : (int)blockIdx.y * a.ntiles);
+    int wi = wg + ((kPersist || LIST) ? 0 : (int)blockIdx.y * a.ntiles);
     if (LIST && wi >= nwork) return;
     ItemAt it = item_at<LIST>(a, wi);
     {
@@ -220,24 +226,33 @@
     const int bl = it.bl;
     const size_t lane_off = (size_t)bl * a.lane_stride + tile_base3(st, it.tile);
     const double* umat = a.umat + (size_t)bl * a.nsubs_total * 12 * 64;
-    const int nwi = wi + (int)gridDim.x;
-    const bool more = kPersist && st.nsubs > 0 && nwi < nwork;
-    const ItemAt nit = more ? item_at<LIST>(a, nwi) : ItemAt{0, 0, 0};
+    int nwi = wi + nwg;
+    bool more = kPersist && st.nsubs > 0 && nwi < nwork;
+    const Stage3Args* na = ca;
+    int nnwork = nwork;
+    if (PAIR && !more && !second) {
+        na = &b0; nwi = wg; nnwork = uniform_load(b0.nitems);
+        more = nwi < nnwork;
+    }
+    const bool change = PAIR && na != ca;
+    const ItemAt nit = more ? item_at<LIST>(*na, nwi) : ItemAt{0, 0, 0};
     const int nbl = nit.bl;
-    const size_t next_off = more ? (size_t)nbl * a.lane_stride + tile_base3(st, nit.tile) : 0;
+    const size_t next_off = more ? (size_t)nbl * na->lane_stride + tile_base3(na->stage, nit.tile) : 0;
+    const unsigned nlo = change ? na->stage.dlo[lane] : lo;
+    const unsigned nlo16 = nlo << 4;
     for (int si = 0; si < st.nsubs; ++si) {
         AQC_STAMP(4 + si);
         if (!(kApplySkip & 512)) __syncthreads();
         if (si + 1 < st.nsubs) fetch_sub<TS::kGpw>(nxt, a.subs, umat, st.sub_begin + si + 1, lane, wave, NW);
-        else if (more) fetch_sub<TS::kGpw>(nxt, a.subs, a.umat + (size_t)nbl * a.nsubs_total * 12 * 64, st.sub_begin, lane, wave, NW);
+        else if (more) fetch_sub<TS::kGpw>(nxt, na->subs, na->umat + (size_t)nbl * na->nsubs_total * 12 * 64, na->stage.sub_begin, lane, wave, NW);
         if (kPersist && more && !(kApplySkip & 64)) {
 #pragma unroll
             for (int c = 0; c < 4; ++c) {
                 if (si == (c < st.nsubs ? c : st.nsubs - 1)) {
 #pragma unroll
                     for (int i = c * (NL / 4); i < (c + 1) * (NL / 4); ++i) {
-                        const size_t ub = next_off + st.dhi[wave + i * NW];
-                        asm volatile("s_nop 4\n\tglobal_load_dwordx4 %0, %1, %2" : "=a"(pw[i]) : "v"(lo16), "s"(uniform_ptr(a.in0 + ub)) : "memory");
+                        const size_t ub = next_off + na->stage.dhi[wave + i * NW];
+                        asm volatile("s_nop 4\n\tglobal_load_dwordx4 %0, %1, %2" : "=a"(pw[i]) : "v"(nlo16), "s"(uniform_ptr(na->in0 + ub)) : "memory");
                     }
                 }
             }
@@ -301,7 +316,8 @@
         }
         if (si + 1 < st.nsubs || more) {
             cur = nxt;
-            fetch_k<TS::kGpw>(ad, a.subs, si + 1 < st.nsubs ? st.sub_begin + si + 1 : st.sub_begin, wave, NW);
+            if (si + 1 < st.nsubs) fetch_k<TS::kGpw>(ad, a.subs, st.sub_begin + si + 1, wave, NW);
+            else fetch_k<TS::kGpw>(ad, na->subs, na->stage.sub_begin, wave, NW);
         }
     }
     AQC_STAMP(4 + st.nsubs);
@@ -320,6 +336,34 @@
     __builtin_amdgcn_s_waitcnt(0xC07F);
     wi = nwi;
     it = nit;
+    if (PAIR) { ca = na; second = second || change; nwork = nnwork; lo = nlo; lo16 = nlo16; }
+    }
+#undef a
+#undef st
+}
+template <int K, bool LIST = false>
+__global__ __launch_bounds__(TileShape<K>::kWaves * 64, 2) void apply_mfma_kernel(const Stage3Args a) {
+    apply_mfma_body<K, LIST>(a, a, (int)blockIdx.x, (int)gridDim.x);
+}
+#ifndef AQC_PAIR_PLAIN_BOUNDARY
+#define AQC_PAIR_PLAIN_BOUNDARY 0
+#endif
+template <int K>
+__global__ __launch_bounds__(TileShape<K>::kWaves * 64, 2) void apply_pair_kernel(const Stage3Args a, const Stage3Args b, const int grid_a) {
+    if constexpr (K >= 12 && !AQC_PAIR_PLAIN_BOUNDARY) {
+        static_assert(sizeof(Stage3Args) % 8 == 0 && alignof(Stage3Args) == 8, "b follows a in the kernel-argument segment without padding");
+        const __attribute__((address_space(4))) char* kp = (const __attribute__((address_space(4))) char*)__builtin_amdgcn_kernarg_segment_ptr();
+        const Stage3Args* pa = (const Stage3Args*)(const void*)kp;
+        const Stage3Args* pb = (const Stage3Args*)(const void*)(kp + sizeof(Stage3Args));
+        apply_mfma_body<K, true, true>(*pa, *pb, (int)blockIdx.x, (int)gridDim.x);
+    } else if (K >= 12) {
+        apply_mfma_body<K, true>(a, a, (int)blockIdx.x, (int)gridDim.x);
+        __syncthreads();
+        apply_mfma_body<K, true>(b, b, (int)blockIdx.x, (int)gridDim.x);
+    } else if ((int)blockIdx.x < grid_a) {
+        apply_mfma_body<K, true>(a, a, (int)blockIdx.x, grid_a);
+    } else {
+        apply_mfma_body<K, true>(b, b, (int)blockIdx.x - grid_a, (int)gridDim.x - grid_a);
     }
 }
 
@@ -358,8 +402,8 @@
             if (((s2 ^ kb) & kfresh) == 0) kneed |= 1u << s2;
     }
 }
-template <int K, bool LIST = false, bool SKIPW = false, bool RLAST = false>
-__global__ __launch_bounds__(SweepShape<K>::kWaves * 64, K >= 12 ? 1 : 2) void sweep_mfma_kernel(const Stage3Args a) {
+template <int K, bool LIST, bool SKIPW, bool RLAST>
+__device__ __forceinline__ void sweep_mfma_body(const Stage3Args& a, const int wg, const int nwg) {
     using TS = TileShape<K, true>;
     constexpr int kSlots = TS::kWaves > 4 ? 4 : TS::kWaves;
     constexpr unsigned tsize = 1u << K;
@@ -382,8 +426,8 @@
     dbl2_t pw[NL], pz[NL];
     unsigned parity = 0;
     AQC_STAMP(0);
-    const int chunk = kPersist ? (LIST ? (nwork + (int)gridDim.x - 1) / (int)gridDim.x : a.chunk) : 0;
-    const int wi_first = kPersist ? (int)blockIdx.x * chunk : (int)blockIdx.x;
+    const int chunk = kPersist ? (LIST ? (nwork + nwg - 1) / nwg : a.chunk) : 0;
+    const int wi_first = kPersist ? wg * chunk : wg;
     const int wi_end = kPersist ? (wi_first + chunk < nwork ? wi_first + chunk : nwork) : wi_first + 1;
     int wi = wi_first;
     if (wi >= nwork) return;
@@ -430,7 +474,7 @@
         if (u1 >= 0 && (((unsigned long long)u1 ^ toff) & st.fresh_nonlocal) == 0) se1 = u1;
     }
     const double* umat = a.umat + (size_t)bl * a.nsubs_total * 12 * 64;
-    const int part = LIST ? it.slot : (kPersist ? (int)blockIdx.x - (bl * a.ntiles) / chunk : tile);
+    const int part = LIST ? it.slot : (kPersist ? wg - (bl * a.ntiles) / chunk : tile);
     const bool seg_first = LIST || !kPersist || wi == wi_first || tile == 0;
     cplx* rpart = a.rpart + (((size_t)bl * a.nsubs_total + st.sub_begin) * a.nparts + part) * 256;
     const int nwi = wi + 1;
@@ -509,6 +553,22 @@
     item_off = next_off;
     }
     AQC_STAMP(kStampSlots - 4);
+}
+template <int K, bool LIST = false, bool SKIPW = false, bool RLAST = false>
+__global__ __launch_bounds__(SweepShape<K>::kWaves * 64, K >= 12 ? 1 : 2) void sweep_mfma_kernel(const Stage3Args a) {
+    sweep_mfma_body<K, LIST, SKIPW, RLAST>(a, (int)blockIdx.x, (int)gridDim.x);
+}
+template <int K, bool RLAST_A, bool RLAST_B>
+__global__ __launch_bounds__(SweepShape<K>::kWaves * 64, K >= 12 ? 1 : 2) void sweep_pair_kernel(const Stage3Args a, const Stage3Args b, const int grid_a) {
+    if (K >= 12) {
+        sweep_mfma_body<K, true, false, RLAST_A>(a, (int)blockIdx.x, (int)gridDim.x);
+        __syncthreads();
+        sweep_mfma_body<K, true, false, RLAST_B>(b, (int)blockIdx.x, (int)gridDim.x);
+    } else if ((int)blockIdx.x < grid_a) {
+        sweep_mfma_body<K, true, false, RLAST_A>(a, (int)blockIdx.x, grid_a);
+    } else {
+        sweep_mfma_body<K, true, false, RLAST_B>(b, (int)blockIdx.x - grid_a, (int)gridDim.x - grid_a);
+    }
 }
 
 constexpr int kGrpChunk = 16;
@@ -938,6 +998,14 @@
     AQC_TRY(big_lds((sweep_mfma_kernel<8, true, false, true>))); AQC_TRY(big_lds((sweep_mfma_kernel<9, true, false, true>)));
     AQC_TRY(big_lds((sweep_mfma_kernel<10, true, false, true>))); AQC_TRY(big_lds((sweep_mfma_kernel<11, true, false, true>)));
     AQC_TRY(big_lds((sweep_mfma_kernel<12, true, false, true>)));
+    AQC_TRY(big_lds(apply_pair_kernel<8>)); AQC_TRY(big_lds(apply_pair_kernel<9>)); AQC_TRY(big_lds(apply_pair_kernel<10>));
+    AQC_TRY(big_lds(apply_pair_kernel<11>)); AQC_TRY(big_lds(apply_pair_kernel<12>));
+    AQC_TRY(big_lds((sweep_pair_kernel<8, false, false>))); AQC_TRY(big_lds((sweep_pair_kernel<9, false, false>)));
+    AQC_TRY(big_lds((sweep_pair_kernel<10, false, false>))); AQC_TRY(big_lds((sweep_pair_kernel<11, false, false>)));
+    AQC_TRY(big_lds((sweep_pair_kernel<12, false, false>)));
+    AQC_TRY(big_lds((sweep_pair_kernel<8, true, false>))); AQC_TRY(big_lds((sweep_pair_kernel<9, true, false>)));
+    AQC_TRY(big_lds((sweep_pair_kernel<10, true, false>))); AQC_TRY(big_lds((sweep_pair_kernel<11, true, false>)));
+    AQC_TRY(big_lds((sweep_pair_kernel<12, true, false>)));
 #undef AQC_TRY
     return hipSuccess;
 }
@@ -963,6 +1031,10 @@
     if (const char* e = getenv("AQC_SWEEP_GRID")) { const long v = atol(e); if (v > 0) return v; }
     return cus[dev];
 }
+static long apply_persist() {
+    static const long persist = []() { const char* e = getenv("AQC_APPLY_PERSIST"); return e ? atol(e) : 2L; }();
+    return persist;
+}
 hipError_t launch_apply3(int ntiles, int batch, int k, hipStream_t s, const Stage3Args& a) {
     if (a.ntiles != ntiles || a.batch != batch) return hipErrorInvalidValue;
     for (int l = 0; l < 64; ++l)
@@ -970,13 +1042,35 @@
     const bool list = a.items != nullptr;
     if (list && (!a.nitems || a.max_items < 1)) return hipErrorInvalidValue;
     const long nwork = list ? (long)a.max_items : (long)ntiles * batch;
-    static const long persist = []() { const char* e = getenv("AQC_APPLY_PERSIST"); return e ? atol(e) : 2L; }();
+    const long persist = apply_persist();
     const dim3 grid = (k >= 12 && persist > 0 && a.stage.nsubs > 0) ? dim3((unsigned)std::min<long>(nwork, persist * persistent_sweep_grid()))
                                                                      : ((k >= 12 || list) ? dim3((unsigned)nwork) : dim3(ntiles, batch));
     if (list && k >= 12 && !(persist > 0 && a.stage.nsubs > 0)) return hipErrorInvalidValue;
     const int t = mfma_threads(k, false);
     const size_t l = apply3_lds_bytes(k);
 #define AQC_LAUNCH(KK) case KK: if (list) apply_mfma_kernel<KK, true><<<grid, t, l, s>>>(a); else apply_mfma_kernel<KK, false><<<grid, t, l, s>>>(a); break
+    switch (k) {
+        AQC_LAUNCH(8); AQC_LAUNCH(9); AQC_LAUNCH(10); AQC_LAUNCH(11); AQC_LAUNCH(12);
+        default: return hipErrorInvalidValue;
+    }
+#undef AQC_LAUNCH
+    return hipGetLastError();
+}
+static_assert(2 * sizeof(Stage3Args) + 16 <= 3840, "two argument blocks must fit the kernel-argument segment");
+hipError_t launch_apply3_pair(int k, hipStream_t s, const Stage3Args& a, const Stage3Args& b) {
+    if (!a.items || !b.items || !a.nitems || !b.nitems || a.max_items < 1 || b.max_items < 1) return hipErrorInvalidValue;
+    const long persist = apply_persist();
+    if (k >= 12 && !(persist > 0 && a.stage.nsubs > 0 && b.stage.nsubs > 0)) {
+        const hipError_t e = launch_apply3(a.ntiles, a.batch, k, s, a);
+        return e != hipSuccess ? e : launch_apply3(b.ntiles, b.batch, k, s, b);
+    }
+    for (int l = 0; l < 64; ++l)
+        if (k >= 12 && (a.stage.dlo[l] >= (1u << 28) || b.stage.dlo[l] >= (1u << 28))) return hipErrorInvalidValue;
+    const long longer = std::max(a.max_items, b.max_items);
+    const dim3 grid((unsigned)(k >= 12 ? std::min<long>(longer, persist * persistent_sweep_grid()) : (long)a.max_items + b.max_items));
+    const int t = mfma_threads(k, false);
+    const size_t l = apply3_lds_bytes(k);
+#define AQC_LAUNCH(KK) case KK: apply_pair_kernel<KK><<<grid, t, l, s>>>(a, b, a.max_items); break
     switch (k) {
         AQC_LAUNCH(8); AQC_LAUNCH(9); AQC_LAUNCH(10); AQC_LAUNCH(11); AQC_LAUNCH(12);
         default: return hipErrorInvalidValue;
@@ -1012,6 +1106,26 @@
                                 else if (skipw) sweep_mfma_kernel<KK, false, true><<<grid, t, l, s>>>(a); \
                                 else if (rlast) sweep_mfma_kernel<KK, false, false, true><<<grid, t, l, s>>>(a); \
                                 else sweep_mfma_kernel<KK, false, false><<<grid, t, l, s>>>(a); break
+    switch (k) {
+        AQC_LAUNCH(8); AQC_LAUNCH(9); AQC_LAUNCH(10); AQC_LAUNCH(11); AQC_LAUNCH(12);
+        default: return hipErrorInvalidValue;
+    }
+#undef AQC_LAUNCH
+    return hipGetLastError();
+}
+
+hipError_t launch_sweep3_pair(int k, hipStream_t s, const Stage3Args& a, const Stage3Args& b) {
+    if (!a.items || !b.items || !a.nitems || !b.nitems || a.max_items < 1 || b.max_items < 1) return hipErrorInvalidValue;
+    if (a.nparts < 1 || b.nparts < 1 || a.supp || b.supp || b.r_only_last) return hipErrorInvalidValue;
+    if (k >= 12 && (a.stage.nsubs <= 0 || b.stage.nsubs <= 0)) return hipErrorInvalidValue;
+    for (int l = 0; l < 64; ++l)
+        if (k >= 12 && (a.stage.dlo[l] >= (1u << 28) || b.stage.dlo[l] >= (1u << 28))) return hipErrorInvalidValue;
+    const long longer = std::max(a.max_items, b.max_items);
+    const dim3 grid((unsigned)(k >= 12 ? std::min<long>(longer, persistent_sweep_grid()) : (long)a.max_items + b.max_items));
+    const int t = mfma_threads(k, true);
+    const size_t l = sweep3_lds_bytes(k);
+#define AQC_LAUNCH(KK) case KK: if (a.r_only_last) sweep_pair_kernel<KK, true, false><<<grid, t, l, s>>>(a, b, a.max_items); \
+                                else sweep_pair_kernel<KK, false, false><<<grid, t, l, s>>>(a, b, a.max_items); break
     switch (k) {
         AQC_LAUNCH(8); AQC_LAUNCH(9); AQC_LAUNCH(10); AQC_LAUNCH(11); AQC_LAUNCH(12);
         default: return hipErrorInvalidValue;
diff --git a/aqc_research_amd/csrc/aqc_launch.h b/aqc_research_amd/csrc/aqc_launch.h
--- a/aqc_research_amd/csrc/aqc_launch.h
+++ b/aqc_research_amd/csrc/aqc_launch.h
@@ -82,6 +82,8 @@
 int mfma_occupancy(int k, bool sweep);
 hipError_t launch_apply3(int ntiles, int batch, int k, hipStream_t s, const Stage3Args& a);
 hipError_t launch_sweep3(int ntiles, int batch, int k, hipStream_t s, const Stage3Args& a);
+hipError_t launch_apply3_pair(int k, hipStream_t s, const Stage3Args& a, const Stage3Args& b);
+hipError_t launch_sweep3_pair(int k, hipStream_t s, const Stage3Args& a, const Stage3Args& b);
 void rgrad_print_stamps(int nsubs);
 int sweep3_chunk(int ntiles, int batch, int k);
 int sweep3_nparts(int ntiles, int batch, int k);
diff --git a/aqc_research_amd/csrc/aqc_ws.h b/aqc_research_amd/csrc/aqc_ws.h
--- a/aqc_research_amd/csrc/aqc_ws.h
+++ b/aqc_research_amd/csrc/aqc_ws.h
@@ -211,6 +211,7 @@
     bool proj_vdag_enabled = true;
     long long proj_vdag_min_elems = 1ll << 24;
     bool proj_fused_enabled = true;
+    bool proj_pairs_enabled = true;
     bool proj_y0_ready = false;
     bool z_from_y = false;
     std::vector<long long> h_gather;
@@ -280,6 +281,8 @@
 int proj_alloc(aqc_ws* ws);
 void proj_free(aqc_ws* ws);
 bool sweep_route_projected(const aqc_ws* ws, bool sparse);
+bool projected_pairs(const aqc_ws* ws);
+Stage3Args projected_sweep_stage(aqc_ws* ws, size_t s);
 int run_projected_stages(aqc_ws* ws);
 aqc::RgradSecond projected_rgrad_plan(aqc_ws* ws);
 bool vdag_route_projected(aqc_ws* ws, int x_buf);
diff --git a/aqc_research_amd/csrc/aqc_ws_project.cpp b/aqc_research_amd/csrc/aqc_ws_project.cpp
--- a/aqc_research_amd/csrc/aqc_ws_project.cpp
+++ b/aqc_research_amd/csrc/aqc_ws_project.cpp
@@ -207,28 +207,42 @@
         HIP_OK(launch_project(a, ws->stream));
     }
     const size_t m = v.h_stages.size();
+    for (size_t s = 0; s < m; ++s) {
+        const Stage3Args a = projected_sweep_stage(ws, s);
+        ProfScope ps(ws, AQC_K_SWEEP_VIRTUAL);
+        HIP_OK(launch_sweep3(a.ntiles, ws->batch, pr.kv, ws->stream, a));
+    }
+    return 0;
+}
+
+Stage3Args projected_sweep_stage(aqc_ws* ws, size_t s) {
+    ProjRoute& pr = ws->proj;
+    DevPlan& v = pr.vsw;
+    const size_t m = v.h_stages.size();
     const int ntiles = 2 * pr.ntiles_v;
-    for (size_t s = 0; s < m; ++s) {
-        Stage3Args a;
-        memset(&a, 0, sizeof a);
-        a.stage = v.h_stages[s];
-        a.subs = v.d_subs3;
-        a.umat = v.d_umat;
-        a.nsubs_total = (int)v.h_subs3.size();
-        a.lane_stride = 2ull << pr.nvp;
-        a.ntiles = ntiles;
-        a.batch = ws->batch;
-        a.in0 = pr.vm; a.in1 = pr.vy; a.out0 = pr.vm; a.out1 = pr.vy;
-        a.store_out = s + 1 < m ? 3 : 0;
-        a.items = pr.d_items; a.nitems = pr.d_count; a.max_items = 2 * ws->batch * pr.ntiles_v;
-        a.rpart = v.d_rpart;
-        a.nparts = ntiles;
-        a.chunk = 0;
-        if (a.stage.nsubs > 0) stage3_first_offsets(a, v.h_subs3[a.stage.sub_begin]);
-        ProfScope ps(ws, AQC_K_SWEEP_VIRTUAL);
-        HIP_OK(launch_sweep3(ntiles, ws->batch, pr.kv, ws->stream, a));
-    }
-    return 0;
+    Stage3Args a;
+    memset(&a, 0, sizeof a);
+    a.stage = v.h_stages[s];
+    a.subs = v.d_subs3;
+    a.umat = v.d_umat;
+    a.nsubs_total = (int)v.h_subs3.size();
+    a.lane_stride = 2ull << pr.nvp;
+    a.ntiles = ntiles;
+    a.batch = ws->batch;
+    a.in0 = pr.vm; a.in1 = pr.vy; a.out0 = pr.vm; a.out1 = pr.vy;
+    a.store_out = s + 1 < m ? 3 : 0;
+    a.items = pr.d_items; a.nitems = pr.d_count; a.max_items = 2 * ws->batch * pr.ntiles_v;
+    a.rpart = v.d_rpart;
+    a.nparts = ntiles;
+    a.chunk = 0;
+    if (a.stage.nsubs > 0) stage3_first_offsets(a, v.h_subs3[a.stage.sub_begin]);
+    return a;
+}
+
+bool projected_pairs(const aqc_ws* ws) {
+    const ProjRoute& pr = ws->proj;
+    return pr.ok && ws->proj_pairs_enabled && !ws->capturing && pr.vsw.h_stages.size() == 1 && pr.vinv.h_stages.size() == 1 &&
+           ws->sweep.k == pr.kv && ws->inv.k == pr.kv;
 }
 
 RgradSecond projected_rgrad_plan(aqc_ws* ws) {
@@ -267,25 +281,27 @@
     return true;
 }
 
+static Stage3Args virtual_apply_stage(aqc_ws* ws, DevPlan& v, size_t s, const double2* src, double2* dst) {
+    ProjRoute& pr = ws->proj;
+    Stage3Args a;
+    memset(&a, 0, sizeof a);
+    a.stage = v.h_stages[s];
+    a.subs = v.d_subs3;
+    a.umat = v.d_umat;
+    a.nsubs_total = (int)v.h_subs3.size();
+    a.lane_stride = 2ull << pr.nvp;
+    a.ntiles = 2 * pr.ntiles_v;
+    a.batch = ws->batch;
+    a.in0 = s == 0 ? src : dst;
+    a.out0 = dst;
+    a.items = pr.d_items; a.nitems = pr.d_count; a.max_items = 2 * ws->batch * pr.ntiles_v;
+    return a;
+}
 static int virtual_apply(aqc_ws* ws, DevPlan& v, const double2* src, double2* dst) {
-    ProjRoute& pr = ws->proj;
-    const size_t m = v.h_stages.size();
-    const int ntiles = 2 * pr.ntiles_v;
-    for (size_t s = 0; s < m; ++s) {
-        Stage3Args a;
-        memset(&a, 0, sizeof a);
-        a.stage = v.h_stages[s];
-        a.subs = v.d_subs3;
-        a.umat = v.d_umat;
-        a.nsubs_total = (int)v.h_subs3.size();
-        a.lane_stride = 2ull << pr.nvp;
-        a.ntiles = ntiles;
-        a.batch = ws->batch;
-        a.in0 = s == 0 ? src : dst;
-        a.out0 = dst;
-        a.items = pr.d_items; a.nitems = pr.d_count; a.max_items = 2 * ws->batch * pr.ntiles_v;
+    for (size_t s = 0; s < v.h_stages.size(); ++s) {
+        const Stage3Args a = virtual_apply_stage(ws, v, s, src, dst);
         ProfScope ps(ws, AQC_K_APPLY_VIRTUAL);
-        HIP_OK(launch_apply3(ntiles, ws->batch, pr.kv, ws->stream, a));
+        HIP_OK(launch_apply3(a.ntiles, ws->batch, ws->proj.kv, ws->stream, a));
     }
     return 0;
 }
@@ -296,6 +312,8 @@
     if (ensure_umat(ws, ws->inv)) return 1;
     if (!ws->d_sw_items || !ws->w_clean) return fail("objective by projection without the sparse route's preparation");
     if (ensure_sweep_items(ws, x_buf)) return 1;
+    const bool pairs = projected_pairs(ws);
+    Stage3Args psi;
     {
         Stage3Args a;
         memset(&a, 0, sizeof a);
@@ -309,12 +327,20 @@
         a.in0 = ws->bufs[x_buf];
         a.out0 = ws->bufs[AQC_BUF_W];
         a.items = ws->d_sw_items; a.nitems = ws->d_sw_counts; a.max_items = 2 * ws->batch;
-        ProfScope ps(ws, AQC_K_APPLY_LIST);
-        HIP_OK(launch_apply3(p.ntiles, ws->batch, p.k, ws->stream, a));
+        if (pairs) {
+            psi = a;
+        } else {
+            ProfScope ps(ws, AQC_K_APPLY_LIST);
+            HIP_OK(launch_apply3(p.ntiles, ws->batch, p.k, ws->stream, a));
+        }
     }
     ProjArgs a = proj_args(ws);
     if (ensure_pattern(ws, a)) return 1;
-    if (virtual_apply(ws, pr.vsw, pr.vm, pr.vme)) return 1;
+    if (pairs) {
+        const Stage3Args mend = virtual_apply_stage(ws, pr.vsw, 0, pr.vm, pr.vme);
+        ProfScope ps(ws, AQC_K_APPLY_VIRTUAL);
+        HIP_OK(launch_apply3_pair(pr.kv, ws->stream, psi, mend));
+    } else if (virtual_apply(ws, pr.vsw, pr.vm, pr.vme)) return 1;
     const unsigned* off_us = pr.d_tab + (1u << pr.t);
     if (ws->proj_fused_enabled && pr.us <= 10 && pr.cb <= 4 && (pr.us <= 8 || pr.vy_copies == 1 << (pr.us - 8))) {
         ProjArgs q = a;
@@ -347,7 +373,7 @@
         HIP_OK(launch_project(q, ws->stream));
     }
     }
-    if (virtual_apply(ws, pr.vinv, pr.vy, pr.vy)) return 1;
+    if (!pairs && virtual_apply(ws, pr.vinv, pr.vy, pr.vy)) return 1;
     {
         DevPlan& iv = ws->inv;
         Stage3Args s3;
@@ -362,8 +388,14 @@
         s3.in0 = ws->bufs[AQC_BUF_ZW];
         s3.out0 = ws->bufs[AQC_BUF_Z];
         s3.items = ws->d_sw_items; s3.nitems = ws->d_sw_counts; s3.max_items = 2 * ws->batch;
-        ProfScope ps(ws, AQC_K_APPLY_LIST);
-        HIP_OK(launch_apply3(iv.ntiles, ws->batch, iv.k, ws->stream, s3));
+        if (pairs) {
+            const Stage3Args y0 = virtual_apply_stage(ws, pr.vinv, 0, pr.vy, pr.vy);
+            ProfScope ps(ws, AQC_K_APPLY_VIRTUAL);
+            HIP_OK(launch_apply3_pair(pr.kv, ws->stream, s3, y0));
+        } else {
+            ProfScope ps(ws, AQC_K_APPLY_LIST);
+            HIP_OK(launch_apply3(iv.ntiles, ws->batch, iv.k, ws->stream, s3));
+        }
     }
     vdag_projected_state_after(ws, x_buf);
     return 0;
diff --git a/aqc_research_amd/csrc/aqc_ws_sweep.cpp b/aqc_research_amd/csrc/aqc_ws_sweep.cpp
--- a/aqc_research_amd/csrc/aqc_ws_sweep.cpp
+++ b/aqc_research_amd/csrc/aqc_ws_sweep.cpp
@@ -453,6 +453,10 @@
         const bool first_stage_r_only = projected && ws->proj_y0_ready && ws->r_only_enabled && p.h_stages[0].nsubs >= 2 &&
                                         p.h_stages[0].nsubs <= ws->r_only_max_subs;
         if (first_stage_r_only) r_only_sub = p.h_stages[0].sub_begin + p.h_stages[0].nsubs - 1;
+        bool pair_virtual = projected && ws->proj_y0_ready && projected_pairs(ws);
+#ifdef AQC_TUNING
+        if (env_int("AQC_STAMPS", 0) != 0) pair_virtual = false;
+#endif
         if (!ws->z_full && !(sparse && ((support_in_gather_set && ws->z_key.gather == ws->gather_gen) ||
                                         (ws->z_key.buf == x_buf && ws->z_key.supp == ws->supp_version[x_buf]))) && ensure_z_full(ws, true))
             return 1;
@@ -491,7 +495,11 @@
             a.debug = env_int("AQC_DEBUG_SKIP", 0);
             if (stamps_begin(ws, a, nwg)) return 1;
 #endif
-            {
+            if (pair_virtual) {
+                const Stage3Args b = projected_sweep_stage(ws, 0);
+                ProfScope ps(ws, AQC_K_SWEEP_LIST);
+                HIP_OK(launch_sweep3_pair(p.k, ws->stream, a, b));
+            } else {
                 ProfScope ps(ws, a.items ? AQC_K_SWEEP_LIST : AQC_K_SWEEP);
                 HIP_OK(launch_sweep3(p.ntiles, ws->batch, p.k, ws->stream, a));
             }
@@ -499,7 +507,7 @@
             if (stamps_sweep(ws, a, s, nwg)) return 1;
 #endif
         }
-        if (projected && run_projected_stages(ws)) return 1;
+        if (projected && !pair_virtual && run_projected_stages(ws)) return 1;
         sweep_state_after(ws, sparse);
         ProfScope ps(ws, AQC_K_FINALIZE);
         RgradSecond vwalk;
```

Result: faster. 1.133 million evals/s, median of 6 (+2.7%).
